# kan-bayashi/espnet

Hardware: AMD Instinct MI355X
Metric: frames/sec, 12L Conformer hybrid CTC/attention training step (B=32 T=1000 d=256 per GPU) (higher is better)
Workload: dtype f32; 1 GPU; BASELINE configs[1]: 12L Conformer enc d=256 h=4 ff=2048 k=31 macaron+cnn rel_pos, 6L Transformer dec, V=5000, fbank B=32 T=1000 L=100, mtlalpha 0.3, lsm 0.1; global_batch=32, frames=1000, parallelism=dp1, optimizer=adam+noam, clip 5.0, launch=hipGraph, wgrad_side_stream=False, optimizer_steps_done=113

## Files before the change

espnet_amd/_lib.py:

```python
import ctypes as C
import os
import re

import torch

_HERE = os.path.dirname(os.path.abspath(__file__))
LIB_PATH = os.path.join(_HERE, "csrc", "libespnet_amd_hip.so")


class EamdError(RuntimeError):
    pass


class GatherT(C.Structure):
    _fields_ = [("enabled", C.c_int32), ("C", C.c_int32), ("ntap", C.c_int32), ("Ho", C.c_int32),
                ("Wo", C.c_int32), ("Hin", C.c_int32), ("Win", C.c_int32), ("sh", C.c_int32),
                ("sw", C.c_int32), ("dh", C.c_int32 * 9), ("dw", C.c_int32 * 9)]


class RowMapT(C.Structure):
    _fields_ = [("enabled", C.c_int32), ("Ho", C.c_int32), ("Wo", C.c_int32), ("Hc", C.c_int32),
                ("Wc", C.c_int32), ("sh", C.c_int32), ("oh", C.c_int32), ("sw", C.c_int32),
                ("ow", C.c_int32)]


class RowStatsT(C.Structure):
    _fields_ = [("part", C.c_void_p), ("col", C.c_void_p), ("zcol", C.c_void_p), ("zfix", C.c_void_p),
                ("fix", C.c_int32), ("reserved", C.c_int32),
                ("rowc", C.c_void_p), ("gscale", C.c_void_p), ("scale", C.c_float), ("reserved2", C.c_int32)]


class GemmT(C.Structure):
    _fields_ = [("A", C.c_void_p), ("B", C.c_void_p), ("C", C.c_void_p), ("bias", C.c_void_p),
                ("aux", C.c_void_p), ("R", C.c_void_p), ("colsum", C.c_void_p),
                ("M", C.c_int32), ("N", C.c_int32), ("K", C.c_int32),
                ("transA", C.c_int32), ("transB", C.c_int32),
                ("lda", C.c_int64), ("ldb", C.c_int64), ("ldc", C.c_int64), ("ldaux", C.c_int64),
                ("ldr", C.c_int64),
                ("batch1", C.c_int32), ("batch2", C.c_int32),
                ("sA1", C.c_int64), ("sA2", C.c_int64), ("sB1", C.c_int64), ("sB2", C.c_int64),
                ("sC1", C.c_int64), ("sC2", C.c_int64),
                ("alpha", C.c_float), ("beta", C.c_float),
                ("a_act", C.c_int32), ("b_act", C.c_int32), ("epilogue", C.c_int32),
                ("splitk", C.c_int32), ("precision", C.c_int32), ("tile", C.c_int32),
                ("gather", GatherT), ("cmap", RowMapT),
                ("Cb", C.c_void_p), ("in_dtype", C.c_int32), ("aux_dtype", C.c_int32),
                ("drop_p", C.c_float), ("drop_salt", C.c_uint64), ("drop_step", C.c_void_p), ("Hb", C.c_void_p),
                ("h_act", C.c_int32), ("h_dtype", C.c_int32),
                ("stats", RowStatsT)]


class FfnT(C.Structure):
    _fields_ = [("x", C.c_void_p), ("w1", C.c_void_p), ("b1", C.c_void_p), ("w2", C.c_void_p), ("b2", C.c_void_p),
                ("R", C.c_void_p), ("out", C.c_void_p), ("f", C.c_void_p), ("h", C.c_void_p),
                ("M", C.c_int32), ("D", C.c_int32), ("F", C.c_int32), ("act", C.c_int32),
                ("alpha", C.c_float), ("p_in", C.c_float), ("salt_in", C.c_uint64), ("p_out", C.c_float),
                ("salt_out", C.c_uint64), ("drop_step", C.c_void_p), ("dtype", C.c_int32), ("hsplit", C.c_int32),
                ("ln_x", C.c_void_p), ("ln_w", C.c_void_p), ("ln_b", C.c_void_p), ("ln_mean", C.c_void_p),
                ("ln_rstd", C.c_void_p), ("ln_eps", C.c_float), ("reserved2", C.c_int32),
                ("lnb_x", C.c_void_p), ("lnb_gamma", C.c_void_p), ("lnb_mean", C.c_void_p), ("lnb_rstd", C.c_void_p),
                ("lnb_dres", C.c_void_p), ("lnb_ws", C.c_void_p), ("lnb_drop_out", C.c_void_p), ("lnb_drop_salt", C.c_uint64),
                ("lnb_drop_p", C.c_float), ("reserved3", C.c_int32)]


class RowProjT(C.Structure):
    _fields_ = [("a", C.c_void_p), ("lda", C.c_int64), ("w", C.c_void_p), ("bias", C.c_void_p), ("R", C.c_void_p),
                ("ldr", C.c_int64), ("out", C.c_void_p), ("ldo", C.c_int64),
                ("M", C.c_int32), ("K", C.c_int32), ("N", C.c_int32), ("a_act", C.c_int32),
                ("alpha", C.c_float), ("p_out", C.c_float), ("salt_out", C.c_uint64), ("drop_step", C.c_void_p),
                ("ln_x", C.c_void_p), ("ln_w", C.c_void_p), ("ln_b", C.c_void_p), ("ln_mean", C.c_void_p),
                ("ln_rstd", C.c_void_p), ("ln_eps", C.c_float), ("lnb_drop_p", C.c_float),
                ("a_scale", C.c_void_p), ("a_shift", C.c_void_p), ("a_out", C.c_void_p),
                ("lnb_x", C.c_void_p), ("lnb_gamma", C.c_void_p), ("lnb_mean", C.c_void_p), ("lnb_rstd", C.c_void_p),
                ("lnb_dres", C.c_void_p), ("lnb_ws", C.c_void_p), ("lnb_drop_out", C.c_void_p), ("lnb_drop_salt", C.c_uint64)]


class FfnPackT(C.Structure):
    _fields_ = [("w1", C.c_void_p), ("w2", C.c_void_p), ("fwd_first", C.c_void_p), ("fwd_second", C.c_void_p),
                ("bwd_first", C.c_void_p), ("bwd_second", C.c_void_p), ("D", C.c_int32), ("F", C.c_int32)]


class RowProjPackT(C.Structure):
    _fields_ = [("w", C.c_void_p), ("image", C.c_void_p), ("K", C.c_int32), ("N", C.c_int32), ("ldw", C.c_int32),
                ("trans", C.c_int32)]


class LstmSeqFwdT(C.Structure):
    _fields_ = [("gx", C.c_void_p), ("w_hh", C.c_void_p), ("b_hh", C.c_void_p), ("live", C.c_void_p),
                ("h_out", C.c_void_p), ("c_out", C.c_void_p), ("y", C.c_void_p), ("acts", C.c_void_p),
                ("reverse", C.c_int32), ("reserved", C.c_int32)]


class LstmSeqBwdT(C.Structure):
    _fields_ = [("dy", C.c_void_p), ("w_t", C.c_void_p), ("acts", C.c_void_p), ("c_out", C.c_void_p),
                ("live", C.c_void_p), ("dgates", C.c_void_p), ("reverse", C.c_int32), ("reserved", C.c_int32)]


_lib = None

HEADER_PATH = os.path.join(os.path.dirname(_HERE), "include", "espnet_amd.h")
_BY_VALUE = {"int": C.c_int, "int32_t": C.c_int, "int64_t": C.c_int64, "uint64_t": C.c_uint64, "float": C.c_float,
             "double": C.c_double}


def parse_prototypes(text):
    text = re.sub(r"/\*.*?\*/", "", text, flags=re.S)
    protos = {}
    for ret, name, params in re.findall(r"\b(\w+)\s+(eamd_\w+)\s*\(([^()]*)\)\s*;", text):
        def ctype(decl, named):
            if "*" in decl:
                return C.c_void_p
            words = [w for w in decl.split() if w != "const"]
            base = " ".join(words[:-1] if named else words)
            if base not in _BY_VALUE:
                raise EamdError(f"{name}: cannot bind by-value type '{base}' of '{decl.strip()}'")
            return _BY_VALUE[base]
        params = [] if params.strip() in ("", "void") else params.split(",")
        protos[name] = (ctype(ret, False), [ctype(p, True) for p in params])
    return protos


with open(HEADER_PATH) as _f:
    PROTOTYPES = parse_prototypes(_f.read())
SYMBOLS = list(PROTOTYPES)


def lib():
    global _lib
    if _lib is None:
        if not os.path.exists(LIB_PATH):
            raise EamdError(
                f"{LIB_PATH} not found: build it with `python -c 'import __graft_entry__ as g; g.build()'` "
                "or `make -C espnet_amd/csrc` (there is no CPU fallback)")
        handle = C.CDLL(LIB_PATH)
        for name, (restype, argtypes) in PROTOTYPES.items():
            fn = getattr(handle, name)
            fn.restype = restype
            fn.argtypes = argtypes
        _lib = handle
    return _lib


_raw_stream = getattr(torch._C, "_cuda_getCurrentRawStream", None)
_cur_device = getattr(torch._C, "_cuda_getDevice", None)


def stream_ptr():
    if _raw_stream is not None and _cur_device is not None:
        return _raw_stream(_cur_device())
    return torch.cuda.current_stream().cuda_stream


EAMD_EUNSUPPORTED = -2


def check(rc, what):
    if rc != 0:
        raise EamdError(f"{what} failed with code {rc}")


def ptr(t, offset=0):
    if t is None:
        return None
    if not t.is_cuda:
        raise EamdError("espnet_amd kernels need GPU tensors (no CPU fallback in the product path)")
    if offset == 0:
        return t.data_ptr()
    return t.data_ptr() + offset * t.element_size()


def f32(t):
    if t.dtype != torch.float32:
        raise EamdError(f"expected float32 tensor, got {t.dtype}")
    return t
```

espnet_amd/csrc/rowproj_f32.hip:

```cpp
#include <stdlib.h>
#include <type_traits>
#include "common.h"
#include "../../include/espnet_amd.h"
#include "ln_bwd_rows.h"

namespace {

constexpr int RBM = 32;
constexpr int RNT = 512;
constexpr int RCH = 256;
constexpr int ST_LD = 36;
constexpr int ST_SZ = RBM * ST_LD;
constexpr int TL_LD = 264;

__device__ __forceinline__ int xs_ld(int K) { return K + 8; }

__device__ __forceinline__ void stage_ln(const eamd_rowproj_t& p, const int m0, const int t, float* xs, const int LD) {
  constexpr int D = 256;
  const int row = t >> 4, l = t & 15;
  const bool live = m0 + row < p.M;
  const long gr = (long)min(m0 + row, p.M - 1);
  const float4* __restrict__ xr = reinterpret_cast<const float4*>(p.ln_x + gr * D);
  float4 v[4];
  float s = 0.f;
#pragma unroll
  for (int j = 0; j < 4; ++j) { v[j] = xr[l + 16 * j]; s += v[j].x + v[j].y + v[j].z + v[j].w; }
#pragma unroll
  for (int m = 1; m < 16; m <<= 1) s += __shfl_xor(s, m);
  const float mean = s / D;
  float q = 0.f;
#pragma unroll
  for (int j = 0; j < 4; ++j) {
    const float a = v[j].x - mean, b = v[j].y - mean, c = v[j].z - mean, d = v[j].w - mean;
    q += a * a + b * b + c * c + d * d;
  }
#pragma unroll
  for (int m = 1; m < 16; m <<= 1) q += __shfl_xor(q, m);
  const float rstd = rsqrtf(q / D + p.ln_eps);
  const float4* __restrict__ g4 = reinterpret_cast<const float4*>(p.ln_w);
  const float4* __restrict__ b4 = reinterpret_cast<const float4*>(p.ln_b);
#pragma unroll
  for (int j = 0; j < 4; ++j) {
    const float4 g = g4[l + 16 * j], b = b4[l + 16 * j];
    float4 o;
    o.x = (v[j].x - mean) * rstd * g.x + b.x;
    o.y = (v[j].y - mean) * rstd * g.y + b.y;
    o.z = (v[j].z - mean) * rstd * g.z + b.z;
    o.w = (v[j].w - mean) * rstd * g.w + b.w;
    const int col = (l + 16 * j) * 4;
    *reinterpret_cast<float4*>(&xs[row * LD + col]) = o;
    if (live) *reinterpret_cast<float4*>(const_cast<float*>(p.a) + gr * D + col) = o;
  }
  if (live && l == 0) { p.ln_mean[gr] = mean; p.ln_rstd[gr] = rstd; }
}

__device__ __forceinline__ void stage_affine(const eamd_rowproj_t& p, const int m0, const int t, float* xs, const int LD) {
  constexpr int D = 256;
#pragma unroll
  for (int i = 0; i < 4; ++i) {
    const int idx = t + RNT * i, row = idx >> 6, c4 = idx & 63;
    const long gr = (long)min(m0 + row, p.M - 1);
    const float4 v = *reinterpret_cast<const float4*>(p.a + gr * p.lda + c4 * 4);
    const float4 sc = *reinterpret_cast<const float4*>(p.a_scale + c4 * 4), sh = *reinterpret_cast<const float4*>(p.a_shift + c4 * 4);
    float4 o;
    o.x = eamd_act(v.x * sc.x + sh.x, p.a_act); o.y = eamd_act(v.y * sc.y + sh.y, p.a_act);
    o.z = eamd_act(v.z * sc.z + sh.z, p.a_act); o.w = eamd_act(v.w * sc.w + sh.w, p.a_act);
    *reinterpret_cast<float4*>(&xs[row * LD + c4 * 4]) = o;
    if (p.a_out && m0 + row < p.M) *reinterpret_cast<float4*>(p.a_out + gr * D + c4 * 4) = o;
  }
}

template <bool LNB>
__global__ __launch_bounds__(RNT, 2) void rowproj_f32_kernel(const eamd_rowproj_t p) {
  extern __shared__ __attribute__((aligned(16))) float sm[];
  const int K = p.K, N = p.N;
  const int LD = xs_ld(K);
  float* const xs = sm;
  const int t = threadIdx.x;
  const int lane = t & 63, wave = __builtin_amdgcn_readfirstlane(t >> 6);
  const int fr = lane & 15, fq = lane >> 4;
  const int m0 = blockIdx.x * RBM;
  const int S = K >> 5;
  const int nchunk = N / RCH;
  const int nsteps = S * nchunk;
  float* const st = sm + RBM * LD + wave * ST_SZ;

  if (p.ln_x) {
    stage_ln(p, m0, t, xs, LD);
  } else if (p.a_scale) {
    stage_affine(p, m0, t, xs, LD);
  } else {
    const int c4n = K >> 2;
    for (int idx = t; idx < RBM * c4n; idx += RNT) {
      const int row = idx / c4n, c4 = idx - row * c4n;
      *reinterpret_cast<f32x4*>(&xs[row * LD + c4 * 4]) =
          *reinterpret_cast<const f32x4*>(p.a + (long)min(m0 + row, p.M - 1) * p.lda + c4 * 4);
    }
  }

  const char* __restrict__ Wb = reinterpret_cast<const char*>(p.w) + (long)wave * 4096 + lane * 16;
  f32x4 bs[4][4];
  auto load_b = [&](auto set_c, int g) __attribute__((always_inline)) {
    constexpr int SET = decltype(set_c)::value;
    const char* base = Wb + (long)min(g, nsteps - 1) * (8 * 4096);
#pragma unroll
    for (int v = 0; v < 4; ++v) bs[SET][v] = *reinterpret_cast<const f32x4*>(base + v * 1024);
  };
  float fA[2][2][4];
  auto read_a = [&](int kcol, auto half_c) __attribute__((always_inline)) {
    constexpr int hh = decltype(half_c)::value;
#pragma unroll
    for (int i = 0; i < 2; ++i) {
      const float4 v = *reinterpret_cast<const float4*>(&xs[(i * 16 + fr) * LD + kcol + hh * 16 + fq * 4]);
      fA[hh][i][0] = v.x; fA[hh][i][1] = v.y; fA[hh][i][2] = v.z; fA[hh][i][3] = v.w;
    }
  };
  f32x4 acc[2][2];
  auto mfma_half = [&](auto set_c, auto half_c) __attribute__((always_inline)) {
    constexpr int SET = decltype(set_c)::value, q = decltype(half_c)::value;
#pragma unroll
    for (int e = 0; e < 4; ++e)
#pragma unroll
      for (int i = 0; i < 2; ++i)
#pragma unroll
        for (int j = 0; j < 2; ++j)
          acc[i][j] = __builtin_amdgcn_mfma_f32_16x16x4f32(fA[q][i][e], bs[SET][q * 2 + j][e], acc[i][j], 0, 0, 0);
  };
  using I0 = std::integral_constant<int, 0>;
  using I1 = std::integral_constant<int, 1>;
  auto step = [&](auto s_c, int g, int kcol, int kcol_next) __attribute__((always_inline)) {
    constexpr int s = decltype(s_c)::value;
    load_b(std::integral_constant<int, (s + 3) & 3>{}, g + 3);
    __builtin_amdgcn_sched_barrier(0);
    read_a(kcol, I1{});
    mfma_half(std::integral_constant<int, s & 3>{}, I0{});
    __builtin_amdgcn_sched_barrier(0);
    read_a(kcol_next, I0{});
    mfma_half(std::integral_constant<int, s & 3>{}, I1{});
  };

  load_b(std::integral_constant<int, 0>{}, 0);
  load_b(std::integral_constant<int, 1>{}, 1);
  load_b(std::integral_constant<int, 2>{}, 2);
  __syncthreads();
  read_a(0, I0{});

  const unsigned thr_out = eamd_drop_thr16(p.p_out);
  const float inv_out = eamd_drop_inv(thr_out);
  const unsigned seed_out = p.p_out > 0.f ? eamd_drop_seed((const unsigned long long*)p.drop_step, p.salt_out) : 0u;

  int g = 0;
  for (int c = 0; c < nchunk; ++c) {
#pragma unroll
    for (int i = 0; i < 2; ++i)
#pragma unroll
      for (int j = 0; j < 2; ++j) acc[i][j] = (f32x4){0.f, 0.f, 0.f, 0.f};
    for (int kp = 0; kp < S; kp += 4) {
      const int k0 = kp * 32;
      step(std::integral_constant<int, 0>{}, g + 0, k0, k0 + 32);
      step(std::integral_constant<int, 1>{}, g + 1, k0 + 32, k0 + 64);
      step(std::integral_constant<int, 2>{}, g + 2, k0 + 64, k0 + 96);
      step(std::integral_constant<int, 3>{}, g + 3, k0 + 96, (kp + 4 < S) ? k0 + 128 : 0);
      g += 4;
    }
    if constexpr (!LNB) {
#pragma unroll
      for (int i = 0; i < 2; ++i)
#pragma unroll
        for (int r = 0; r < 4; ++r)
          *reinterpret_cast<float2*>(&st[(i * 16 + fq * 4 + r) * ST_LD + 2 * fr]) = make_float2(acc[i][0][r], acc[i][1][r]);
      __builtin_amdgcn_fence(__ATOMIC_RELEASE, "wavefront");
      __builtin_amdgcn_wave_barrier();
      __builtin_amdgcn_fence(__ATOMIC_ACQUIRE, "wavefront");
      const int col0 = c * RCH + wave * 32 + (lane & 7) * 4;
      float4 b4 = make_float4(0.f, 0.f, 0.f, 0.f);
      if (p.bias) b4 = *reinterpret_cast<const float4*>(p.bias + col0);
#pragma unroll
      for (int it = 0; it < 4; ++it) {
        const int lr = it * 8 + (lane >> 3);
        const int row = m0 + lr;
        const float4 a4 = *reinterpret_cast<const float4*>(&st[lr * ST_LD + (lane & 7) * 4]);
        if (row < p.M) {
          float v[4] = {a4.x + b4.x, a4.y + b4.y, a4.z + b4.z, a4.w + b4.w};
          const long gi = (long)row * N + col0;
          if (p.p_out > 0.f) {
            bool keep[4];
            eamd_drop_keep4(seed_out, (unsigned long long)gi, thr_out, keep);
#pragma unroll
            for (int e = 0; e < 4; ++e) v[e] = keep[e] ? v[e] * inv_out : 0.f;
          }
          float4 r4 = make_float4(0.f, 0.f, 0.f, 0.f);
          if (p.R) r4 = *reinterpret_cast<const float4*>(p.R + (long)row * p.ldr + col0);
          *reinterpret_cast<float4*>(p.out + (long)row * p.ldo + col0) =
              make_float4(v[0] * p.alpha + r4.x, v[1] * p.alpha + r4.y, v[2] * p.alpha + r4.z, v[3] * p.alpha + r4.w);
        }
      }
      __builtin_amdgcn_wave_barrier();
    }
  }

  if constexpr (LNB) {
    constexpr int D = 256;
    float* const tl = sm;
    float* const gs = sm + RBM * TL_LD;
    float* const bsum = gs + RBM * D;
    __syncthreads();
#pragma unroll
    for (int i = 0; i < 2; ++i)
#pragma unroll
      for (int r = 0; r < 4; ++r)
        *reinterpret_cast<float2*>(&tl[(i * 16 + fq * 4 + r) * TL_LD + wave * 32 + 2 * fr]) = make_float2(acc[i][0][r], acc[i][1][r]);
    __syncthreads();
    const EamdLnbArgs la{p.lnb_x, p.lnb_gamma, p.lnb_mean, p.lnb_rstd, p.lnb_dres, p.lnb_ws, p.lnb_drop_out, p.lnb_drop_p,
                         (unsigned long long)p.lnb_drop_salt, p.drop_step, p.out, (long)p.ldo, p.M};
    eamd_ln_bwd_rows32<TL_LD>(la, tl, gs, bsum, m0, t, (int)blockIdx.x);
  }
}

struct PackJob { const float* w; float* img; int K, N, ldw, trans; long npiece; };
constexpr int PACK_JOBS = 48;
struct PackTable { PackJob j[PACK_JOBS]; };
__global__ __launch_bounds__(256) void rowproj_pack_kernel(const PackTable tab) {
  const PackJob jb = tab.j[blockIdx.y];
  for (long piece = (long)blockIdx.x * 256 + threadIdx.x; piece < jb.npiece; piece += (long)gridDim.x * 256) {
    const int lane = piece & 63, v = (piece >> 6) & 3, w = (piece >> 8) & 7;
    const long gs_ = piece >> 11;
    const int S = jb.K >> 5;
    const int c = (int)(gs_ / S), s = (int)(gs_ - (long)c * S);
    const int fr = lane & 15, fq = lane >> 4, q = v >> 1, j = v & 1;
    const int col = c * RCH + w * 32 + 2 * fr + j, k = s * 32 + q * 16 + fq * 4;
    float4 o;
    if (jb.trans) {
      const float* r0 = jb.w + (long)k * jb.ldw + col;
      o = make_float4(r0[0], r0[jb.ldw], r0[2L * jb.ldw], r0[3L * jb.ldw]);
    } else {
      o = *reinterpret_cast<const float4*>(jb.w + (long)col * jb.ldw + k);
    }
    *reinterpret_cast<float4*>(jb.img + piece * 4) = o;
  }
}

bool al16(const void* q) { return (reinterpret_cast<uintptr_t>(q) & 15) == 0; }

size_t smem_bytes(int K, bool lnb) {
  size_t rows = (size_t)RBM * (K + 8);
  if (lnb) {
    const size_t need = (size_t)RBM * TL_LD + 2 * (size_t)RBM * 256;
    return (rows > need ? rows : need) * sizeof(float);
  }
  return (rows + 8 * (size_t)ST_SZ) * sizeof(float);
}

int check_rowproj(const eamd_rowproj_t* p) {
  if (!p || !p->a || !p->w || !p->out) return EAMD_EINVAL;
  if (p->M <= 0 || p->K <= 0 || p->N <= 0) return EAMD_EINVAL;
  if (p->K % 256 != 0 || p->N % RCH != 0 || p->K > 768) return EAMD_EUNSUPPORTED;
  if (p->lda < p->K || p->ldo < p->N || (p->R && p->ldr < p->N)) return EAMD_EINVAL;
  if (p->lda % 4 != 0 || p->ldo % 4 != 0 || (p->R && p->ldr % 4 != 0)) return EAMD_EUNSUPPORTED;
  if (!al16(p->a) || !al16(p->w) || !al16(p->out) || (p->R && !al16(p->R)) || (p->bias && !al16(p->bias))) return EAMD_EUNSUPPORTED;
  if (p->p_out < 0.f || p->p_out >= 1.f) return EAMD_EINVAL;
  if (p->p_out > 0.f && (!p->drop_step || p->ldo != p->N)) return EAMD_EINVAL;
  if (p->ln_x) {
    if (p->K != 256 || p->a_scale || !p->ln_w || !p->ln_b || !p->ln_mean || !p->ln_rstd || p->lda != 256) return EAMD_EINVAL;
    if (!al16(p->ln_x) || !al16(p->ln_w) || !al16(p->ln_b)) return EAMD_EUNSUPPORTED;
  }
  if (p->a_scale) {
    if (p->K != 256 || !p->a_shift) return EAMD_EINVAL;
    if (!al16(p->a_scale) || !al16(p->a_shift) || (p->a_out && !al16(p->a_out))) return EAMD_EUNSUPPORTED;
  }
  if (p->lnb_x) {
    if (p->N != 256 || !p->lnb_gamma || !p->lnb_mean || !p->lnb_rstd || !p->lnb_ws || p->R || p->p_out > 0.f) return EAMD_EINVAL;
    if (p->lnb_drop_out && (!p->drop_step || p->lnb_drop_p < 0.f || p->lnb_drop_p >= 1.f)) return EAMD_EINVAL;
    if (!al16(p->lnb_x) || !al16(p->lnb_gamma) || (p->lnb_dres && !al16(p->lnb_dres)) || (p->lnb_drop_out && !al16(p->lnb_drop_out)))
      return EAMD_EUNSUPPORTED;
  }
  return EAMD_OK;
}

template <bool LNB>
int launch_rowproj(const eamd_rowproj_t& p, hipStream_t stream) {
  const size_t smem = smem_bytes(p.K, LNB);
  static int attr_done = 0;
  if (!attr_done) {
    const hipError_t e = hipFuncSetAttribute(reinterpret_cast<const void*>(&rowproj_f32_kernel<LNB>),
                                             hipFuncAttributeMaxDynamicSharedMemorySize, (int)smem_bytes(768, LNB));
    if (e != hipSuccess) return (int)e;
    attr_done = 1;
  }
  hipLaunchKernelGGL((rowproj_f32_kernel<LNB>), dim3((p.M + RBM - 1) / RBM), dim3(RNT), smem, stream, p);
  EAMD_LAUNCH_CHECK();
  return EAMD_OK;
}

}

extern "C" int64_t eamd_rowproj_lnb_workspace(int M) { return (int64_t)((M + RBM - 1) / RBM) * 2 * 256; }

extern "C" int eamd_rowproj(const eamd_rowproj_t* p, void* stream) {
  const int rc = check_rowproj(p);
  if (rc != EAMD_OK) return rc;
  return p->lnb_x ? launch_rowproj<true>(*p, (hipStream_t)stream) : launch_rowproj<false>(*p, (hipStream_t)stream);
}

extern "C" int eamd_rowproj_pack_f32(const eamd_rowproj_pack_t* jobs, int njobs, void* stream) {
  if (!jobs || njobs <= 0) return EAMD_EINVAL;
  for (int i0 = 0; i0 < njobs; i0 += PACK_JOBS) {
    const int n = njobs - i0 < PACK_JOBS ? njobs - i0 : PACK_JOBS;
    PackTable tab;
    long most = 0;
    for (int i = 0; i < n; ++i) {
      const eamd_rowproj_pack_t& q = jobs[i0 + i];
      if (!q.w || !q.image || q.K <= 0 || q.N <= 0 || q.ldw <= 0) return EAMD_EINVAL;
      if (q.K % 256 != 0 || q.N % RCH != 0 || !al16(q.image)) return EAMD_EUNSUPPORTED;
      if (!q.trans && (!al16(q.w) || q.ldw % 4 != 0)) return EAMD_EUNSUPPORTED;
      if (q.ldw < (q.trans ? q.N : q.K)) return EAMD_EINVAL;
      tab.j[i] = PackJob{q.w, q.image, q.K, q.N, q.ldw, q.trans, (long)q.K * q.N / 4};
      if (tab.j[i].npiece > most) most = tab.j[i].npiece;
    }
    const unsigned bx = (unsigned)((most + 255) / 256 < 256 ? (most + 255) / 256 : 256);
    hipLaunchKernelGGL(rowproj_pack_kernel, dim3(bx, n), dim3(256), 0, (hipStream_t)stream, tab);
    EAMD_LAUNCH_CHECK();
  }
  return EAMD_OK;
}
```

espnet_amd/functional.py:

```python
import math

import torch

from . import ops
from .ops import (ACT_NONE, ACT_RELU, ACT_SWISH, EPI_DACT_FACTOR, EPI_MUL_AUX, EPI_MUL_DSWISH, EPI_MUL_RELU_MASK, EPI_NONE,
                  EPI_RELU)


class GradSink:

    on_done = None
    on_use = None

    @staticmethod
    def use(params):
        if GradSink.on_use is not None and torch.is_grad_enabled():
            GradSink.on_use(params)
        return params

    def __init__(self, params):
        self.params = list(params)
        self.ret = [None] * len(self.params)

    def buf(self, i):
        p = self.params[i]
        if p is None:
            return None
        g = getattr(p, "_eamd_grad", None)
        if g is not None:
            return g
        if self.ret[i] is None:
            self.ret[i] = torch.zeros_like(p)
        return self.ret[i]

    def results(self):
        if GradSink.on_done is not None:
            ops.wgrad_join()
            GradSink.on_done(self.params)
        return tuple(self.ret)


FUSE_GRAD_DROP = True


def _tag_out(out, p_out, s_out):
    if FUSE_GRAD_DROP and p_out > 0.0:
        out._eamd_out_drop = (float(p_out), int(s_out))
    return out


def _prev_drop(x):
    return getattr(x, "_eamd_out_drop", None) if FUSE_GRAD_DROP else None


def _grad_in(dout, do, p_out, s_out):
    pre = getattr(dout, "_eamd_dropped", None)
    if pre is not None and pre[1] == (float(p_out), int(s_out)) and pre[0].numel() == do.numel():
        return pre[0].view(do.shape)
    return ops.dropout(do, p_out, s_out, out_dtype=ops.act_dtype()) if p_out > 0.0 else ops.to_act(do)


def _ln_fwd_in(x2, ln_w, ln_b, eps, adt):
    if eps is None:
        return ops.to_act(x2), None, None
    return ops.layernorm_fwd(x2, ln_w, ln_b, eps, adt)


def _ln_bwd_out(dxn, x2, ln_w, mean, rstd, do, gbuf, bbuf, prev, shp):
    if mean is None:
        return dxn.float().view(shp) if dxn.dtype != torch.float32 else dxn.view(shp)
    if prev is not None and x2.shape[1] in (256, 512):
        dx, dx16 = ops.layernorm_bwd(dxn, x2, ln_w, mean, rstd, do, gbuf, bbuf, drop=prev)
        out = dx.view(shp)
        out._eamd_dropped = (dx16, prev)
        return out
    return ops.layernorm_bwd(dxn, x2, ln_w, mean, rstd, do, gbuf, bbuf).view(shp)


def _rp_ln_bwd(dy, img, x2, ln_w, mean, rstd, do, gbuf, bbuf, prev, shp):
    M, D = x2.shape
    ws = ops.rowproj_lnb_ws(M, x2.device)
    dcopy = torch.empty(M, D, device=x2.device, dtype=torch.float32) if prev is not None else None
    dx = ops.rowproj(dy, img, D, lnb=(x2, ln_w, mean, rstd, do, ws, dcopy, prev))
    ops.ln_partials_reduce(ws, gbuf, bbuf, (M + 31) // 32, D)
    out = dx.view(shp)
    if prev is not None:
        out._eamd_dropped = (dcopy, prev)
    return out


def _act_epi(act):
    return {ACT_RELU: EPI_MUL_RELU_MASK, ACT_SWISH: EPI_MUL_DSWISH}[act]


class _NoGradCtx:
    needs_input_grad = (False,) * 64

    def save_for_backward(self, *tensors):
        pass

    def mark_non_differentiable(self, *tensors):
        pass

    def set_materialize_grads(self, value):
        pass


def run(fn, *args):
    if torch.is_grad_enabled():
        return fn.apply(*args)
    with ops.inference():
        return fn.forward(_NoGradCtx(), *args)


class DropoutFn(torch.autograd.Function):
    @staticmethod
    def forward(ctx, x, p, salt):
        ctx.cfg = (p, salt)
        return ops.dropout(x.contiguous(), p, salt)

    @staticmethod
    def backward(ctx, dy):
        p, salt = ctx.cfg
        return ops.dropout(dy.contiguous(), p, salt), None, None


def dropout(x, p, salt, training):
    return DropoutFn.apply(x, p, salt) if (training and p > 0.0) else x


class MaskRowsFn(torch.autograd.Function):

    @staticmethod
    def forward(ctx, x, keep):
        k8 = keep.reshape(-1).to(torch.uint8).contiguous()
        ctx.save_for_backward(k8)
        return ops.mask_rows(x.reshape(-1, x.shape[-1]).contiguous(), k8).view(x.shape)

    @staticmethod
    def backward(ctx, dy):
        (k8,) = ctx.saved_tensors
        return ops.mask_rows(dy.reshape(-1, dy.shape[-1]).contiguous(), k8).view(dy.shape), None


class LayerNormFn(torch.autograd.Function):
    @staticmethod
    def forward(ctx, x, weight, bias, eps):
        shp = x.shape
        x2 = x.reshape(-1, shp[-1]).contiguous()
        y, mean, rstd = ops.layernorm_fwd(x2, weight, bias, eps)
        ctx.save_for_backward(x2, mean, rstd)
        ctx.pr = GradSink.use((weight, bias))
        ctx.shp = shp
        ctx.prev = _prev_drop(x)
        return y.view(shp)

    @staticmethod
    def backward(ctx, dy):
        x2, mean, rstd = ctx.saved_tensors
        w, b = ctx.pr
        sink = GradSink([w, b])
        dy2 = dy.reshape(x2.shape).contiguous()
        dx = _ln_bwd_out(dy2, x2, w, mean, rstd, None, sink.buf(0), sink.buf(1), ctx.prev, ctx.shp)
        return (dx,) + sink.results() + (None,)


class LinearFn(torch.autograd.Function):
    @staticmethod
    def forward(ctx, x, weight, bias):
        shp = x.shape
        x2 = ops.to_act(x.reshape(-1, shp[-1]).contiguous())
        y = ops.linear_fwd(x2, ops.wshadow(weight), bias)
        ctx.save_for_backward(x2)
        ctx.pr = GradSink.use((weight, bias))
        ctx.shp = shp
        return y.view(*shp[:-1], weight.shape[0])

    @staticmethod
    def backward(ctx, dy):
        (x2,) = ctx.saved_tensors
        w, b = ctx.pr
        sink = GradSink([w, b] if b is not None else [w])
        dy2 = ops.to_act(dy.reshape(x2.shape[0], w.shape[0]).contiguous())
        dx = ops.linear_bwd_x(dy2, ops.wshadow(w)) if ctx.needs_input_grad[0] else None
        ops.linear_bwd_w(dy2, x2, sink.buf(0), db=sink.buf(1) if b is not None else None)
        res = sink.results()
        return (dx.view(ctx.shp) if dx is not None else None, res[0], res[1] if b is not None else None)


FFN_FACTOR = True


class FFNBlockFn(torch.autograd.Function):

    @staticmethod
    def forward(ctx, x, ln_w, ln_b, w1, b1, w2, b2, scale, act, eps, drop=(0.0, 0, 0.0, 0)):
        shp = x.shape
        D = shp[-1]
        adt = ops.act_dtype()
        p_in, s_in, p_out, s_out = drop
        x2 = x.reshape(-1, D).contiguous()
        assert eps is not None or p_out <= 0.0
        fused = ops.fast()
        h, zf = None, False
        one = eps is not None and (ops.fast() or ops.f32_epilogue_drop())
        ln_in = None
        if one and ops.FFN_LN_FUSED and x2.dtype == torch.float32 and D == 256:
            xn = torch.empty(x2.shape, device=x2.device, dtype=adt)
            if ops.ffn_fused_ok(xn, ops.wshadow(w1), ops.wshadow(w2), act):
                mean = torch.empty(x2.shape[0], device=x2.device, dtype=torch.float32)
                rstd = torch.empty(x2.shape[0], device=x2.device, dtype=torch.float32)
                ln_in = (x2, ln_w, ln_b, eps, mean, rstd)
        if ln_in is None:
            xn, mean, rstd = _ln_fwd_in(x2, ln_w, ln_b, eps, adt)
        if one and (ln_in is not None or ops.ffn_fused_ok(xn, ops.wshadow(w1), ops.wshadow(w2), act)):
            need = any(ctx.needs_input_grad[:7])
            packs = ops.ffn_pack(w1, w2)
            out, z, h = ops.ffn_fwd(xn, ops.wshadow(w1), b1, ops.wshadow(w2), b2, act=act, alpha=scale, R=x2,
                                    drop=(p_in, s_in, p_out, s_out), save=need, packed=packs[:2], ln=ln_in)
            ctx.packs = packs[2:]
            ctx.save_for_backward(x2, mean, rstd, xn, z, h)
            ctx.pr = GradSink.use((ln_w, ln_b, w1, b1, w2, b2))
            ctx.cfg = (scale, act, shp, drop)
            ctx.zf, ctx.one_launch = True, True
            ctx.prev = _prev_drop(x)
            return _tag_out(out.view(shp), p_out, s_out)
        ctx.one_launch = False
        if act not in (ACT_RELU, ACT_SWISH):
            if not (p_in > 0.0 and (fused or ops.f32_epilogue_drop())):
                z = ops.linear_fwd(xn, ops.wshadow(w1), b1)
                h = ops.act_fwd_any(z, act)
                if p_in > 0.0:
                    h = ops.dropout(h, p_in, s_in)
                hop = ops.to_act(h)
                if p_out > 0.0 and (fused or ops.f32_epilogue_drop()):
                    out = ops.linear_fwd(hop, ops.wshadow(w2), b2, R=x2 if eps is not None else None, alpha=scale, drop=(p_out, s_out))
                elif p_out > 0.0:
                    out = ops.axpby(x2, ops.dropout(ops.linear_fwd(hop, ops.wshadow(w2), b2), p_out, s_out), 1.0, scale)
                else:
                    out = ops.linear_fwd(hop, ops.wshadow(w2), b2, R=x2 if eps is not None else None, alpha=scale)
                ctx.save_for_backward(x2, mean, rstd, xn, z, hop)
                ctx.pr = GradSink.use((ln_w, ln_b, w1, b1, w2, b2))
                ctx.cfg = (scale, act, shp, drop)
                ctx.zf, ctx.generic_act = False, True
                ctx.prev = _prev_drop(x)
                return _tag_out(out.view(shp), p_out, s_out)
        ctx.generic_act = False
        if p_in > 0.0 and (fused or ops.f32_epilogue_drop()):
            h = torch.empty(x2.shape[0], w1.shape[0], device=x2.device, dtype=adt)
            z = ops.linear_fwd(xn, ops.wshadow(w1), b1, out_dtype=adt, drop=(p_in, s_in), Hb=h, h_act=act,
                               act=EPI_DACT_FACTOR if FFN_FACTOR else EPI_NONE)
            zf = FFN_FACTOR
        else:
            z = ops.linear_fwd(xn, ops.wshadow(w1), b1, out_dtype=adt)
            if p_in > 0.0:
                h = ops.dropout(z, p_in, s_in, act=act)
        src, a_act = (h, ACT_NONE) if h is not None else (z, act)
        if p_out > 0.0 and (fused or ops.f32_epilogue_drop()):
            out = ops.linear_fwd(src, ops.wshadow(w2), b2, R=x2, alpha=scale, a_act=a_act, drop=(p_out, s_out))
        elif p_out > 0.0:
            br = ops.linear_fwd(src, ops.wshadow(w2), b2, a_act=a_act)
            out = ops.axpby(x2, ops.dropout(br, p_out, s_out), 1.0, scale)
        else:
            out = ops.linear_fwd(src, ops.wshadow(w2), b2, R=x2 if eps is not None else None, alpha=scale, a_act=a_act)
        ctx.save_for_backward(x2, mean, rstd, xn, z, h)
        ctx.pr = GradSink.use((ln_w, ln_b, w1, b1, w2, b2))
        ctx.cfg = (scale, act, shp, drop)
        ctx.zf = zf
        ctx.prev = _prev_drop(x)
        return _tag_out(out.view(shp), p_out, s_out)

    @staticmethod
    def backward(ctx, dout):
        x2, mean, rstd, xn, z, h = ctx.saved_tensors
        ln_w, ln_b, w1, b1, w2, b2 = ctx.pr
        scale, act, shp, (p_in, s_in, p_out, s_out) = ctx.cfg
        adt = ops.act_dtype()
        sink = GradSink(ctx.pr)
        do = dout.reshape(x2.shape).contiguous()
        dob = _grad_in(dout, do, p_out, s_out)
        inner = h is not None
        if h is not None:
            ops.linear_bwd_w(dob, h, sink.buf(4), alpha=scale, db=sink.buf(5))
        else:
            ops.linear_bwd_w(dob, z, sink.buf(4), alpha=scale, b_act=act, db=sink.buf(5))
        if getattr(ctx, "generic_act", False):
            dh = ops.linear_bwd_x(dob, ops.wshadow(w2), alpha=scale)
            if p_in > 0.0:
                dh = ops.dropout(dh, p_in, s_in)
            dz = ops.to_act(ops.act_bwd_any(dh, z, act))
            ops.linear_bwd_w(dz, xn, sink.buf(2), db=sink.buf(3))
            dxn = ops.linear_bwd_x(dz, ops.wshadow(w1))
            dx = _ln_bwd_out(dxn, x2, ln_w, mean, rstd, do, sink.buf(0), sink.buf(1), ctx.prev, shp)
            return (dx,) + sink.results() + (None, None, None, None)
        if ctx.one_launch and dob.dtype == z.dtype:
            M, D = x2.shape
            if mean is not None and D == 256 and ops.ROWPROJ and ops.ffn_bwd_lnb_ok(M, w1.shape[0], dob.dtype):
                ws = ops.rowproj_lnb_ws(M, x2.device)
                prev = ctx.prev
                dcopy = torch.empty(M, D, device=x2.device, dtype=torch.float32) if prev is not None else None
                dz, dx = ops.ffn_bwd(dob, w1, w2, z, alpha=scale, packed=ctx.packs,
                                     lnb=(x2, ln_w, mean, rstd, do, ws, dcopy, prev))
                ops.ln_partials_reduce(ws, sink.buf(0), sink.buf(1), (M + 31) // 32, D)
                ops.linear_bwd_w(dz, xn, sink.buf(2), db=sink.buf(3))
                dx = dx.view(shp)
                if prev is not None:
                    dx._eamd_dropped = (dcopy, prev)
                return (dx,) + sink.results() + (None, None, None, None)
            dz, dxn = ops.ffn_bwd(dob, w1, w2, z, alpha=scale, packed=ctx.packs)
            ops.linear_bwd_w(dz, xn, sink.buf(2), db=sink.buf(3))
            dx = _ln_bwd_out(dxn, x2, ln_w, mean, rstd, do, sink.buf(0), sink.buf(1), ctx.prev, shp)
            return (dx,) + sink.results() + (None, None, None, None)
        if ctx.zf:
            dz = ops.linear_bwd_x(dob, ops.wshadow(w2), epilogue=EPI_MUL_AUX, aux=z, alpha=scale, out_dtype=adt)
        elif inner and (ops.fast() or ops.f32_epilogue_drop()):
            dz = ops.linear_bwd_x(dob, ops.wshadow(w2), epilogue=_act_epi(act), aux=z, alpha=scale, out_dtype=adt,
                                  drop=(p_in, s_in))
        else:
            dz = ops.linear_bwd_x(dob, ops.wshadow(w2), epilogue=_act_epi(act), aux=z, alpha=scale, out_dtype=adt)
            if inner:
                dz = ops.dropout(dz, p_in, s_in)
        ops.linear_bwd_w(dz, xn, sink.buf(2), db=sink.buf(3))
        dxn = ops.linear_bwd_x(dz, ops.wshadow(w1))
        dx = _ln_bwd_out(dxn, x2, ln_w, mean, rstd, do, sink.buf(0), sink.buf(1), ctx.prev, shp)
        return (dx,) + sink.results() + (None, None, None, None)


class Conv1dFFNBlockFn(torch.autograd.Function):

    @staticmethod
    def forward(ctx, x, ln_w, ln_b, w1, b1, w2, b2, scale, eps, drop=(0.0, 0, 0.0, 0)):
        B, T, D = x.shape
        H, k1 = w1.shape[0], w1.shape[2]
        k2 = w2.shape[2] if w2.dim() == 3 else 1
        adt = ops.act_dtype()
        p_in, s_in, p_out, s_out = drop
        x2 = x.reshape(-1, D).contiguous()
        xn, mean, rstd = ops.layernorm_fwd(x2, ln_w, ln_b, eps, adt)
        w1k = torch.empty(H, k1 * D, device=x.device, dtype=torch.float32)
        ops.permute4(w1.contiguous(), w1k, (H, D, k1, 1), (k1 * D, 1, D, 0))
        w1k = ops.to_act(w1k)
        col1 = ops.unfold1d(xn, B, T, D, k1) if k1 > 1 else xn
        z = ops.linear_fwd(col1, w1k, b1)
        h = ops.dropout(z, p_in, s_in, act=ACT_RELU, out_dtype=adt)
        if k2 > 1:
            w2k = torch.empty(D, k2 * H, device=x.device, dtype=torch.float32)
            ops.permute4(w2.contiguous(), w2k, (D, H, k2, 1), (k2 * H, 1, H, 0))
            w2k = ops.to_act(w2k)
            col2 = ops.unfold1d(h, B, T, H, k2)
        else:
            w2k, col2 = ops.wshadow(w2), h
        if p_out > 0.0:
            br = ops.linear_fwd(col2, w2k, b2)
            out = ops.axpby(x2, ops.dropout(br, p_out, s_out), 1.0, scale)
        else:
            out = ops.linear_fwd(col2, w2k, b2, R=x2, alpha=scale)
        ctx.save_for_backward(x2, mean, rstd, col1, z, col2, w1k, w2k)
        ctx.pr = GradSink.use((ln_w, ln_b, w1, b1, w2, b2))
        ctx.cfg = (scale, (B, T, D, H, k1, k2), drop)
        return out.view(B, T, D)

    @staticmethod
    def backward(ctx, dout):
        x2, mean, rstd, col1, z, col2, w1k, w2k = ctx.saved_tensors
        ln_w, ln_b, w1, b1, w2, b2 = ctx.pr
        scale, (B, T, D, H, k1, k2), (p_in, s_in, p_out, s_out) = ctx.cfg
        adt = ops.act_dtype()
        sink = GradSink(ctx.pr)
        do = dout.reshape(x2.shape).contiguous()
        dob = ops.dropout(do, p_out, s_out, out_dtype=adt) if p_out > 0.0 else ops.to_act(do)
        if k2 > 1:
            dw2k = torch.zeros(D, k2 * H, device=do.device, dtype=torch.float32)
            ops.linear_bwd_w(dob, col2, dw2k, alpha=scale, db=sink.buf(5))
            ops.permute4(dw2k, sink.buf(4), (D, k2, H, 1), (H * k2, 1, k2, 0), accumulate=True)
            dh = ops.fold1d(ops.linear_bwd_x(dob, w2k, alpha=scale), B, T, H, k2)
        else:
            ops.linear_bwd_w(dob, col2, sink.buf(4), alpha=scale, db=sink.buf(5))
            dh = ops.linear_bwd_x(dob, w2k, alpha=scale)
        if p_in > 0.0:
            dh = ops.dropout(dh, p_in, s_in)
        dz = ops.to_act(ops.act_bwd_any(dh, z, ACT_RELU))
        dw1k = torch.zeros(H, k1 * D, device=do.device, dtype=torch.float32)
        ops.linear_bwd_w(dz, col1, dw1k, db=sink.buf(3))
        ops.permute4(dw1k, sink.buf(2), (H, k1, D, 1), (D * k1, 1, k1, 0), accumulate=True)
        dcol = ops.linear_bwd_x(dz, w1k)
        dxn = ops.fold1d(dcol, B, T, D, k1) if k1 > 1 else dcol
        dx = ops.layernorm_bwd(dxn, x2, ln_w, mean, rstd, do, sink.buf(0), sink.buf(1))
        return (dx.view(B, T, D),) + sink.results() + (None, None, None)


def _ldp(T2):
    return (T2 + 7) // 8 * 8


class _MV:

    __slots__ = ("t", "off", "ld")

    def __init__(self, t, off=0, ld=None):
        self.t, self.off, self.ld = t, off, (t.shape[-1] if ld is None else ld)


def _mv(x):
    return x if isinstance(x, _MV) else _MV(x)


def attn_scores_fwd(qu, qv, k, p, mask, B, T1, T2, H, dk):
    D = H * dk
    ldp = _ldp(T2)
    qu, k = _mv(qu), _mv(k)
    ac = torch.empty(H * B * T1 * ldp, device=qu.t.device, dtype=torch.float32)
    ops.gemm(qu.t, k.t, ac, T1, T2, dk, qu.ld, k.ld, ldp, batch=(B, H), sA=(T1 * qu.ld, dk), sB=(T2 * k.ld, dk),
             sC=(T1 * ldp, B * T1 * ldp), a_off=qu.off, b_off=k.off)
    bd = None
    if p is not None:
        pm = _mv(p)
        bd = torch.empty_like(ac)
        ops.gemm(qv, pm.t, bd, T1, T2, dk, D, pm.ld, ldp, batch=(B, H), sA=(T1 * D, dk), sB=(0, dk),
                 sC=(T1 * ldp, B * T1 * ldp), b_off=pm.off)
    if ops.fast():
        P = torch.empty(H * B * T1 * ldp, device=ac.device, dtype=torch.bfloat16)
    else:
        P = ac
    ops.softmax_fwd(ac, bd, mask, P, H * B, B, T1, T2, ldp, 1.0 / math.sqrt(dk))
    return P


FUSE_ATTN = True
ATTN_RECOMPUTE_MB = 256.0
ATTN_TAP = None


def attn_fwd_fused(qu, qv, k, v, p, mask, B, T1, T2, H, dk, drop=None, shift_len=None):
    qu, k, v = _mv(qu), _mv(k), _mv(v)
    qv3 = p3 = None
    if p is not None:
        qvm, pm = _mv(qv), _mv(p)
        qv3, p3 = (qvm.t, qvm.off, qvm.ld), (pm.t, pm.off, pm.ld)
    return ops.attn_fwd((qu.t, qu.off, qu.ld), qv3, (k.t, k.off, k.ld), (v.t, v.off, v.ld), p3, mask, B, T1, T2, H, dk,
                        _ldp(T2), 1.0 / math.sqrt(dk), drop=drop, shift_len=shift_len)


def attn_context_fwd(P, v, B, T1, T2, H, dk):
    D = H * dk
    ldp = _ldp(T2)
    v = _mv(v)
    ctxv = torch.empty(B * T1, D, device=P.device, dtype=ops.act_dtype())
    ops.gemm(P, v.t, ctxv, T1, dk, T2, ldp, v.ld, D, transB=1, batch=(B, H), sA=(T1 * ldp, B * T1 * ldp),
             sB=(T2 * v.ld, dk), sC=(T1 * D, dk), b_off=v.off)
    return ctxv


def attn_core_bwd(dctx, P, qu, qv, k, v, p, B, T1, T2, H, dk, Pd=None, attn_drop=(0.0, 0), dqkv=None, dkv_out=None, shift_len=None,
                  dp_out=None):
    D = H * dk
    ldp = _ldp(T2)
    dev = dctx.device
    adt = ops.act_dtype()
    qu, k, v = _mv(qu), _mv(k), _mv(v)
    sP = (T1 * ldp, B * T1 * ldp)
    if dkv_out is not None:
        assert dqkv is None
        ldo = dkv_out.ld
        dkk, dk_off, dv, dv_off = dkv_out.t, dkv_out.off, dkv_out.t, dkv_out.off + D
    elif dqkv is None:
        dv, dv_off, ldo = torch.empty(B * T2, D, device=dev, dtype=adt), 0, D
        dkk, dk_off = torch.empty(B * T2, D, device=dev, dtype=adt), 0
    else:
        ldo = 3 * D
        dv, dv_off, dkk, dk_off = dqkv, 2 * D, dqkv, D
    kv_try = kv_fused = FUSE_ATTN and ops.FUSED_ATTN_KV and P.dtype == adt and dk == 64 and dctx.dtype == adt \
        and qu.t.dtype == adt
    if not kv_fused:
        ops.gemm(Pd if Pd is not None else P, dctx, dv, T2, dk, T1, ldp, D, ldo, transA=1, transB=1, batch=(B, H), sA=sP,
                 sB=(T1 * D, dk), sC=(T2 * ldo, dk), c_off=dv_off)
    dq_in_qkv = dqkv is not None and p is None
    dS = dbd = dqu = None
    if FUSE_ATTN and P.dtype == adt and ops.attn_fwd_supported(T1, T2, dk, p is not None):
        dS = torch.empty(H * B * T1 * ldp, device=dev, dtype=adt)
        dbd = torch.empty(H * B * T1 * ldp, device=dev, dtype=adt) if p is not None else None
        dqu = None if dq_in_qkv else torch.empty(B * T1, D, device=dev, dtype=torch.float32)
        dq_view = (dqkv, 0, ldo) if dq_in_qkv else (dqu, 0, D)
        if not ops.attn_bwd_q((dctx, 0, D), (k.t, k.off, k.ld), (v.t, v.off, v.ld), P, dS, dbd, dq_view, B, T1, T2, H, dk,
                              ldp, 1.0 / math.sqrt(dk), drop=attn_drop if Pd is not None else None, shift_len=shift_len):
            dS = None
    if dS is None and shift_len is not None:
        raise ops._lib.EamdError("relative-position attention backward on a shape-bucketed batch needs the fused kernel")
    if dS is None:
        dP = torch.empty(H * B * T1 * ldp, device=dev, dtype=torch.float32)
        ops.gemm(dctx, v.t, dP, T1, T2, dk, D, v.ld, ldp, batch=(B, H), sA=(T1 * D, dk), sB=(T2 * v.ld, dk), sC=sP,
                 b_off=v.off)
        if Pd is not None:
            dP = ops.dropout(dP, attn_drop[0], attn_drop[1])
        dbd = torch.empty(H * B * T1 * ldp, device=dev, dtype=adt) if p is not None else None
        if ops.fast():
            dS = torch.empty(H * B * T1 * ldp, device=dev, dtype=torch.bfloat16)
            ops.softmax_bwd(P, dP, dbd, H * B, T1, T2, ldp, 1.0 / math.sqrt(dk), dS16=dS)
        else:
            ops.softmax_bwd(P, dP, dbd, H * B, T1, T2, ldp, 1.0 / math.sqrt(dk))
            dS = dP
        if dq_in_qkv:
            dqu = None
            ops.gemm(dS, k.t, dqkv, T1, dk, T2, ldp, k.ld, ldo, transB=1, batch=(B, H), sA=sP, sB=(T2 * k.ld, dk),
                     sC=(T1 * ldo, dk), b_off=k.off)
        else:
            dqu = torch.empty(B * T1, D, device=dev, dtype=torch.float32)
            ops.gemm(dS, k.t, dqu, T1, dk, T2, ldp, k.ld, D, transB=1, batch=(B, H), sA=sP, sB=(T2 * k.ld, dk),
                     sC=(T1 * D, dk), b_off=k.off)
    dqv = dp = dpt = None
    if p is not None:
        pm = _mv(p)
        dqv = torch.empty(B * T1, D, device=dev, dtype=torch.float32)
        ops.gemm(dbd, pm.t, dqv, T1, dk, T2, ldp, pm.ld, D, transB=1, batch=(B, H), sA=sP, sB=(0, dk), sC=(T1 * D, dk),
                 b_off=pm.off)
        if dp_out is None:
            dp = torch.zeros(T2, D, device=dev, dtype=torch.float32)
            dpt, dp_off, ldd = dp, 0, D
        else:
            dpt, dp_off, ldd = dp_out.t, dp_out.off, dp_out.ld
    if kv_fused:
        kv_fused = ops.attn_bwd_kv(Pd if Pd is not None else P, dS, None, (dctx, 0, D), (qu.t, qu.off, qu.ld), None,
                                   (dv, dv_off, ldo), (dkk, dk_off, ldo), None, B, T1, T2, H, dk, ldp)
    if not kv_fused:
        if kv_try:
            ops.gemm(Pd if Pd is not None else P, dctx, dv, T2, dk, T1, ldp, D, ldo, transA=1, transB=1, batch=(B, H), sA=sP,
                     sB=(T1 * D, dk), sC=(T2 * ldo, dk), c_off=dv_off)
        ops.gemm(dS, qu.t, dkk, T2, dk, T1, ldp, qu.ld, ldo, transA=1, transB=1, batch=(B, H), sA=sP, sB=(T1 * qu.ld, dk),
                 sC=(T2 * ldo, dk), b_off=qu.off, c_off=dk_off)
    if p is not None:
        ops.gemm(dbd, qv, dpt, T2, dk, B * T1, ldp, D, ldd, transA=1, transB=1, batch=(1, H),
                 sA=(0, B * T1 * ldp), sB=(0, dk), sC=(0, dk), c_off=dp_off,
                 splitk=max(2, ops.auto_splitk(T2, dk, B * T1) // 2))
    return dqu, dqv, dkk, dv, dp


FUSE_QKV = True


def _adjacent3(a, b, c):
    n = a.numel() * a.element_size()
    return (a.is_contiguous() and b.is_contiguous() and c.is_contiguous() and a.numel() == b.numel() == c.numel()
            and b.data_ptr() == a.data_ptr() + n and c.data_ptr() == b.data_ptr() + n)


def _qkv_adjacent(wq, wk, wv, bq, bk, bv):
    if not FUSE_QKV or bq is None or not (_adjacent3(wq, wk, wv) and _adjacent3(bq, bk, bv)):
        return False
    gw = [getattr(t, "_eamd_grad", None) for t in (wq, wk, wv, bq, bk, bv)]
    if any(g is None for g in gw) or not (_adjacent3(*gw[:3]) and _adjacent3(*gw[3:])):
        return False
    return _adjacent3(ops.wshadow(wq), ops.wshadow(wk), ops.wshadow(wv))


def _span3(first, shape):
    stride = (shape[1], 1) if len(shape) == 2 else (1,)
    return first.detach().as_strided(shape, stride)


SHARE_PROJ = True


def _adjacent_run(ts):
    return all(a.is_contiguous() and b.is_contiguous() and b.data_ptr() == a.data_ptr() + a.numel() * a.element_size()
               for a, b in zip(ts, ts[1:]))


def shared_proj_ok(weights, biases=None):
    if not SHARE_PROJ or len(weights) < 2:
        return False
    for grp in (weights, biases):
        if grp is None:
            continue
        gr = [getattr(t, "_eamd_grad", None) for t in grp]
        if any(g is None for g in gr) or not (_adjacent_run(list(grp)) and _adjacent_run(gr)):
            return False
        if not _adjacent_run([ops.wshadow(t) for t in grp]):
            return False
    return True


class SharedProj:

    def __init__(self, out, nblk, zero_grad, grad_dtype):
        self.out, self.n = out, nblk
        self.ld = out.shape[1]
        self.width = self.ld // nblk
        self.dout, self.pending, self.done = None, [], 0
        self.zero_grad, self.grad_dtype = zero_grad, grad_dtype

    def block(self, i, sub=0):
        return _MV(self.out, i * self.width + sub, self.ld)

    def grad_block(self, i):
        if self.dout is None:
            mk = torch.zeros if self.zero_grad else torch.empty
            self.dout = mk(self.out.shape, device=self.out.device, dtype=self.grad_dtype)
        self.pending.append(i)
        return _MV(self.dout, i * self.width, self.ld)


class SharedProjFn(torch.autograd.Function):

    @staticmethod
    def forward(ctx, inp, box, zero_grad, nblk, n_w, *params):
        ctx.set_materialize_grads(False)
        ws, bs = params[:n_w], params[n_w:]
        Din = ws[0].shape[1]
        rows_w = sum(w.shape[0] for w in ws)
        adt = ops.act_dtype()
        inp2 = ops.to_act_shared(inp).reshape(-1, Din)
        W = ops.wshadow(ws[0]).detach().as_strided((rows_w, Din), (Din, 1))
        b = bs[0].detach().as_strided((rows_w,), (1,)) if bs else None
        out = ops.linear_fwd(inp2, W, b, out_dtype=adt)
        sp = SharedProj(out, nblk, zero_grad, torch.float32 if zero_grad else adt)
        box.append(sp)
        ctx.sp, ctx.inp2, ctx.W, ctx.shape = sp, inp2, W, inp.shape
        ctx.pr = GradSink.use(params)
        ctx.n_w = n_w
        return torch.zeros((), device=inp.device)

    @staticmethod
    def backward(ctx, _dtoken):
        sp, inp2, W = ctx.sp, ctx.inp2, ctx.W
        params = ctx.pr
        ws, bs = params[:ctx.n_w], params[ctx.n_w:]
        blocks = sorted(sp.pending)
        sp.pending = []
        dinp = None
        if blocks:
            assert blocks == list(range(blocks[0], blocks[-1] + 1)), "consumers of one backward pass are consecutive blocks"
            lo, hi = blocks[0] * sp.width, (blocks[-1] + 1) * sp.width
            M, Din, n = inp2.shape[0], inp2.shape[1], hi - lo
            dy = sp.dout if sp.dout.dtype == inp2.dtype else ops.to_act(sp.dout)
            rows_w = W.shape[0]
            dW = ws[0]._eamd_grad.as_strided((rows_w, Din), (Din, 1))[lo:hi]
            db = bs[0]._eamd_grad.as_strided((rows_w,), (1,))[lo:hi] if bs else None
            sk = ops.auto_splitk(n, Din, M)
            ops.gemm(dy, inp2, dW, n, Din, M, sp.ld, Din, Din, transA=1, transB=1, splitk=sk,
                     beta=1.0 if sk == 1 else 0.0, colsum=db, a_off=lo)
            if ctx.needs_input_grad[0]:
                dinp = torch.empty(M, Din, device=inp2.device, dtype=torch.float32)
                ops.gemm(dy, W, dinp, M, Din, n, sp.ld, Din, Din, transB=1, a_off=lo, b_off=lo * Din)
                dinp = dinp.view(ctx.shape)
            sp.done += len(blocks)
        if sp.done >= sp.n and GradSink.on_done is not None:
            ops.wgrad_join()
            GradSink.on_done(params)
        return (dinp, None, None, None, None) + (None,) * len(params)


class MHABlockFn(torch.autograd.Function):

    @staticmethod
    def forward(ctx, x, memory, pos_emb, mask, H, eps, last_query_only, drop, pre, token, *params):
        p_att, s_att, p_out, s_out = drop
        pre_kv = pre if (pre is not None and pre[0] == "kv") else None
        pre_pos = pre if (pre is not None and pre[0] == "pos") else None
        ln_w, ln_b, wq, bq, wk, bk, wv, bv, wo, bo = params[:10]
        rel = len(params) > 10
        B, T1f, D = x.shape
        dk = D // H
        adt = ops.act_dtype()
        x2 = x.reshape(-1, D).contiguous()
        fused = memory is None and not last_query_only and _qkv_adjacent(wq, wk, wv, bq, bk, bv)
        rp = None
        if fused and eps is not None and D == 256 and x2.dtype == torch.float32 and adt == torch.float32 \
                and ops.rowproj_ok(x2.shape[0], D, 3 * D) and (p_out <= 0.0 or ops.f32_epilogue_drop()):
            w3 = _span3(ops.wshadow(wq), (3 * D, D))
            rp = ops.rowproj_images(wq, [(w3, False), (w3, True), (wo.detach(), False), (wo.detach(), True)])
        if rp is not None:
            xn = torch.empty_like(x2)
            mean = torch.empty(x2.shape[0], device=x2.device, dtype=torch.float32)
            rstd = torch.empty_like(mean)
        else:
            xn, mean, rstd = _ln_fwd_in(x2, ln_w, ln_b, eps, adt)
        assert eps is not None or (p_out <= 0.0 and not last_query_only)
        if memory is None:
            kv_in, T2 = xn, T1f
        else:
            kv_in, T2 = ops.to_act_shared(memory).reshape(-1, D), memory.shape[1]
        if last_query_only:
            xq = xn.view(B, T1f, D)[:, -1, :]
            res = x2.view(B, T1f, D)[:, -1, :]
            if torch.is_grad_enabled():
                xq, res = xq.contiguous(), res.contiguous()
            T1 = 1
        else:
            xq, res, T1 = xn, (x2 if eps is not None else None), T1f
        if rp is not None:
            qkv = ops.rowproj(xn, rp[0], 3 * D, bias=_span3(bq, (3 * D,)), ln=(x2, ln_w, ln_b, eps, mean, rstd))
            q, k, v = _MV(qkv, 0, 3 * D), _MV(qkv, D, 3 * D), _MV(qkv, 2 * D, 3 * D)
        elif fused:
            w3, b3 = _span3(ops.wshadow(wq), (3 * D, D)), _span3(bq, (3 * D,))
            qkv = ops.linear_fwd(xq, w3, b3, out_dtype=adt)
            q, k, v = _MV(qkv, 0, 3 * D), _MV(qkv, D, 3 * D), _MV(qkv, 2 * D, 3 * D)
        else:
            qkv = None
            q = ops.linear_fwd(xq, ops.wshadow(wq), bq, out_dtype=adt)
            if pre_kv is not None:
                assert memory is not None
                k, v = pre_kv[1].block(pre_kv[2], 0), pre_kv[1].block(pre_kv[2], D)
            else:
                k = ops.linear_fwd(kv_in, ops.wshadow(wk), bk, out_dtype=adt)
                v = ops.linear_fwd(kv_in, ops.wshadow(wv), bv, out_dtype=adt)
        pos2 = None
        if rel:
            wpos, pu, pv = params[10:13]
            if pre_pos is not None:
                p = pre_pos[1].block(pre_pos[2])
            else:
                pos2 = ops.to_act_shared(pos_emb).reshape(-1, D)
                p = ops.linear_fwd(pos2, ops.wshadow(wpos), None, out_dtype=adt)
            if fused:
                qu, qv = ops.add_bias2(qkv, pu.reshape(-1), pv.reshape(-1), rows=B * T1, D=D, ldq=3 * D, q_off=0)
            else:
                qu, qv = ops.add_bias2(q, pu.reshape(-1), pv.reshape(-1))
        else:
            p, qu, qv = None, q, None
        fwd = None
        tb = ops.time_bound() if (rel and T1 == T2) else None
        ctx.shift_len = tb
        if FUSE_ATTN and ops.attn_fwd_supported(T1, T2, dk, rel):
            fwd = attn_fwd_fused(qu, qv, k, v, p, mask, B, T1, T2, H, dk, drop=(p_att, s_att) if p_att > 0.0 else None,
                                 shift_len=tb)
        if fwd is not None:
            P, Pd, cx = fwd
        else:
            if tb is not None:
                raise ops._lib.EamdError("relative-position attention on a shape-bucketed batch needs the fused attention kernels "
                                         "(d_k = 64, T' <= 4096: ops.attn_fwd_supported; train.BucketedGraphStep checks this per bucket up front); "
                                         "this shape runs the GEMM + softmax path")
            P = attn_scores_fwd(qu, qv, k, p, mask, B, T1, T2, H, dk)
            Pd = ops.dropout(P, p_att, s_att) if p_att > 0.0 else P
            cx = attn_context_fwd(Pd, v, B, T1, T2, H, dk)
        if ATTN_TAP is not None:
            ATTN_TAP.append(Pd.view(H, B, T1, _ldp(T2))[..., :T2].permute(1, 0, 2, 3).float())
        if rp is not None:
            out = ops.rowproj(cx, rp[2], D, bias=bo, R=res, drop=(p_out, s_out) if p_out > 0.0 else None)
        elif p_out > 0.0 and (ops.fast() or ops.f32_epilogue_drop()):
            out = ops.linear_fwd(cx, ops.wshadow(wo), bo, R=res, drop=(p_out, s_out))
        elif p_out > 0.0:
            br = ops.linear_fwd(cx, ops.wshadow(wo), bo)
            out = ops.axpby(res, ops.dropout(br, p_out, s_out), 1.0, 1.0)
        else:
            out = ops.linear_fwd(cx, ops.wshadow(wo), bo, R=res)
        ctx.rp = rp
        ctx.recompute = None
        if fwd is not None and ATTN_RECOMPUTE_MB >= 0:
            held = P.numel() * P.element_size() * (2 if p_att > 0.0 else 1)
            if held >= ATTN_RECOMPUTE_MB * 2 ** 20:
                ctx.recompute = mask
                P = Pd = None
        p_sv = None if pre_pos is not None else p
        if fused:
            ctx.save_for_backward(x2, mean, rstd, xn, None, qu if rel else None, qv, qkv, None, p_sv, P, cx, pos2,
                                  Pd if (p_att > 0.0 and P is not None) else None)
        elif pre_kv is not None:
            ctx.save_for_backward(x2, mean, rstd, xn, None, qu, qv, None, None, p_sv, P, cx, pos2,
                                  Pd if (p_att > 0.0 and P is not None) else None)
        else:
            ctx.save_for_backward(x2, mean, rstd, xn, kv_in if memory is not None else None, qu, qv, k, v, p_sv, P, cx,
                                  pos2, Pd if (p_att > 0.0 and P is not None) else None)
        ctx.pre = pre
        if pre is not None:
            skip = (4, 5, 6, 7) if pre_kv is not None else (10,)
            params = tuple(None if i in skip else q_ for i, q_ in enumerate(params))
        ctx.pr = GradSink.use(params)
        ctx.fused = fused
        ctx.cfg = (B, T1, T2, H, dk, D, rel, memory is not None, last_query_only, drop)
        ctx.prev = _prev_drop(x)
        return _tag_out(out.view(B, T1, D), p_out, s_out)

    @staticmethod
    def backward(ctx, dout):
        x2, mean, rstd, xn, mem2, qu, qv, k, v, p, P, cx, pos2, Pd = ctx.saved_tensors
        B, T1, T2, H, dk, D, rel, cross, last, (p_att, s_att, p_out, s_out) = ctx.cfg
        assert not last, "cached decoding path is inference-only"
        params = ctx.pr
        ln_w, ln_b, wq, bq, wk, bk, wv, bv, wo, bo = params[:10]
        adt = ops.act_dtype()
        sink = GradSink(params)
        pre = ctx.pre
        pre_kv = pre if (pre is not None and pre[0] == "kv") else None
        dp_out = None
        if pre is not None and pre[0] == "pos":
            p, dp_out = pre[1].block(pre[2]), pre[1].grad_block(pre[2])
        do = dout.reshape(-1, D).contiguous()
        dob = _grad_in(dout, do, p_out, s_out)
        rp = ctx.rp
        ops.linear_bwd_w(dob, cx, sink.buf(8), db=sink.buf(9))
        if rp is not None:
            dctx = ops.rowproj(dob, rp[3], D)
        else:
            dctx = ops.linear_bwd_x(dob, ops.wshadow(wo), out_dtype=adt)
        def again(qu_, qv_, k_, v_):
            f = attn_fwd_fused(qu_, qv_, k_, v_, p, ctx.recompute, B, T1, T2, H, dk, drop=(p_att, s_att) if p_att > 0.0 else None,
                               shift_len=ctx.shift_len)
            if f is None:
                raise ops._lib.EamdError("attention recompute: the fused forward declined operands it took in forward")
            return f[0], (f[1] if p_att > 0.0 else None)
        if ctx.fused:
            qkv = k
            dqkv = torch.empty(B * T1, 3 * D, device=do.device, dtype=adt)
            quv = qu if rel else _MV(qkv, 0, 3 * D)
            if P is None:
                P, Pd = again(quv, qv, _MV(qkv, D, 3 * D), _MV(qkv, 2 * D, 3 * D))
            dqu, dqv, _, _, dp = attn_core_bwd(dctx, P, quv, qv, _MV(qkv, D, 3 * D), _MV(qkv, 2 * D, 3 * D), p, B, T1,
                                               T2, H, dk, Pd=Pd, attn_drop=(p_att, s_att), dqkv=dqkv, dp_out=dp_out,
                                               shift_len=ctx.shift_len)
            if rel:
                wpos = params[10]
                ops.add_cast_colsum2(dqu, dqv, sink.buf(11).view(-1), sink.buf(12).view(-1), out=dqkv, out_off=0,
                                     ld_out=3 * D)
                if dp_out is None:
                    ops.linear_bwd_w(ops.to_act(dp), pos2, sink.buf(10))
            ops.linear_bwd_w(dqkv, xn, _span3(sink.buf(2), (3 * D, D)), db=_span3(sink.buf(3), (3 * D,)))
            if rp is not None:
                dx = _rp_ln_bwd(dqkv, rp[1], x2, ln_w, mean, rstd, do, sink.buf(0), sink.buf(1), ctx.prev, (B, T1, D))
            else:
                dxn = ops.linear_bwd_x(dqkv, _span3(ops.wshadow(wq), (3 * D, D)))
                dx = _ln_bwd_out(dxn, x2, ln_w, mean, rstd, do, sink.buf(0), sink.buf(1), ctx.prev, (B, T1, D))
            return (dx, None, None, None, None, None, None, None, None, None) + sink.results()
        dkv_out = None
        if pre_kv is not None:
            k, v = pre_kv[1].block(pre_kv[2], 0), pre_kv[1].block(pre_kv[2], D)
            dkv_out = pre_kv[1].grad_block(pre_kv[2])
        if P is None:
            P, Pd = again(qu, qv, k, v)
        dqu, dqv, dkk, dv, dp = attn_core_bwd(dctx, P, qu, qv, k, v, p, B, T1, T2, H, dk,
                                              Pd=Pd, attn_drop=(p_att, s_att), dkv_out=dkv_out, dp_out=dp_out,
                                              shift_len=ctx.shift_len)
        if rel:
            wpos = params[10]
            dq = ops.add_cast_colsum2(dqu, dqv, sink.buf(11).view(-1), sink.buf(12).view(-1))
            if dp_out is None:
                ops.linear_bwd_w(ops.to_act(dp), pos2, sink.buf(10))
        else:
            dq = ops.to_act(dqu)
        kv_in = mem2 if cross else xn
        ops.linear_bwd_w(dq, xn, sink.buf(2), db=sink.buf(3))
        dxn = ops.linear_bwd_x(dq, ops.wshadow(wq))
        dmem = None
        if pre_kv is not None:
            dx = _ln_bwd_out(dxn, x2, ln_w, mean, rstd, do, sink.buf(0), sink.buf(1), ctx.prev, (B, T1, D))
            return (dx, None, None, None, None, None, None, None, None, None) + sink.results()
        ops.linear_bwd_w(dkk, kv_in, sink.buf(4), db=sink.buf(5))
        ops.linear_bwd_w(dv, kv_in, sink.buf(6), db=sink.buf(7))
        if cross:
            dmem = ops.linear_bwd_x(dkk, ops.wshadow(wk))
            ops.linear_bwd_x(dv, ops.wshadow(wv), out=dmem, beta=1.0)
            dmem = dmem.view(B, T2, D)
        else:
            ops.linear_bwd_x(dkk, ops.wshadow(wk), out=dxn, beta=1.0)
            ops.linear_bwd_x(dv, ops.wshadow(wv), out=dxn, beta=1.0)
        dx = _ln_bwd_out(dxn, x2, ln_w, mean, rstd, do, sink.buf(0), sink.buf(1), ctx.prev, (B, T1, D))
        return (dx, dmem, None, None, None, None, None, None, None, None) + sink.results()


FUSE_GLU_DWCONV = True


class ConvModuleBlockFn(torch.autograd.Function):
    @staticmethod
    def forward(ctx, x, running_mean, running_var, training, act, eps, bn_eps, bn_momentum, drop, *params):
        p_out, s_out = drop
        ln_w, ln_b, w1, b1, wd, bd_, g, be, w2, b2 = params
        B, T, D = x.shape
        Cc = w2.shape[0]
        K = wd.shape[-1]
        M = B * T
        adt = ops.act_dtype()
        x2 = x.reshape(M, D).contiguous()
        rp = None
        if eps is not None and D == 256 and Cc == 256 and x2.dtype == torch.float32 and adt == torch.float32 \
                and ops.rowproj_ok(M, D, 2 * Cc) and (p_out <= 0.0 or ops.f32_epilogue_drop()):
            w1v, w2v = w1.detach().view(2 * Cc, D), w2.detach().view(Cc, Cc)
            rp = ops.rowproj_images(w1, [(w1v, False), (w1v, True), (w2v, False), (w2v, True)])
        if rp is not None:
            xn = torch.empty_like(x2)
            mean = torch.empty(M, device=x2.device, dtype=torch.float32)
            rstd = torch.empty_like(mean)
            a = ops.rowproj(xn, rp[0], 2 * Cc, bias=b1, ln=(x2, ln_w, ln_b, eps, mean, rstd))
        else:
            xn, mean, rstd = _ln_fwd_in(x2, ln_w, ln_b, eps, adt)
            a = ops.linear_fwd(xn, ops.wshadow(w1).view(2 * Cc, D), b1)
        assert eps is not None or p_out <= 0.0
        tb = ops.time_bound()
        bound = (T, tb) if tb is not None else None
        if bound is not None:
            ops.mask_time(a, T, tb)
        gl = d = bmean = None
        nbt = getattr(running_mean, "_eamd_nbt", None)
        if FUSE_GLU_DWCONV:
            d = ops.dwconv_glu_fwd(a, wd.view(Cc, K), bd_, B, T, Cc, K,
                                   bn=(bn_eps, bn_momentum, running_mean, running_var, nbt) if (training and bound is None) else None)
            if d is not None and training and bound is None:
                d, bmean, brstd = d
        if d is None:
            gl = ops.glu_fwd(a, Cc)
            d = ops.dwconv_fwd(gl, wd.view(Cc, K), bd_, B, T, Cc, K)
        if training:
            if bmean is None:
                bmean, brstd = ops.bn_stats(d, M, Cc, bn_eps, bn_momentum, running_mean, running_var, nbt, bound=bound)
        else:
            bmean = running_mean
            brstd = ops.axpby(running_var, None, 1.0, 0.0)
            brstd = torch.rsqrt_(brstd.add_(bn_eps))
        e = ops.bn_apply(d, bmean, brstd, g, be, M, Cc, act, adt)
        ctx.rp = rp
        if rp is not None:
            out = ops.rowproj(e, rp[2], Cc, bias=b2, R=x2, drop=(p_out, s_out) if p_out > 0.0 else None)
        elif p_out > 0.0 and (ops.fast() or ops.f32_epilogue_drop()):
            out = ops.linear_fwd(e, ops.wshadow(w2).view(Cc, Cc), b2, R=x2, drop=(p_out, s_out))
        elif p_out > 0.0:
            br = ops.linear_fwd(e, ops.wshadow(w2).view(Cc, Cc), b2)
            out = ops.axpby(x2, ops.dropout(br, p_out, s_out), 1.0, 1.0)
        else:
            out = ops.linear_fwd(e, ops.wshadow(w2).view(Cc, Cc), b2, R=x2 if eps is not None else None)
        ctx.save_for_backward(x2, mean, rstd, xn, a, gl, d, bmean, brstd, e)
        ctx.pr = GradSink.use(params)
        ctx.cfg = (B, T, D, Cc, K, act, training, drop)
        ctx.bound = bound
        ctx.prev = _prev_drop(x)
        return _tag_out(out.view(B, T, D), p_out, s_out)

    @staticmethod
    def backward(ctx, dout):
        x2, mean, rstd, xn, a, gl, d, bmean, brstd, e = ctx.saved_tensors
        ln_w, ln_b, w1, b1, wd, bd_, g, be, w2, b2 = ctx.pr
        B, T, D, Cc, K, act, training, (p_out, s_out) = ctx.cfg
        M = B * T
        adt = ops.act_dtype()
        sink = GradSink(ctx.pr)
        do = dout.reshape(M, D).contiguous()
        dob = _grad_in(dout, do, p_out, s_out)
        rp = ctx.rp
        ops.linear_bwd_w(dob, e, sink.buf(8).view(Cc, Cc), db=sink.buf(9))
        if rp is not None:
            de = ops.rowproj(dob, rp[3], Cc)
        else:
            de = ops.linear_bwd_x(dob, ops.wshadow(w2).view(Cc, Cc))
        dd = ops.bn_bwd(de, d, bmean, brstd, g, be, sink.buf(6), sink.buf(7), M, Cc, act, training, bound=ctx.bound)
        if gl is None:
            da = ops.dwconv_glu_bwd_x(dd, wd.view(Cc, K), a, B, T, Cc, K, adt)
            if ctx.bound is not None:
                ops.mask_time(da, T, ctx.bound[1])
            ops.dwconv_glu_bwd_w(dd, a, sink.buf(4).view(Cc, K), sink.buf(5), B, T, Cc, K)
        else:
            dgl = ops.dwconv_bwd_x(dd, wd.view(Cc, K), B, T, Cc, K)
            ops.dwconv_bwd_w(dd, gl, sink.buf(4).view(Cc, K), sink.buf(5), B, T, Cc, K)
            da = ops.glu_bwd(dgl, a, Cc, adt)
            if ctx.bound is not None:
                ops.mask_time(da, T, ctx.bound[1])
        ops.linear_bwd_w(da, xn, sink.buf(2).view(2 * Cc, D), db=sink.buf(3))
        if rp is not None and da.dtype == torch.float32:
            dx = _rp_ln_bwd(da, rp[1], x2, ln_w, mean, rstd, do, sink.buf(0), sink.buf(1), ctx.prev, (B, T, D))
        else:
            dxn = ops.linear_bwd_x(da, ops.wshadow(w1).view(2 * Cc, D))
            dx = _ln_bwd_out(dxn, x2, ln_w, mean, rstd, do, sink.buf(0), sink.buf(1), ctx.prev, (B, T, D))
        return (dx, None, None, None, None, None, None, None, None) + sink.results()


_TAPS_FWD = [(kh, kw) for kh in range(3) for kw in range(3)]
_CLASSES = [((0, 0), [(0, 0), (0, 2), (2, 0), (2, 2)]), ((0, 1), [(0, 1), (2, 1)]),
            ((1, 0), [(1, 0), (1, 2)]), ((1, 1), [(1, 1)])]


def _conv3s2_fwd(y_in, w, b, B, Hi, Wi, Cc, adt):
    Ho, Wo = (Hi - 3) // 2 + 1, (Wi - 3) // 2 + 1
    wf, wd = ops.conv2_weight_prep(w, adt)
    g = ops.make_gather(Cc, _TAPS_FWD, Ho, Wo, Hi, Wi, 2, 2)
    M = B * Ho * Wo
    y = torch.empty(M, Cc, device=y_in.device, dtype=adt)
    ops.gemm(y_in, wf, y, M, Cc, 9 * Cc, 9 * Cc, Cc, Cc, transB=1, bias=b, epilogue=EPI_RELU, gather=g)
    return y, wd, Ho, Wo


FUSE_CONV1_WGRAD = True


def _conv3s2_bwd_w(dy, y_in, dw_buf, db_buf, B, Hi, Wi, Ho, Wo, Cc):
    dev = dy.device
    M = B * Ho * Wo
    bsum = not ops.fast() and dy.dtype == torch.float32 and y_in.dtype == torch.float32
    if not bsum:
        ops.colsum(dy, db_buf)
    dwf = torch.zeros(9 * Cc, Cc, device=dev, dtype=torch.float32)
    g = ops.make_gather(Cc, _TAPS_FWD, Ho, Wo, Hi, Wi, 2, 2)
    f32_big = (not ops.fast()) and Cc % 128 == 0
    tile = 128 if f32_big else 64
    ntile = (9 * Cc // tile) * ((Cc + tile - 1) // tile)
    want = 1024 if ops.fast() else 1008 if f32_big else 2304
    sk = max(2, min(64, (want + ntile - 1) // ntile, max(1, M // 256)))
    ops.gemm(y_in, dy, dwf, 9 * Cc, Cc, M, 9 * Cc, Cc, Cc, transA=1, transB=1, gather=g, splitk=sk, tile=tile,
             colsum=db_buf if bsum else None)
    ops.conv2_weight_grad(dwf, dw_buf, Cc, Cc)


def _conv3s2_dx_classes(dy, y_in, wd, dy_in, B, Hi, Wi, Ho, Wo, Cc, tile=0):
    q0, classes = 0, []
    for (ph, pw), taps in _CLASSES:
        Hc, Wc = (Hi - ph + 1) // 2, (Wi - pw + 1) // 2
        if Hc > 0 and Wc > 0:
            gt = ops.make_gather(Cc, [((ph - kh) // 2, (pw - kw) // 2) for kh, kw in taps], Hc, Wc, Ho, Wo, 1, 1)
            cm = ops.make_rowmap(Hc, Wc, Hi, Wi, 2, ph, 2, pw)
            nt = len(taps)
            ops.gemm(dy, wd, dy_in, B * Hc * Wc, Cc, nt * Cc, nt * Cc, Cc, Cc, transB=1, b_off=q0 * Cc * Cc,
                     gather=gt, cmap=cm, epilogue=EPI_MUL_RELU_MASK, aux=y_in, ldaux=Cc, defer=classes, tile=tile)
        q0 += len(taps)
    return classes


def _conv3s2_bwd(dy, y_in, wd, dw_buf, db_buf, B, Hi, Wi, Ho, Wo, Cc, adt):
    _conv3s2_bwd_w(dy, y_in, dw_buf, db_buf, B, Hi, Wi, Ho, Wo, Cc)
    dy_in = torch.empty(y_in.shape, device=dy.device, dtype=adt)
    ops.gemm_multi(_conv3s2_dx_classes(dy, y_in, wd, dy_in, B, Hi, Wi, Ho, Wo, Cc))
    return dy_in


def _conv1w_fusable(y_in, Cc):
    return FUSE_CONV1_WGRAD and not ops.fast() and y_in.dtype == torch.float32 and Cc % 128 == 0


def _conv3s2_bwd_conv1w(dy, y_in, wd, dw_buf, db_buf, B, Hi, Wi, Ho, Wo, Cc, x, dw1_buf, db1_buf):
    _conv3s2_bwd_w(dy, y_in, dw_buf, db_buf, B, Hi, Wi, Ho, Wo, Cc)
    ops.conv2_bwd_x_conv1_bwd_w(_conv3s2_dx_classes(dy, y_in, wd, None, B, Hi, Wi, Ho, Wo, Cc, tile=128), x, dw1_buf, db1_buf)


def _taps(k):
    return [(kh, kw) for kh in range(k) for kw in range(k)]


def _conv_ks_fwd(y_in, w, b, B, Hi, Wi, Cc, adt, k, st):
    Ho, Wo = (Hi - k) // st + 1, (Wi - k) // st + 1
    KK = k * k
    wf = torch.empty(KK, Cc, Cc, device=y_in.device, dtype=torch.float32)
    ops.permute4(w.contiguous(), wf, (Cc, Cc, KK, 1), (1, Cc, Cc * Cc, 0))
    wd = torch.empty(KK, Cc, Cc, device=y_in.device, dtype=torch.float32)
    ops.permute4(w.contiguous(), wd, (Cc, Cc, KK, 1), (Cc, 1, Cc * Cc, 0))
    wf, wd = ops.to_act(wf), ops.to_act(wd)
    M = B * Ho * Wo
    y32 = torch.empty(M, Cc, device=y_in.device, dtype=torch.float32)
    taps = _taps(k)
    for t0 in range(0, KK, 9):
        ch = taps[t0:t0 + 9]
        g = ops.make_gather(Cc, ch, Ho, Wo, Hi, Wi, st, st)
        ops.gemm(y_in, wf, y32, M, Cc, len(ch) * Cc, len(ch) * Cc, Cc, Cc, transB=1, bias=b if t0 == 0 else None,
                 beta=0.0 if t0 == 0 else 1.0, gather=g, b_off=t0 * Cc * Cc)
    y = ops.dropout(y32, 0.0, 0, act=ACT_RELU, out_dtype=adt)
    return y, wd, Ho, Wo


def _conv_ks_bwd(dy, y_in, wd, dw_buf, db_buf, B, Hi, Wi, Ho, Wo, Cc, adt, k, st):
    dev = dy.device
    M = B * Ho * Wo
    KK = k * k
    taps = _taps(k)
    ops.colsum(dy, db_buf)
    dwf = torch.zeros(KK * Cc, Cc, device=dev, dtype=torch.float32)
    for t0 in range(0, KK, 9):
        ch = taps[t0:t0 + 9]
        g = ops.make_gather(Cc, ch, Ho, Wo, Hi, Wi, st, st)
        ntile = (len(ch) * Cc // 64) * ((Cc + 63) // 64)
        sk = max(2, min(64, (1024 + ntile - 1) // ntile, max(1, M // 256)))
        ops.gemm(y_in, dy, dwf, len(ch) * Cc, Cc, M, len(ch) * Cc, Cc, Cc, transA=1, transB=1, gather=g, splitk=sk, tile=64,
                 c_off=t0 * Cc * Cc)
    ops.permute4(dwf, dw_buf, (KK, Cc, Cc, 1), (1, KK, Cc * KK, 0), accumulate=True)
    dy_in = torch.empty(y_in.shape, device=dev, dtype=adt)
    order, classes = [], []
    for ph in range(st):
        for pw in range(st):
            ct = [(kh, kw) for kh in range(ph, k, st) for kw in range(pw, k, st)]
            classes.append(((ph, pw), ct))
            order += [kh * k + kw for kh, kw in ct]
    wd_cls = wd.index_select(0, torch.tensor(order, device=dev)).contiguous()
    q0, jobs = 0, []
    for (ph, pw), ct in classes:
        Hc, Wc = (Hi - ph + st - 1) // st, (Wi - pw + st - 1) // st
        if Hc > 0 and Wc > 0 and ct:
            gt = ops.make_gather(Cc, [((ph - kh) // st, (pw - kw) // st) for kh, kw in ct], Hc, Wc, Ho, Wo, 1, 1)
            cm = ops.make_rowmap(Hc, Wc, Hi, Wi, st, ph, st, pw)
            nt = len(ct)
            ops.gemm(dy, wd_cls, dy_in, B * Hc * Wc, Cc, nt * Cc, nt * Cc, Cc, Cc, transB=1, b_off=q0 * Cc * Cc,
                     gather=gt, cmap=cm, epilogue=EPI_MUL_RELU_MASK, aux=y_in, ldaux=Cc, defer=jobs)
        q0 += len(ct)
    ops.gemm_multi(jobs)
    return dy_in


class Conv2dSubsamplingFn(torch.autograd.Function):

    @staticmethod
    def forward(ctx, x, xscale, c1_w, c1_b, lin_w, lin_b, *convs):
        B, T, F = x.shape
        Cc = c1_w.shape[0]
        D = lin_w.shape[0]
        H1, W1 = (T - 3) // 2 + 1, (F - 3) // 2 + 1
        adt = ops.act_dtype()
        x = x.contiguous()
        ys = [ops.conv1_fwd(x, c1_w, c1_b, B, T, F, Cc, adt)]
        dims, wds = [(H1, W1)], []
        for i in range(0, len(convs), 2):
            k = convs[i].shape[-1]
            if k == 3:
                y, wd, Ho, Wo = _conv3s2_fwd(ys[-1].view(-1, Cc), convs[i], convs[i + 1], B, dims[-1][0], dims[-1][1], Cc, adt)
            else:
                y, wd, Ho, Wo = _conv_ks_fwd(ys[-1].view(-1, Cc), convs[i], convs[i + 1], B, dims[-1][0], dims[-1][1], Cc,
                                             adt, k, (k + 1) // 2)
            ys.append(y)
            wds.append(wd)
            dims.append((Ho, Wo))
        Hl, Wl = dims[-1]
        assert lin_w.shape[1] == Cc * Wl
        wl = torch.empty(D, Wl * Cc, device=x.device, dtype=torch.float32)
        ops.permute4(lin_w, wl, (D, Cc, Wl, 1), (Wl * Cc, 1, Cc, 0))
        wl = ops.to_act(wl)
        out = ops.linear_fwd(ys[-1].view(B * Hl, Wl * Cc), wl, lin_b, alpha=xscale)
        ctx.save_for_backward(x, wl, *ys, *wds)
        ctx.pr = GradSink.use((c1_w, c1_b, lin_w, lin_b) + tuple(convs))
        ctx.cfg = (B, T, F, Cc, D, dims, xscale)
        ctx.ks = [convs[i].shape[-1] for i in range(0, len(convs), 2)]
        return out.view(B, Hl, D)

    @staticmethod
    def backward(ctx, dout):
        B, T, F, Cc, D, dims, xscale = ctx.cfg
        n = len(dims) - 1
        x, wl = ctx.saved_tensors[:2]
        ys = ctx.saved_tensors[2:3 + n]
        wds = ctx.saved_tensors[3 + n:]
        adt = ops.act_dtype()
        sink = GradSink(ctx.pr)
        dev = x.device
        Hl, Wl = dims[-1]
        dob = ops.to_act(dout.reshape(B * Hl, D).contiguous())
        ylv = ys[-1].view(B * Hl, Wl * Cc)
        dwl = torch.zeros(D, Wl * Cc, device=dev, dtype=torch.float32)
        ops.linear_bwd_w(dob, ylv, dwl, alpha=xscale, db=sink.buf(3))
        ops.permute4(dwl, sink.buf(2), (D, Wl, Cc, 1), (Wl * Cc, 1, Wl, 0), accumulate=True)
        dy = ops.linear_bwd_x(dob, wl, epilogue=EPI_MUL_RELU_MASK, aux=ylv, alpha=xscale, out_dtype=adt)
        dy = dy.view(B * Hl * Wl, Cc)
        for i in range(n - 1, -1, -1):
            (Hi, Wi), (Ho, Wo) = dims[i], dims[i + 1]
            if i == 0 and ctx.ks[i] == 3 and _conv1w_fusable(ys[0], Cc):
                _conv3s2_bwd_conv1w(dy, ys[0].view(-1, Cc), wds[0], sink.buf(4), sink.buf(5), B, Hi, Wi, Ho, Wo, Cc, x,
                                    sink.buf(0), sink.buf(1))
                return (None, None) + sink.results()
            if ctx.ks[i] == 3:
                dy = _conv3s2_bwd(dy, ys[i].view(-1, Cc), wds[i], sink.buf(4 + 2 * i), sink.buf(5 + 2 * i), B, Hi, Wi, Ho,
                                  Wo, Cc, adt)
            else:
                dy = _conv_ks_bwd(dy, ys[i].view(-1, Cc), wds[i], sink.buf(4 + 2 * i), sink.buf(5 + 2 * i), B, Hi, Wi, Ho,
                                  Wo, Cc, adt, ctx.ks[i], (ctx.ks[i] + 1) // 2)
        ops.conv1_bwd_w(dy, x, sink.buf(0), sink.buf(1), B, T, F, Cc)
        return (None, None) + sink.results()


class EmbedPEFn(torch.autograd.Function):
    @staticmethod
    def forward(ctx, tokens, table, pe, scale, pos_offset):
        B, U = tokens.shape
        if U == 1 and not torch.is_grad_enabled():
            return ops.embed_pe(tokens, table, pe, U, scale, pos_offset).view(B, U, table.shape[1])
        tok = tokens.contiguous()
        out = ops.embed_pe(tok, table, pe, U, scale, pos_offset)
        ctx.save_for_backward(tok)
        ctx.pr = GradSink.use((table,))
        ctx.scale = scale
        return out.view(B, U, table.shape[1])

    @staticmethod
    def backward(ctx, dout):
        (tok,) = ctx.saved_tensors
        sink = GradSink(ctx.pr)
        ops.embed_bwd(tok, dout.reshape(-1, dout.shape[-1]).contiguous(), sink.buf(0), ctx.scale)
        return (None,) + sink.results() + (None, None, None)


class PosEncFn(torch.autograd.Function):

    @staticmethod
    def forward(ctx, x, pe, scale):
        B, T, D = x.shape
        ctx.scale = scale
        return ops.posenc(x.reshape(-1, D).contiguous(), pe, T, scale).view(B, T, D)

    @staticmethod
    def backward(ctx, dout):
        return ops.axpby(dout.contiguous(), None, ctx.scale, 0.0), None, None


class ScaledPosEncFn(torch.autograd.Function):

    @staticmethod
    def forward(ctx, x, pe, alpha, scale):
        B, T, D = x.shape
        ctx.save_for_backward(pe)
        ctx.pr = GradSink.use((alpha,))
        ctx.cfg = (T, scale)
        return ops.posenc_scaled(x.reshape(-1, D).contiguous(), pe, alpha.reshape(1), T, scale).view(B, T, D)

    @staticmethod
    def backward(ctx, dout):
        (pe,) = ctx.saved_tensors
        T, scale = ctx.cfg
        sink = GradSink(ctx.pr)
        do = dout.contiguous()
        ops.posenc_scaled_bwd(do.view(-1, do.shape[-1]), pe, sink.buf(0).view(1), T)
        dx = do if scale == 1.0 else ops.axpby(do, None, scale, 0.0)
        res = sink.results()
        return dx, None, res[0], None


# ... 100 lines not shown
```

espnet_amd/nets/e2e_asr_transformer.py:

```python
import argparse
import math
from itertools import groupby

import numpy as np
import torch

from .. import functional as F_
from .. import ops
from .asr_interface import ASRInterface
from .modules import (CTC, Decoder, LabelSmoothingLoss, TransformerEncoder, make_non_pad_mask,
                      embed_output_lengths, grad_cut, subsampled_lengths, subsampled_stride, subsequent_mask, th_accuracy)

CTC_LOSS_THRESHOLD = 10000


def strtobool(v):
    v = str(v).lower()
    if v in ("y", "yes", "t", "true", "on", "1"):
        return 1
    if v in ("n", "no", "f", "false", "off", "0"):
        return 0
    raise ValueError("invalid truth value %r" % (v,))


def add_arguments_transformer_common(group):
    group.add_argument("--transformer-init", type=str, default="pytorch")
    group.add_argument("--transformer-input-layer", type=str, default="conv2d",
                       choices=["conv2d", "linear", "embed"])
    group.add_argument("--transformer-attn-dropout-rate", default=None, type=float)
    group.add_argument("--transformer-lr", default=10.0, type=float)
    group.add_argument("--transformer-warmup-steps", default=25000, type=int)
    group.add_argument("--transformer-length-normalized-loss", default=True, type=strtobool)
    group.add_argument("--transformer-encoder-selfattn-layer-type", type=str, default="selfattn")
    group.add_argument("--transformer-decoder-selfattn-layer-type", type=str, default="selfattn")
    group.add_argument("--wshare", default=4, type=int)
    group.add_argument("--ldconv-encoder-kernel-length", default="21_23_25_27_29_31_33_35_37_39_41_43", type=str)
    group.add_argument("--ldconv-decoder-kernel-length", default="11_13_15_17_19_21", type=str)
    group.add_argument("--ldconv-usebias", type=strtobool, default=False)
    group.add_argument("--dropout-rate", default=0.0, type=float)
    group.add_argument("--elayers", default=4, type=int)
    group.add_argument("--eunits", "-u", default=300, type=int)
    group.add_argument("--adim", default=320, type=int)
    group.add_argument("--aheads", default=4, type=int)
    group.add_argument("--dlayers", default=1, type=int)
    group.add_argument("--dunits", default=320, type=int)
    return group


_DEFAULTS = dict(mtlalpha=0.3, lsm_weight=0.0, ctc_type="warpctc", report_cer=False, report_wer=False,
                 char_list=None, sym_space="<space>", sym_blank="<blank>")


def fill_missing_args(args, add_arguments):
    parser = argparse.ArgumentParser()
    add_arguments(parser)
    defaults, _ = parser.parse_known_args([])
    merged = dict(_DEFAULTS)
    merged.update(vars(defaults))
    merged.update(vars(args))
    return argparse.Namespace(**merged)


class Reporter:

    def __init__(self):
        self.last = {}

    def report(self, loss_ctc, loss_att, acc, cer_ctc, cer, wer, mtl_loss):
        self.last = dict(loss_ctc=loss_ctc, loss_att=loss_att, acc=acc, cer_ctc=cer_ctc, cer=cer, wer=wer,
                         loss=mtl_loss)


class E2E(ASRInterface, torch.nn.Module):

    @staticmethod
    def add_arguments(parser):
        group = parser.add_argument_group("transformer model setting")
        add_arguments_transformer_common(group)
        return parser

    def get_total_subsampling_factor(self):
        return 4

    reports_errors = True

    def _build_encoder(self, idim, args):
        if args.transformer_encoder_selfattn_layer_type != "selfattn":
            raise NotImplementedError("encoder selfattention_layer_type must be selfattn for the Transformer E2E")
        return TransformerEncoder(
            idim=idim, attention_dim=args.adim, attention_heads=args.aheads, linear_units=args.eunits,
            num_blocks=args.elayers, input_layer=args.transformer_input_layer, dropout_rate=args.dropout_rate,
            positional_dropout_rate=args.dropout_rate, attention_dropout_rate=args.transformer_attn_dropout_rate)

    def __init__(self, idim, odim, args, ignore_id=-1):
        torch.nn.Module.__init__(self)
        args = fill_missing_args(args, self.add_arguments)
        if args.transformer_attn_dropout_rate is None:
            args.transformer_attn_dropout_rate = args.dropout_rate
        self.encoder = self._build_encoder(idim, args)
        if args.mtlalpha < 1:
            self.decoder = Decoder(
                odim=odim, selfattention_layer_type=args.transformer_decoder_selfattn_layer_type,
                attention_dim=args.adim, attention_heads=args.aheads, linear_units=args.dunits,
                num_blocks=args.dlayers, dropout_rate=args.dropout_rate, positional_dropout_rate=args.dropout_rate,
                self_attention_dropout_rate=args.transformer_attn_dropout_rate,
                src_attention_dropout_rate=args.transformer_attn_dropout_rate)
            self.criterion = LabelSmoothingLoss(odim, ignore_id, args.lsm_weight,
                                                bool(args.transformer_length_normalized_loss))
        else:
            self.decoder = None
            self.criterion = None
        self.blank = 0
        self.sos = odim - 1
        self.eos = odim - 1
        self.odim = odim
        self.ignore_id = ignore_id
        self.subsample = np.array([1])
        self.reporter = Reporter()
        self.adim = args.adim
        self.mtlalpha = args.mtlalpha
        if args.mtlalpha > 0.0:
            self.ctc = CTC(odim, args.adim, args.dropout_rate, ctc_type=args.ctc_type, reduce=True)
        else:
            self.ctc = None
        if self.reports_errors and (args.report_cer or args.report_wer):
            from .e2e_asr_common import ErrorCalculator
            self.error_calculator = ErrorCalculator(args.char_list, args.sym_space, args.sym_blank, args.report_cer,
                                                    args.report_wer)
        else:
            self.error_calculator = None
        self.rnnlm = None
        self.sync_report = True
        self.reset_parameters(args)

    def reset_parameters(self, args):
        init_type = args.transformer_init
        if init_type == "pytorch":
            return
        fn = {"xavier_uniform": torch.nn.init.xavier_uniform_, "xavier_normal": torch.nn.init.xavier_normal_,
              "kaiming_uniform": lambda p: torch.nn.init.kaiming_uniform_(p, nonlinearity="relu"),
              "kaiming_normal": lambda p: torch.nn.init.kaiming_normal_(p, nonlinearity="relu")}
        if init_type not in fn:
            raise ValueError("Unknown initialization: " + init_type)
        for p in self.parameters():
            if p.dim() > 1:
                fn[init_type](p.data)
        for p in self.parameters():
            if p.dim() == 1:
                p.data.zero_()
        for m in self.modules():
            if isinstance(m, (torch.nn.Embedding, torch.nn.LayerNorm)):
                m.reset_parameters()

    def prepare(self, xs_pad, ilens, ys_pad, pad_to=None):
        il = [int(v) for v in (ilens.tolist() if isinstance(ilens, torch.Tensor) else ilens)]
        tmax = max(il)
        dev = next(self.parameters()).device
        hl_true = tbound = None
        if pad_to is not None:
            Tb, Lb = pad_to
            assert Tb >= tmax
            hl_true = embed_output_lengths(self.encoder.embed, il, tmax)
            tbound = embed_output_lengths(self.encoder.embed, [tmax], tmax)[0]
            xp = xs_pad.new_zeros(xs_pad.shape[0], Tb, xs_pad.shape[2])
            xp[:, :tmax] = xs_pad[:, :tmax]
            yp = ys_pad.new_full((ys_pad.shape[0], Lb), self.ignore_id)
            n = min(Lb, ys_pad.shape[1])
            yp[:, :n] = ys_pad[:, :n]
            xs_pad, ys_pad, tmax = xp, yp, Tb
        xs_pad = ops.h2d_async(xs_pad[:, :tmax], dev).contiguous()
        ys_host = ys_pad
        ys_pad = ops.h2d_async(ys_pad, dev).contiguous()
        if hl_true is None:
            mask_len = il
        else:
            stride = max(1, subsampled_stride(self.encoder.embed))
            mask_len = [(h - 1) * stride + 1 if h > 0 else 0 for h in hl_true]
        src_mask = ops.h2d_async(make_non_pad_mask(mask_len, tmax).unsqueeze(-2).to(torch.uint8), dev)
        batch = dict(xs_pad=xs_pad, ys_pad=ys_pad, src_mask=src_mask, B=xs_pad.size(0))
        if tbound is not None:
            batch["tbound"] = ops.h2d_async(torch.tensor([tbound], dtype=torch.int32), dev)
        if self.decoder is not None:
            batch.update(self.decoder_inputs(ys_host, ys_pad, dev))
        if self.mtlalpha > 0.0:
            hl = hl_true if hl_true is not None else embed_output_lengths(self.encoder.embed, il, tmax)
            batch["hs_len"] = ops.h2d_async(torch.tensor(hl, dtype=torch.int32), dev)
        return batch

    def decoder_inputs(self, ys_host, ys_pad, dev):
        ys_in_pad, ys_out_pad, _ = ops.add_sos_eos(ys_pad, self.sos, self.eos, self.ignore_id)
        U = ys_in_pad.size(1)
        ys_mask = subsequent_mask(U).unsqueeze(0).expand(ys_pad.size(0), U, U).to(torch.uint8).contiguous()
        return dict(ys_in_pad=ys_in_pad, ys_out_pad=ys_out_pad, ys_mask=ops.h2d_async(ys_mask, dev),
                    n_valid=(ys_out_pad != self.ignore_id).sum())

    def forward_core(self, batch):
        xs_pad = batch["xs_pad"]
        ops.set_time_bound(batch.get("tbound"))
        try:
            hs_pad, hs_mask = self.encoder(xs_pad, batch["src_mask"])
        finally:
            ops.set_time_bound(None)
        hs_pad = grad_cut(hs_pad)
        self.hs_pad = hs_pad
        if hs_mask is not None and not hs_mask.is_contiguous():
            hs_mask = hs_mask.contiguous()
        loss_att = loss_ctc = None
        self._acc_t = None
        if self.decoder is not None:
            pred_pad, _ = self.decoder(batch["ys_in_pad"], batch["ys_mask"], hs_pad, hs_mask)
            self.pred_pad = pred_pad
            loss_att = self.criterion(pred_pad, batch["ys_out_pad"])
            self._acc_t = ops.reduce_sum(self.criterion.correct_rows) / batch["n_valid"]
        if self.mtlalpha > 0.0:
            loss_ctc = self.ctc(hs_pad.view(batch["B"], -1, self.adim), batch["hs_len"], batch["ys_pad"])
        alpha = self.mtlalpha
        if alpha == 0:
            self.loss = loss_att
        elif alpha == 1:
            self.loss = loss_ctc
        else:
            self.loss = F_.WeightedSumFn.apply(loss_ctc, loss_att, alpha)
        self._loss_ctc_t, self._loss_att_t = loss_ctc, loss_att
        self._cer_ctc_n = self._cer_n = self._wer_n = None
        if not self.training and self.error_calculator is not None:
            with torch.no_grad():
                if self.mtlalpha > 0.0:
                    ys_hat = self.ctc.argmax(hs_pad.view(batch["B"], -1, self.adim))
                    self._cer_ctc_n = self.error_calculator.counts(ys_hat, batch["ys_pad"], is_ctc=True)
                if self.decoder is not None:
                    B, U, V = pred_pad.shape
                    ys_hat = ops.argmax_rows(pred_pad.detach().reshape(B * U, V).contiguous()).view(B, U)
                    self._cer_n, self._wer_n = self.error_calculator.counts(ys_hat, batch["ys_pad"])
        return self.loss

    def forward(self, xs_pad, ilens, ys_pad):
        self.loss = self.forward_core(self.prepare(xs_pad, ilens, ys_pad))
        self.acc = None
        if self.sync_report:
            self._report()
        return self.loss

    def _report(self):
        lc = float(self._loss_ctc_t.detach()) if self._loss_ctc_t is not None else None
        la = float(self._loss_att_t.detach()) if self._loss_att_t is not None else None
        self.acc = float(self._acc_t) if self.decoder is not None else None
        loss_data = float(self.loss.detach())
        cer_ctc = cer = wer = None
        if self.error_calculator is not None:
            n_ctc, n_cer, n_wer = self.error_calculator.sums(self._cer_ctc_n, self._cer_n, self._wer_n)
            cer_ctc = float(n_ctc[0]) / n_ctc[1] if n_ctc is not None and n_ctc[1] > 0 else None
            cer = float(n_cer[0]) / n_cer[1] if n_cer is not None else None
            wer = float(n_wer[0]) / n_wer[1] if n_wer is not None else None
        if loss_data < CTC_LOSS_THRESHOLD and not math.isnan(loss_data):
            self.reporter.report(lc, la, self.acc, cer_ctc, cer, wer, loss_data)
        return loss_data

    def scorers(self):
        from .ctc_prefix_score import CTCPrefixScorer
        return dict(decoder=self.decoder, ctc=CTCPrefixScorer(self.ctc, self.eos))

    def encode(self, x):
        self.eval()
        dev = next(self.parameters()).device
        x = torch.as_tensor(np.asarray(x) if not isinstance(x, torch.Tensor) else x, dtype=torch.float32)
        x = x.to(dev).unsqueeze(0)
        with torch.no_grad():
            enc_output, _ = self.encoder(x, None)
        return enc_output.squeeze(0)

    @ops.inference_call
    def recognize(self, x, recog_args, char_list=None, rnnlm=None, use_jit=False, ngram=None):
        if self.mtlalpha == 1.0:
            recog_args.ctc_weight = 1.0
        if self.mtlalpha > 0 and recog_args.ctc_weight == 1.0 and recog_args.beam_size > 1:
            self._refuse_rnnlm_for_pure_ctc(rnnlm)
            enc_output = self.encode(x)
            return self._ctc_prefix_beam(enc_output.unsqueeze(0), [enc_output.shape[0]], recog_args, ngram)[0]
        enc_output = self.encode(x).unsqueeze(0)
        if self.mtlalpha > 0 and recog_args.ctc_weight == 1.0:
            with torch.no_grad():
                ids = self.ctc.argmax(enc_output).to(torch.int32)
                hyp, n = ops.ctc_collapse(ids.contiguous(), None, self.blank)
            hyp = hyp[0, : int(n[0])].tolist()
            return [{"score": 0.0, "yseq": [self.sos] + hyp}]
        from .beam_search import recognize_beam
        return recognize_beam(self, enc_output.squeeze(0), recog_args, char_list, rnnlm, ngram=ngram)

    @staticmethod
    def _refuse_rnnlm_for_pure_ctc(rnnlm):
        if rnnlm is not None:
            raise ValueError("a neural LM (rnnlm) cannot be fused into the time-synchronous pure-CTC beam search: "
                             "pass an n-gram LM (ngram=) or decode with ctc_weight < 1")

    def _ctc_prefix_beam(self, hs_pad, hlens, recog_args, ngram):
        if self.blank != 0 or self.eos != self.odim - 1:
            raise ValueError("CTC prefix beam search: blank = 0 and eos = odim - 1, not %d / %d" % (self.blank, self.eos))
        return self.ctc.prefix_beam_search(
            hs_pad, hlens, beam_size=recog_args.beam_size, cand_size=getattr(recog_args, "ctc_cand_size", None),
            nbest=min(getattr(recog_args, "nbest", 1), recog_args.beam_size), penalty=getattr(recog_args, "penalty", 0.0),
            ngram=ngram, ngram_weight=getattr(recog_args, "ngram_weight", 0.0) if ngram is not None else 0.0)

    @ops.inference_call
    def recognize_batch(self, xs, recog_args, char_list=None, rnnlm=None, ngram=None):
        if self.mtlalpha == 1.0 or (self.mtlalpha > 0 and recog_args.ctc_weight == 1.0):
            if recog_args.beam_size > 1:
                self._refuse_rnnlm_for_pure_ctc(rnnlm)
                encs = [self.encode(x) for x in xs]
                hs_pad = torch.nn.utils.rnn.pad_sequence(encs, batch_first=True)
                return self._ctc_prefix_beam(hs_pad, [e.shape[0] for e in encs], recog_args, ngram)
            return [self.recognize(x, recog_args, char_list, rnnlm) for x in xs]
        from .beam_search import recognize_beam_batch
        return recognize_beam_batch(self, [self.encode(x) for x in xs], recog_args, char_list, rnnlm, ngram=ngram)

    def greedy_ctc_batch(self, xs_pad, ilens):
        il = [int(v) for v in (ilens.tolist() if isinstance(ilens, torch.Tensor) else ilens)]
        tmax = max(il)
        with torch.no_grad():
            hs, _ = self.encoder(xs_pad[:, :tmax], make_non_pad_mask(il).unsqueeze(-2))
            ids = self.ctc.argmax(hs).to(torch.int32).contiguous()
            hl = torch.tensor(embed_output_lengths(self.encoder.embed, il, tmax), dtype=torch.int32).to(ids.device)
            return ops.ctc_collapse(ids, hl, self.blank)

    def calculate_all_attentions(self, xs_pad, ilens, ys_pad):
        from .modules import MultiHeadedAttention
        self.eval()
        F_.ATTN_TAP = []
        try:
            with torch.no_grad():
                self.forward(xs_pad, ilens, ys_pad)
        finally:
            F_.ATTN_TAP = None
        ret = dict()
        for name, m in self.named_modules():
            if isinstance(m, MultiHeadedAttention) and m.attn is not None:
                ret[name] = m.attn.cpu().numpy()
        self.train()
        return ret

    def calculate_all_ctc_probs(self, xs_pad, ilens, ys_pad):
        if self.mtlalpha == 0:
            return None
        self.eval()
        with torch.no_grad():
            self.forward(xs_pad, ilens, ys_pad)
            ret = self.ctc.softmax(self.hs_pad).cpu().numpy()
        self.train()
        return ret
```

espnet_amd/ops.py:

```python
import ctypes as C
import os
import math

import torch

from . import _lib
from ._lib import GatherT, GemmT, RowMapT, check, ptr, stream_ptr

ACT_NONE, ACT_RELU, ACT_SWISH = 0, 1, 2
EPI_NONE, EPI_RELU, EPI_SWISH, EPI_MUL_RELU_MASK, EPI_MUL_DSWISH, EPI_MUL_AUX, EPI_DACT_FACTOR, EPI_ROW_STATS, EPI_ROW_GRAD = 0, 1, 2, 3, 4, 5, 6, 7, 8

_PRECISIONS = {"fp32": 0, "bf16": 1}
_state = {"precision": 0}


def set_precision(name):
    if name not in _PRECISIONS:
        raise ValueError(f"precision must be one of {list(_PRECISIONS)}")
    _state["precision"] = _PRECISIONS[name]


def get_precision():
    return [k for k, v in _PRECISIONS.items() if v == _state["precision"]][0]

# ... 288 lines not shown
        if dyc.shape[0] <= STACK_WGRAD_MAX_ROWS:
            sk = auto_splitk(dyc.shape[1], xc.shape[1], dyc.shape[0])
            gemm(dyc, xc, dW, dyc.shape[1], xc.shape[1], dyc.shape[0], dyc.shape[1], xc.shape[1], xc.shape[1], transA=1,
                 transB=1, splitk=sk, beta=1.0 if sk == 1 else 0.0, colsum=db, group=True)
        else:
            _linear_bwd_w(dyc, xc, dW, db=db)
    items = _wgroup["items"]
    if not items:
        return
    _wgroup["items"], _wgroup["ranges"], _wgroup["bytes"] = [], [], 0
    for tile in (64, 128):
        part = [it for it in items if (128 if it[0].tile == 128 else 64) == tile]
        if part:
            _wgroup_launch(part, tile)


def _wgroup_launch(items, tile):
    L = _lib.lib()

    def separately():
        for p, keep in items:
            if _gemm_record is not None:
                _gemm_record.append((p, keep, lambda sp, p=p: check(L.eamd_gemm(C.byref(p), sp), "eamd_gemm")))
            check(L.eamd_gemm(C.byref(p), stream_ptr()), "eamd_gemm")

    if len(items) == 1:
        return separately()
    n = len(items)
    dev = items[0][1][0].device
    arr = (GemmT * n)(*[it[0] for it in items])
    first = (C.c_int32 * (n + 1))()
    total = L.eamd_gemm_group_plan(arr, n, first)
    check(min(total, 0), "eamd_gemm_group_plan")
    nb_desc, nb_first = C.sizeof(arr), C.sizeof(first)
    host = _wgroup_staging(nb_desc + nb_first)
    if host is None:
        return separately()
    C.memmove(host.data_ptr(), arr, nb_desc)
    C.memmove(host.data_ptr() + nb_desc, first, nb_first)
    tab = torch.empty(nb_desc + nb_first, dtype=torch.uint8, device=dev)
    tab.copy_(host, non_blocking=True)
    in_dtype = int(arr[0].in_dtype)
    args = (ptr(tab), ptr(tab, nb_desc), n, total, in_dtype, tile)
    check(L.eamd_gemm_group_launch(*args, stream_ptr()), "eamd_gemm_group_launch")
    if _gemm_record is not None:
        _gemm_record.append((dict(kind="group%d" % tile, flop=sum(2.0 * it[0].M * it[0].N * it[0].K * it[0].batch1 * it[0].batch2 for it in items)),
                             (tab, [it[1] for it in items]),
                             lambda sp, args=args: check(L.eamd_gemm_group_launch(*args, sp), "eamd_gemm_group_launch")))


def cast_bf16(x, out=None):
    if out is None:
        out = torch.empty(x.shape, device=x.device, dtype=torch.bfloat16)
    assert x.dtype == torch.float32 and x.is_contiguous() and out.numel() == x.numel()
    check(_lib.lib().eamd_cast_bf16(ptr(x), ptr(out), x.numel(), stream_ptr()), "eamd_cast_bf16")
    return out


def auto_splitk(m_out, n_out, k_red):
    tiles = ((m_out + 63) // 64) * ((n_out + 63) // 64)
    if tiles >= 512:
        return 1
    want = 4.0 * (128.0 / tiles) ** 0.5
    s = 1
    while s < want:
        s *= 2
    return max(1, min(s, 64, max(1, k_red // 128)))


LINEAR_ROWS = True
_infer = 0


class inference:

    def __enter__(self):
        global _infer
        _infer += 1

    def __exit__(self, *exc):
        global _infer
        _infer -= 1
        return False


def inference_call(fn):
    import functools

    @functools.wraps(fn)
    def wrapped(*a, **k):
        with inference():
            return fn(*a, **k)
    return wrapped
LINEAR_ROWS_MAX = 16
LINEAR_ROWS_BLOCK_MAX = 1024
LINEAR_ROWS_KSPLIT = True


def linear_fwd(x, W, b, out=None, *, act=EPI_NONE, R=None, alpha=1.0, a_act=ACT_NONE, out_dtype=torch.float32,
               drop=None, Hb=None, h_act=ACT_NONE):
    M, K = x.shape
    N = W.shape[0]
    assert W.shape[1] == K and W.is_contiguous() and x.stride(1) == 1 and (R is None or R.stride(-1) == 1)
    if (LINEAR_ROWS and (M <= LINEAR_ROWS_MAX or (M <= LINEAR_ROWS_BLOCK_MAX and (K <= 512 or (K >= 1024 and LINEAR_ROWS_KSPLIT)) and N <= 1024
                                                  and K % 16 == 0)) and out is None and out_dtype == torch.float32 and x.dtype == torch.float32 and W.dtype == torch.float32
            and act in (EPI_NONE, EPI_RELU, EPI_SWISH) and a_act in (ACT_NONE, ACT_RELU, ACT_SWISH) and drop is None and Hb is None
            and K % 4 == 0 and _state["precision"] == 0 and _infer > 0 and not torch.is_grad_enabled()
            and (R is None or (tuple(R.shape) == (M, N) and (M == 1 or R.stride(0) >= N))) and (M == 1 or x.stride(0) >= K)):
        y = torch.empty(M, N, device=x.device, dtype=torch.float32)
        rc = _lib.lib().eamd_linear_rows_f32(ptr(x), ptr(W), ptr(b), ptr(R), ptr(y), M, N, K, a_act, act, alpha,
                                             x.stride(0), R.stride(0) if R is not None else 0, stream_ptr())
        if rc == 0:
            return y
        if rc != _lib.EAMD_EUNSUPPORTED:
            check(rc, "eamd_linear_rows_f32")
    x = x.contiguous()
    R = R.contiguous() if R is not None else None
    sk = 1
    if (out_dtype if out is None else out.dtype) == torch.float32 and act == EPI_NONE and drop is None and Hb is None:
        if R is None and alpha == 1.0:
            sk = _skinny_splitk(M, N, K)
        elif K >= 1024 and M <= 512 and x.is_cuda and torch.cuda.is_current_stream_capturing():
            sk = _skinny_splitk(M, N, K, max_rows=512)
    if out is None:
        out = zeros(M, N, device=x.device) if sk > 1 else torch.empty(M, N, device=x.device, dtype=out_dtype)
    elif sk > 1:
        out.zero_()
    gemm(x, W, out, M, N, K, K, K, N, bias=b, epilogue=act, R=R, ldr=N, alpha=alpha, a_act=a_act, drop=drop, Hb=Hb,
         h_act=h_act, splitk=sk)
    return out


class _ZeroArena:
    buf = None
    off = 0
    need = 0
    cap = 0
    active = False
    tracking = False
    capture = 0


_zarena = _ZeroArena()
ZERO_ARENA = True
ZERO_ARENA_MAX = 1024 << 20


def _capture_id():
    if not torch.cuda.is_available() or not torch.cuda.is_current_stream_capturing():
        return 0
    try:
        from . import graphs
        return graphs.capture_id()
    except Exception:
        return -1


def zero_arena_begin(device):
    a = _zarena
    if a.tracking:
        a.cap = min(ZERO_ARENA_MAX, (int(a.need * 1.25) + 4095) // 4096 * 4096)
    a.off, a.need, a.tracking = 0, 0, True
    a.active = ZERO_ARENA and a.cap > 0
    a.capture = _capture_id() if (a.active and torch.device(device).type == "cuda") else 0
    a.buf = torch.zeros(a.cap // 4, device=device, dtype=torch.float32) if a.active else None


def zero_arena_off():
    a = _zarena
    a.active, a.tracking, a.buf, a.off, a.need, a.capture = False, False, None, 0, 0, 0


def zeros(*shape, device):
    if len(shape) == 1 and isinstance(shape[0], (tuple, list, torch.Size)):
        shape = tuple(shape[0])
    n = 1
    for d in shape:
        n *= int(d)
    a = _zarena
    nb = (n * 4 + 255) // 256 * 256
    if a.tracking:
        a.need += nb
    if a.active and n > 0 and a.off + nb <= a.buf.numel() * 4 and a.buf.device == torch.device(device) \
            and (not a.buf.is_cuda or _capture_id() == a.capture):
        t = a.buf[a.off // 4: a.off // 4 + n].view(shape)
        a.off += nb
        return t
    return torch.zeros(shape, device=device, dtype=torch.float32)


def _skinny_splitk(M, N, K, max_rows=64):
    if M > max_rows or N * K < 512 * 512:
        return 1
    tiles = (M + 63) // 64 * ((N + 63) // 64)
    sk = 1
    while tiles * sk < 256 and K // (sk * 2) >= 128:
        sk *= 2
    return sk


def linear_bwd_x(dy, W, out=None, *, beta=0.0, epilogue=EPI_NONE, aux=None, alpha=1.0, out_dtype=torch.float32,
                 drop=None):
    M, N = dy.shape
    K = W.shape[1]
    assert W.shape[0] == N and dy.is_contiguous()
    fresh = out is None
    sk = 1
    if fresh and out_dtype == torch.float32 and epilogue == EPI_NONE and aux is None and drop is None and alpha == 1.0:
        sk = _skinny_splitk(M, K, N)
    if out is None:
        assert beta == 0.0
        out = zeros(M, K, device=dy.device) if sk > 1 else torch.empty(M, K, device=dy.device, dtype=out_dtype)
    gemm(dy, W, out, M, K, N, N, K, K, transB=1, beta=beta, epilogue=epilogue, aux=aux, ldaux=K, alpha=alpha,
         drop=drop, splitk=sk)
    return out


FUSED_FFN = True
FUSED_FFN_MIN_ROWS = 4096


def ffn_fused_ok(x, w1, w2, act):
    bf = x.dtype == torch.bfloat16
    if not FUSED_FFN or x.dtype != w1.dtype or w1.dtype != w2.dtype or (bf and _state["precision"] != 1) or \
            (not bf and (x.dtype != torch.float32 or _state["precision"] != 0)):
        return False
    return (x.shape[1] == 256 and w1.shape[1] == 256 and w1.shape[0] % (256 if bf else 128) == 0 and w1.shape[0] >= 256
            and tuple(w2.shape) == (256, w1.shape[0]) and act in (ACT_RELU, ACT_SWISH)
            and (x.shape[0] >= FUSED_FFN_MIN_ROWS or ffn_hsplit(x.shape[0], w1.shape[0], bf) > 1))


FUSED_FFN_HSPLIT_MIN_ROWS = 1536


def ffn_hsplit(M, F, bf):
    if bf or M >= FUSED_FFN_MIN_ROWS or M < FUSED_FFN_HSPLIT_MIN_ROWS or F % 256 != 0 or F < 512:
        return 1
    return 2


def _ffn_desc(x, w1, b1, w2, b2, R, out, f, h, act, alpha, drop, F=None):
    p = _lib.FfnT()
    p.x, p.w1, p.b1, p.w2, p.b2, p.R = ptr(x), ptr(w1), ptr(b1), ptr(w2), ptr(b2), ptr(R)
    p.out, p.f, p.h = ptr(out), ptr(f), ptr(h)
    p.M, p.D, p.F, p.act = x.shape[0], x.shape[1], (F if F is not None else w1.shape[0]), act
    p.alpha = alpha
    p.dtype = 1 if x.dtype == torch.bfloat16 else 0
    p_in, s_in, p_out, s_out = drop
    p.p_in, p.salt_in, p.p_out, p.salt_out = float(p_in), int(s_in), float(p_out), int(s_out)
    if p_in > 0.0 or p_out > 0.0:
        p.drop_step = ptr(rng_state(x.device))
    return p


def _ffn_call(name, p, keep):
    fn = getattr(_lib.lib(), name)
    if _gemm_record is not None:
        _gemm_record.append((dict(kind=name, flop=4.0 * p.M * p.D * p.F), keep, lambda sp, p=p: check(fn(C.byref(p), sp), name)))
    check(fn(C.byref(p), stream_ptr()), name)


FFN_LN_FUSED = True


def ffn_fwd(x, w1, b1, w2, b2, *, act, alpha=1.0, R=None, drop=(0.0, 0, 0.0, 0), save=True, packed=None, ln=None):
    M, D = x.shape
    F = w1.shape[0]
    dt = x.dtype
    for t_ in (x, w1, w2):
        if t_.dtype != dt or dt not in (torch.float32, torch.bfloat16) or not t_.is_contiguous():
            raise _lib.EamdError("ffn_fwd: contiguous float32 or bfloat16 operands of one dtype")
    for t_ in tuple(v for v in (b1, b2, R) if v is not None):
        if t_.dtype != torch.float32 or not t_.is_contiguous():
            raise _lib.EamdError("ffn_fwd: biases / residual are contiguous float32 tensors")
    hs = ffn_hsplit(M, F, dt == torch.bfloat16)
    out = zeros(M, D, device=x.device) if hs > 1 else torch.empty(M, D, device=x.device, dtype=torch.float32)
    f = torch.empty(M, F, device=x.device, dtype=dt) if save else None
    h = torch.empty(M, F, device=x.device, dtype=dt) if save else None
    if packed is None:
        packed = ffn_pack(w1, w2)[:2]
    p = _ffn_desc(x, packed[0], b1, packed[1], b2, R, out, f, h, act, alpha, drop, F=F)
    p.hsplit = hs
    if ln is not None:
        xr, g, b, eps, mean, rstd = ln
        for t_ in (xr, g, b, mean, rstd):
            if t_.dtype != torch.float32 or not t_.is_contiguous():
                raise _lib.EamdError("ffn_fwd: LayerNorm operands are contiguous float32 tensors")
        if tuple(xr.shape) != (M, D) or g.numel() != D or b.numel() != D or mean.numel() < M or rstd.numel() < M:
            raise _lib.EamdError("ffn_fwd: LayerNorm operand shapes")
        p.ln_x, p.ln_w, p.ln_b, p.ln_mean, p.ln_rstd, p.ln_eps = ptr(xr), ptr(g), ptr(b), ptr(mean), ptr(rstd), float(eps)
    _ffn_call("eamd_ffn_fwd", p, (x, packed, b1, b2, R, out, f, h, ln))
    return out, f, h


def ffn_pack(w1, w2):
    F, D = w1.shape
    bf = fast() or w1.dtype == torch.bfloat16
    s1, s2 = (wshadow(w1), wshadow(w2)) if w1.dtype != torch.bfloat16 else (w1, w2)
    dt = torch.bfloat16 if bf else torch.float32
    buf = getattr(w1, "_eamd_ffn_pack", None)
    if buf is None or buf.numel() != 4 * F * D or buf.device != s1.device or buf.dtype != dt:
        buf = torch.empty(4, F * D, device=s1.device, dtype=dt)
        w1._eamd_ffn_pack = buf
    elif _rp["active"] and getattr(w1, "_eamd_ffn_pack_epoch", -1) == _rp["epoch"]:
        return buf[0], buf[1], buf[2], buf[3]
    name = "eamd_ffn_pack_bf16" if bf else "eamd_ffn_pack_f32"
    check(getattr(_lib.lib(), name)(ptr(s1), ptr(s2), ptr(buf[0]), ptr(buf[1]), ptr(buf[2]), ptr(buf[3]), D, F, stream_ptr()), name)
    return buf[0], buf[1], buf[2], buf[3]


def ffn_prepack(pairs):
    if fast() or not pairs or not _rp["active"]:
        return
    arr = (_lib.FfnPackT * len(pairs))()
    n = 0
    for w1, w2 in pairs:
        F, D = w1.shape
        if D != 256 or F % 128 != 0 or F < 256 or w1.dtype != torch.float32:
            continue
        buf = getattr(w1, "_eamd_ffn_pack", None)
        if buf is None or buf.numel() != 4 * F * D or buf.device != w1.device or buf.dtype != torch.float32:
            buf = torch.empty(4, F * D, device=w1.device, dtype=torch.float32)
            w1._eamd_ffn_pack = buf
        q = arr[n]
        q.w1, q.w2, q.fwd_first, q.fwd_second, q.bwd_first, q.bwd_second = ptr(w1), ptr(w2), ptr(buf[0]), ptr(buf[1]), ptr(buf[2]), ptr(buf[3])
        q.D, q.F = D, F
        w1._eamd_ffn_pack_epoch = _rp["epoch"]
        n += 1
    if n:
        check(_lib.lib().eamd_ffn_pack_f32_multi(arr, n, stream_ptr()), "eamd_ffn_pack_f32_multi")


def ffn_bwd_lnb_ok(M, F, dt):
    return dt == torch.float32 and ffn_hsplit(M, F, False) == 1


def ffn_bwd(dy, w1, w2, f, *, alpha=1.0, packed=None, lnb=None):
    M, D = dy.shape
    F = w1.shape[0]
    dt = dy.dtype
    assert f.shape == (M, F) and f.dtype == dt and f.is_contiguous() and dy.is_contiguous()
    dz = torch.empty(M, F, device=dy.device, dtype=dt)
    hs = ffn_hsplit(M, F, dt == torch.bfloat16)
    dx = zeros(M, D, device=dy.device) if hs > 1 else torch.empty(M, D, device=dy.device, dtype=torch.float32)
    if packed is None:
        packed = ffn_pack(w1, w2)[2:]
    assert packed[0].numel() == F * D and packed[1].numel() == F * D and packed[0].dtype == dt
    p = _ffn_desc(dy, packed[0], None, packed[1], None, None, dx, f, dz, ACT_NONE, alpha, (0.0, 0, 0.0, 0), F=F)
    p.hsplit = hs
    if lnb is not None:
        xb, g, mean, rstd, dres, ws, d_out, d_ps = lnb
        p.lnb_x, p.lnb_gamma, p.lnb_mean, p.lnb_rstd, p.lnb_dres, p.lnb_ws = ptr(xb), ptr(g), ptr(mean), ptr(rstd), ptr(dres), ptr(ws)
        if d_out is not None:
            p.lnb_drop_out, p.lnb_drop_p, p.lnb_drop_salt, p.drop_step = ptr(d_out), float(d_ps[0]), int(d_ps[1]), ptr(rng_state(dy.device))
    _ffn_call("eamd_ffn_bwd", p, (dy, packed, f, dz, dx, lnb))
    return dz, dx


ROWPROJ = True
ROWPROJ_MIN_ROWS = 4096


def rowproj_ok(M, K, N):
    return (ROWPROJ and _state["precision"] == 0 and M >= ROWPROJ_MIN_ROWS and K % 256 == 0 and N % 256 == 0 and 256 <= K <= 768
            and N <= 1024)


_rp = {"epoch": 0, "active": False}
_rp_bufs = {}


def rowproj_prepack(groups):
    _rp["epoch"] += 1
    _rp["active"] = True
    flat = [job for _, jobs in groups for job in jobs]
    if not flat:
        return
    imgs = rowproj_pack(flat)
    i = 0
    for holder, jobs in groups:
        holder._eamd_rp = (_rp["epoch"], [id(w) for w, _ in jobs], imgs[i:i + len(jobs)])
        i += len(jobs)
    _rp["active"] = True


def rowproj_prepack_end():
    _rp["active"] = False


def rowproj_images(holder, jobs):
    c = getattr(holder, "_eamd_rp", None)
    if _rp["active"] and c is not None and c[0] == _rp["epoch"] and len(c[2]) == len(jobs):
        return c[2]
    return rowproj_pack(jobs)


def rowproj_pack(jobs):
    arr = (_lib.RowProjPackT * len(jobs))()
    imgs = []
    for q, (W, trans) in zip(arr, jobs):
        assert W.dim() == 2 and W.dtype == torch.float32 and W.stride(1) == 1
        K, N = (W.shape[0], W.shape[1]) if trans else (W.shape[1], W.shape[0])
        key = (W.data_ptr(), K, N, bool(trans), W.device.index)
        img = _rp_bufs.get(key)
        if img is None:
            if len(_rp_bufs) > 4096:
                _rp_bufs.clear()
            img = _rp_bufs[key] = torch.empty(K * N, device=W.device, dtype=torch.float32)
        q.w, q.image, q.K, q.N, q.ldw, q.trans = ptr(W), ptr(img), K, N, W.stride(0), bool(trans)
        imgs.append(img)
    check(_lib.lib().eamd_rowproj_pack_f32(arr, len(jobs), stream_ptr()), "eamd_rowproj_pack_f32")
    return imgs


def rowproj(a, img, N, *, bias=None, R=None, alpha=1.0, drop=None, ln=None, affine=None, lnb=None, out=None):
    M, K = a.shape
    dev = a.device
    if out is None:
        out = torch.empty(M, N, device=dev, dtype=torch.float32)
    p = _lib.RowProjT()
    p.a, p.lda, p.w, p.bias = ptr(a), a.stride(0), ptr(img), ptr(bias)
    p.R, p.ldr = ptr(R), (R.stride(0) if R is not None else 0)
    p.out, p.ldo = ptr(out), out.stride(0)
    p.M, p.K, p.N, p.alpha = M, K, N, float(alpha)
    if drop is not None and drop[0] > 0.0:
        p.p_out, p.salt_out, p.drop_step = float(drop[0]), int(drop[1]), ptr(rng_state(dev))
    if ln is not None:
        xr, g, b, eps, mean, rstd = ln
        p.ln_x, p.ln_w, p.ln_b, p.ln_mean, p.ln_rstd, p.ln_eps = ptr(xr), ptr(g), ptr(b), ptr(mean), ptr(rstd), float(eps)
    if affine is not None:
        sc, sh, act, a_out = affine
        p.a_scale, p.a_shift, p.a_act, p.a_out = ptr(sc), ptr(sh), int(act), ptr(a_out)
    if lnb is not None:
        xb, g, mean, rstd, dres, ws, d_out, d_ps = lnb
        p.lnb_x, p.lnb_gamma, p.lnb_mean, p.lnb_rstd, p.lnb_dres, p.lnb_ws = ptr(xb), ptr(g), ptr(mean), ptr(rstd), ptr(dres), ptr(ws)
        if d_out is not None:
            p.lnb_drop_out, p.lnb_drop_p, p.lnb_drop_salt, p.drop_step = ptr(d_out), float(d_ps[0]), int(d_ps[1]), ptr(rng_state(dev))
    fn = _lib.lib().eamd_rowproj
    keep = (a, img, bias, R, out, ln, affine, lnb)
    if _gemm_record is not None:
        _gemm_record.append((dict(kind="rowproj", flop=2.0 * M * K * N), keep, lambda sp, p=p: check(fn(C.byref(p), sp), "eamd_rowproj")))
    check(fn(C.byref(p), stream_ptr()), "eamd_rowproj")
    return out


def rowproj_lnb_ws(M, device):
    return torch.empty(_lib.lib().eamd_rowproj_lnb_workspace(M), device=device, dtype=torch.float32)


_wgrad = {"stream": None, "used": False}


def enable_wgrad_stream(enable=True):
    _wgrad["stream"] = torch.cuda.Stream() if enable else None
    _wgrad["used"] = False


def wgrad_group_end():
    wgrad_group_flush()
    _wgroup["on"] = False


def wgrad_join():
    wgrad_group_flush()
    st = _wgrad["stream"]
    if st is not None and _wgrad["used"]:
        torch.cuda.current_stream().wait_stream(st)
        _wgrad["used"] = False


def linear_bwd_w(dy, x, dW, *, alpha=1.0, b_act=ACT_NONE, db=None, group=True):
    st = _wgrad["stream"]
    if st is None:
        return _linear_bwd_w(dy, x, dW, alpha=alpha, b_act=b_act, db=db, group=group)
    cur = torch.cuda.current_stream()
    st.wait_stream(cur)
    with torch.cuda.stream(st):
        _linear_bwd_w(dy, x, dW, alpha=alpha, b_act=b_act, db=db)
    dy.record_stream(st)
    x.record_stream(st)
    _wgrad["used"] = True


def _linear_bwd_w(dy, x, dW, *, alpha=1.0, b_act=ACT_NONE, db=None, group=True):
    M, N = dy.shape
    K = x.shape[1]
    assert x.shape[0] == M and dW.numel() == N * K and dW.dtype == torch.float32
    grouping = group and _wgroup["on"] and _wgrad["stream"] is None
    if (grouping and M <= STACK_WGRAD_MAX_ROWS and alpha == 1.0 and b_act == ACT_NONE
            and dy.is_contiguous() and x.is_contiguous() and _in_grad_arena(dW)):
        key = (dW.data_ptr(), db.data_ptr() if db is not None else 0, dy.dtype, x.dtype, N, K)
        _wgroup["stack"].setdefault(key, (dW, db, [], []))
        ent = _wgroup["stack"][key]
        ent[2].append(dy)
        ent[3].append(x)
        return
    sk = auto_splitk(N, K, M)
    tile = 0
    t64 = ((N + 63) // 64) * ((K + 63) // 64)
    if grouping and t64 <= GROUP_WGRAD_MAX_TILES and _in_grad_arena(dW):
        if t64 >= GROUP_WGRAD_TILE128_MIN and N >= 128 and K >= 128 and dy.dtype == torch.float32 and _state["precision"] == 0:
            tile = 128
            sk = max(1, min(GROUP_WGRAD_T128_WGS // (((N + 127) // 128) * ((K + 127) // 128)), M // 256))
        else:
            tile = 64
            sk = max(1, sk // GROUP_WGRAD_SK_DIV)
    gemm(dy, x, dW, N, K, M, N, K, K, transA=1, transB=1, alpha=alpha, b_act=b_act, splitk=sk, tile=tile,
         beta=1.0 if sk == 1 else 0.0, colsum=db, group=grouping)


def colsum(x, out, scale=1.0, rows=None, D=None, ld=None):
    rows = x.shape[0] if rows is None else rows
    D = x.shape[1] if D is None else D
    ld = D if ld is None else ld
    assert out.numel() >= D
    check(_lib.lib().eamd_colsum(ptr(x), ld, ptr(out), rows, D, scale,
                                 1 if x.dtype == torch.bfloat16 else 0, stream_ptr()), "eamd_colsum")


def layernorm_fwd(x, gamma, beta, eps, out_dtype=torch.float32):
    rows, D = x.shape
    y = torch.empty(rows, D, device=x.device, dtype=out_dtype)
    mean = torch.empty(rows, device=x.device, dtype=torch.float32)
    rstd = torch.empty(rows, device=x.device, dtype=torch.float32)
    y32, y16 = (ptr(y), None) if out_dtype == torch.float32 else (None, ptr(y))
    check(_lib.lib().eamd_layernorm_fwd(ptr(x), ptr(gamma), ptr(beta), y32, y16, ptr(mean), ptr(rstd), rows, D,
                                        eps, stream_ptr()), "eamd_layernorm_fwd")
    return y, mean, rstd


class _LnReduceJob(C.Structure):
    _fields_ = [("ws", C.c_void_p), ("dgamma", C.c_void_p), ("dbeta", C.c_void_p), ("nblk", C.c_int32), ("D", C.c_int32)]


defer_ln_reduce = True
_ln_pending = []
_ln_task = -1


def flush_ln_reduce():
    global _ln_pending, _ln_task
    jobs, _ln_pending, _ln_task = _ln_pending, [], -1
    if not jobs:
        return
    tab = (_LnReduceJob * len(jobs))()
    for i, (ws, dg, db, nblk, D) in enumerate(jobs):
        tab[i].ws, tab[i].dgamma, tab[i].dbeta, tab[i].nblk, tab[i].D = ws.data_ptr(), dg.data_ptr(), db.data_ptr(), nblk, D
    with torch.cuda.device(jobs[0][0].device):
        check(_lib.lib().eamd_layernorm_bwd_reduce(tab, len(jobs), stream_ptr()), "eamd_layernorm_bwd_reduce")


def ln_partials_reduce(ws, dgamma, dbeta, nblk, D):
    if _defer_ln(ws, dgamma, dbeta, nblk, D):
        return
    tab = (_LnReduceJob * 1)()
    tab[0].ws, tab[0].dgamma, tab[0].dbeta, tab[0].nblk, tab[0].D = ws.data_ptr(), dgamma.data_ptr(), dbeta.data_ptr(), nblk, D
    check(_lib.lib().eamd_layernorm_bwd_reduce(tab, 1, stream_ptr()), "eamd_layernorm_bwd_reduce")


def _defer_ln(ws, dgamma, dbeta, nblk, D):
    global _ln_pending, _ln_task
    if not defer_ln_reduce or not (getattr(dgamma, "_eamd_arena", False) and getattr(dbeta, "_eamd_arena", False)):
        return False
    task = torch._C._current_graph_task_id()
    if task < 0:
        return False
    if task != _ln_task:
        _ln_pending = []
        torch.autograd.Variable._execution_engine.queue_callback(flush_ln_reduce)
        _ln_task = task
    _ln_pending.append((ws, dgamma, dbeta, nblk, D))
    return True


def layernorm_bwd(dy, x, gamma, mean, rstd, dres, dgamma, dbeta, drop=None):
    rows, D = x.shape
    assert dy.shape == x.shape and dgamma.numel() == D and dbeta.numel() == D
    dx = torch.empty_like(x)
    L = _lib.lib()
    nws = L.eamd_layernorm_bwd_workspace(rows, D)
    ws = torch.empty(nws, device=x.device, dtype=torch.float32)
    pg, pb = ptr(dgamma), ptr(dbeta)
    if _defer_ln(ws, dgamma, dbeta, nws // (2 * D), D):
        pg = pb = None
    if drop is not None:
        dx16 = torch.empty(rows, D, device=x.device, dtype=act_dtype())
        fn, name = ((L.eamd_layernorm_bwd_drop, "eamd_layernorm_bwd_drop") if fast()
                    else (L.eamd_layernorm_bwd_drop_f32, "eamd_layernorm_bwd_drop_f32"))
        check(fn(ptr(dy), ptr(x), ptr(gamma), ptr(mean), ptr(rstd), ptr(dres), ptr(dx), ptr(dx16),
                 drop[0], ptr(rng_state(x.device)), drop[1], pg,
                 pb, ptr(ws), rows, D, stream_ptr()), name)
        return dx, dx16
    check(L.eamd_layernorm_bwd(ptr(dy), ptr(x), ptr(gamma), ptr(mean), ptr(rstd), ptr(dres), ptr(dx),
                               pg, pb, ptr(ws), rows, D, stream_ptr()), "eamd_layernorm_bwd")
    return dx


F32_FUSED_ATTN = True


def attn_fwd_supported(T1, T2, dk, rel):
    if dk != 64 or (rel and T1 != T2):
        return False
    return (fast() or F32_FUSED_ATTN) and T2 <= 4096


def attn_fwd(qu, qv, k, v, pos, mask, B, T1, T2, H, dk, ldp, scale, drop=None, shift_len=None):
    dev = qu[0].device
    dt = qu[0].dtype
    D = H * dk
    mb = mi = 0
    if mask is not None:
        assert mask.dtype == torch.uint8 and mask.is_contiguous() and mask.dim() == 3 and mask.shape[0] in (1, B)
        assert mask.shape[2] == T2 and mask.shape[1] in (1, T1)
        mb = 0 if mask.shape[0] == 1 else mask.shape[1] * mask.shape[2]
        mi = 0 if mask.shape[1] == 1 else T2
    assert dt in (torch.bfloat16, torch.float32)
    for t_, _, _ in (qu, k, v) + ((qv,) if qv is not None else ()):
        assert t_.dtype == dt and t_.is_cuda
    assert pos is None or (pos[0].dtype == dt and pos[2] >= D)
    P = torch.empty(H * B * T1 * ldp, device=dev, dtype=dt)
    cx = torch.empty(B * T1, D, device=dev, dtype=dt)
    dropping = drop is not None and drop[0] > 0.0
    Pd = torch.empty_like(P) if dropping else P
    dargs = ((ptr(Pd), drop[0], ptr(rng_state(dev)), drop[1]) if dropping
             else (None, 0.0, None, 0))
    args = (ptr(qu[0], qu[1]), qu[2], ptr(qv[0], qv[1]) if qv is not None else None, qv[2] if qv is not None else 0,
            ptr(k[0], k[1]), k[2], ptr(v[0], v[1]), v[2], ptr(pos[0], pos[1]) if pos is not None else None,
            pos[2] if pos is not None else 0,
            ptr(mask), mb, mi, ptr(P), ldp, ptr(cx), D, B, H, T1, T2, dk, scale) + dargs
    args = args + (ptr(shift_len) if (pos is not None and T1 == T2) else None,)
    name = "eamd_attn_fwd" if dt == torch.bfloat16 else "eamd_attn_fwd_f32"
    fn = getattr(_lib.lib(), name)
    rc = fn(*args, stream_ptr())
    if rc == _lib.EAMD_EUNSUPPORTED:
        return None
    check(rc, name)
    if _gemm_record is not None:
        _gemm_record.append((dict(kind=name, flop=0.0), (qu, qv, k, v, pos, mask, P, Pd, cx), lambda sp, args=args: check(fn(*args, sp), name)))
    return P, Pd, cx


def attn_bwd_q(dctx, k, v, P, dS, dbd, dq, B, T1, T2, H, dk, ldp, scale, drop=None, shift_len=None):
    dropping = drop is not None and drop[0] > 0.0
    dargs = ((drop[0], ptr(rng_state(P.device)), drop[1]) if dropping
             else (0.0, None, 0))
    if P.dtype == torch.bfloat16:
        name = "eamd_attn_bwd_q"
        args = (ptr(dctx[0], dctx[1]), dctx[2], ptr(k[0], k[1]), k[2], ptr(v[0], v[1]), v[2], ptr(P), ldp,
                ptr(dS), ptr(dbd), ptr(dq[0], dq[1]), dq[2], dq[0].dtype == torch.bfloat16, B, H, T1, T2, dk,
                scale) + dargs
    else:
        name = "eamd_attn_bwd_q_f32"
        for t_ in (dctx[0], k[0], v[0], P, dS, dq[0]) + ((dbd,) if dbd is not None else ()):
            assert t_.dtype == torch.float32
        args = (ptr(dctx[0], dctx[1]), dctx[2], ptr(k[0], k[1]), k[2], ptr(v[0], v[1]), v[2], ptr(P), ldp,
                ptr(dS), ptr(dbd), ptr(dq[0], dq[1]), dq[2], B, H, T1, T2, dk, scale) + dargs
    args = args + (ptr(shift_len) if (dbd is not None and T1 == T2) else None,)
    fn = getattr(_lib.lib(), name)
    rc = fn(*args, stream_ptr())
    if rc == _lib.EAMD_EUNSUPPORTED:
        return False
    check(rc, name)
    if _gemm_record is not None:
        _gemm_record.append((dict(kind=name, flop=0.0), (dctx, k, v, P, dS, dbd, dq), lambda sp, args=args: check(fn(*args, sp), name)))
    return True


FUSED_ATTN_KV = True


def attn_bwd_kv(Pd, dS, dbd, dctx, qu, qv, dv, dk_, dpos, B, T1, T2, H, dk, ldp):
    dt = Pd.dtype
    assert dt in (torch.float32, torch.bfloat16)
    for t_ in (Pd, dS, dctx[0], qu[0], dv[0], dk_[0]):
        assert t_.dtype == dt and t_.is_cuda
    assert dv[2] == dk_[2]
    rel = dbd is not None
    if dt == torch.float32:
        args = (ptr(Pd), ptr(dS), ptr(dbd) if rel else None, ldp, ptr(dctx[0], dctx[1]), dctx[2], ptr(qu[0], qu[1]),
                qu[2], ptr(qv[0], qv[1]) if rel else None, qv[2] if rel else 0, ptr(dv[0], dv[1]), ptr(dk_[0], dk_[1]),
                dv[2], ptr(dpos[0], dpos[1]) if rel else None, dpos[2] if rel else 0, B, H, T1, T2, dk)
        name = "eamd_attn_bwd_kv_f32"
    else:
        assert not rel, "the bf16 key-side launch leaves the positional product to the GEMM"
        args = (ptr(Pd), ptr(dS), ldp, ptr(dctx[0], dctx[1]), dctx[2], ptr(qu[0], qu[1]), qu[2],
                ptr(dv[0], dv[1]), ptr(dk_[0], dk_[1]), dv[2], B, H, T1, T2, dk)
        name = "eamd_attn_bwd_kv"
    fn = getattr(_lib.lib(), name)
    rc = fn(*args, stream_ptr())
    if rc == _lib.EAMD_EUNSUPPORTED:
        return False
    check(rc, name)
    if _gemm_record is not None:
        _gemm_record.append((dict(kind=name, flop=0.0), (Pd, dS, dbd, dctx, qu, qv, dv, dk_, dpos),
                             lambda sp, args=args: check(fn(*args, sp), name)))
    return True


def softmax_fwd(ac, bd, mask, P, nblocks, B, T1, T2, ld, scale):
    mb = mi = 0
    if mask is not None:
        assert mask.dtype == torch.uint8 and mask.is_contiguous() and mask.dim() == 3 and mask.shape[0] in (1, B)
        assert mask.shape[2] == T2 and mask.shape[1] in (1, T1)
        mb = 0 if mask.shape[0] == 1 else mask.shape[1] * mask.shape[2]
        mi = 0 if mask.shape[1] == 1 else T2
    assert ac.numel() >= nblocks * T1 * ld and P.numel() >= nblocks * T1 * ld
    p32, p16 = (ptr(P), None) if P.dtype == torch.float32 else (None, ptr(P))
    check(_lib.lib().eamd_softmax_fwd(ptr(ac), ptr(bd), ptr(mask), mb, mi, p32, p16, nblocks,
                                      B, T1, T2, ld, scale, stream_ptr()),
          "eamd_softmax_fwd")


def softmax_bwd(P, dP, dbd, nblocks, T1, T2, ld, scale, dS16=None):
    assert P.numel() >= nblocks * T1 * ld and dP.numel() >= nblocks * T1 * ld and dP.dtype == torch.float32
    if P.dtype == torch.bfloat16:
        assert dS16 is not None and dS16.dtype == torch.bfloat16 and (dbd is None or dbd.dtype == torch.bfloat16)
        check(_lib.lib().eamd_softmax_bwd(None, ptr(P), ptr(dP), None, ptr(dS16), ptr(dbd), nblocks, T1, T2,
                                          ld, scale, stream_ptr()), "eamd_softmax_bwd")
    else:
        check(_lib.lib().eamd_softmax_bwd(ptr(P), None, ptr(dP), ptr(dbd), None, None, nblocks, T1, T2,
                                          ld, scale, stream_ptr()), "eamd_softmax_bwd")


def lsm_loss(logits, target, smoothing, inv_denom, ignore_id, want_grad=True):
    rows, V = logits.shape
    assert target.numel() == rows and target.dtype == torch.int64
    loss_rows = torch.empty(rows, device=logits.device, dtype=torch.float32)
    correct = torch.empty(rows, device=logits.device, dtype=torch.float32)
    grad = torch.empty_like(logits) if want_grad else None
    check(_lib.lib().eamd_lsm_loss(ptr(logits), ptr(target), ptr(loss_rows), ptr(correct), ptr(grad), rows, V,
                                   ignore_id, smoothing, inv_denom, stream_ptr()),
          "eamd_lsm_loss")
    return loss_rows, correct, grad


def argmax_rows(x):
    rows, V = x.shape
    out = torch.empty(rows, device=x.device, dtype=torch.int32)
    check(_lib.lib().eamd_argmax_rows(ptr(x), V, ptr(out), rows, V, stream_ptr()), "eamd_argmax_rows")
    return out


def reduce_sum(x, scale=1.0):
    out = torch.empty((), device=x.device, dtype=torch.float32)
# ... 1691 lines not shown
```

include/espnet_amd.h:

```cpp
#ifndef ESPNET_AMD_H_
#define ESPNET_AMD_H_
#include <stdint.h>
#ifdef __cplusplus
extern "C" {
#endif

int eamd_abi_version(void);

typedef struct {
  int32_t enabled;
  int32_t C;
  int32_t ntap;
  int32_t Ho, Wo;
  int32_t Hin, Win;
  int32_t sh, sw;
  int32_t dh[9], dw[9];
} eamd_gather_t;

typedef struct {
  int32_t enabled;
  int32_t Ho, Wo;
  int32_t Hc, Wc;
  int32_t sh, oh, sw, ow;
} eamd_rowmap_t;

typedef struct {
  const float* A; const float* B; float* C;
  const float* bias; const float* aux; const float* R;
  float* colsum;
  int32_t M, N, K;
  int32_t transA, transB;
  int64_t lda, ldb, ldc, ldaux, ldr;
  int32_t batch1, batch2;
  int64_t sA1, sA2, sB1, sB2, sC1, sC2;
  float alpha, beta;
  int32_t a_act, b_act, epilogue;
  int32_t splitk;
  int32_t precision;
  int32_t tile;
  eamd_gather_t gather;
  eamd_rowmap_t cmap;
  void* Cb;
  int32_t in_dtype;
  int32_t aux_dtype;
  float drop_p;
  uint64_t drop_salt;
  const uint64_t* drop_step;
  void* Hb;
  int32_t h_act;
  int32_t h_dtype;
  struct {
    float* part; const int32_t* col; float* zcol; float* zfix; int32_t fix; int32_t reserved;
    const float* rowc; const float* gscale; float scale; int32_t reserved2;
  } stats;
} eamd_gemm_t;

int eamd_gemm(const eamd_gemm_t* p, void* stream);

#define EAMD_GEMM_MULTI_MAX 4
int eamd_gemm_multi(const eamd_gemm_t* descs, int n, void* stream);

int eamd_conv2_bwd_x_conv1_bwd_w(const eamd_gemm_t* descs, int n, const float* x, int T, int F, float* part, float* dw,
                                 float* db, void* stream);

int eamd_gemm_group_plan(const eamd_gemm_t* descs, int n, int32_t* first);
int eamd_gemm_group_launch(const eamd_gemm_t* descs_dev, const int32_t* first_dev, int n, int total, int in_dtype, int tile,
                           void* stream);

typedef struct {
  const float* x; const float* w1; const float* b1; const float* w2; const float* b2; const float* R;
  float* out; float* f; float* h;
  int32_t M, D, F, act;
  float alpha;
  float p_in; uint64_t salt_in; float p_out; uint64_t salt_out; const void* drop_step;
  int32_t dtype;
  int32_t hsplit;
  const float* ln_x; const float* ln_w; const float* ln_b; float* ln_mean; float* ln_rstd;
  float ln_eps; int32_t reserved2;
  const float* lnb_x; const float* lnb_gamma; const float* lnb_mean; const float* lnb_rstd; const float* lnb_dres;
  float* lnb_ws; float* lnb_drop_out; uint64_t lnb_drop_salt; float lnb_drop_p; int32_t reserved3;
} eamd_ffn_t;
int eamd_ffn_fwd(const eamd_ffn_t* p, void* stream);
int eamd_ffn_bwd(const eamd_ffn_t* p, void* stream);
typedef struct {
  const float* w1; const float* w2;
  float* fwd_first; float* fwd_second; float* bwd_first; float* bwd_second;
  int32_t D, F;
} eamd_ffn_pack_t;
int eamd_ffn_pack_f32_multi(const eamd_ffn_pack_t* jobs, int njobs, void* stream);

typedef struct {
  const float* a; int64_t lda;
  const float* w; const float* bias;
  const float* R; int64_t ldr;
  float* out; int64_t ldo;
  int32_t M, K, N, a_act;
  float alpha; float p_out; uint64_t salt_out; const void* drop_step;
  const float* ln_x; const float* ln_w; const float* ln_b; float* ln_mean; float* ln_rstd; float ln_eps; float lnb_drop_p;
  const float* a_scale; const float* a_shift; float* a_out;
  const float* lnb_x; const float* lnb_gamma; const float* lnb_mean; const float* lnb_rstd; const float* lnb_dres;
  float* lnb_ws; float* lnb_drop_out; uint64_t lnb_drop_salt;
} eamd_rowproj_t;
typedef struct {
  const float* w; float* image;
  int32_t K, N, ldw, trans;
} eamd_rowproj_pack_t;
int eamd_rowproj(const eamd_rowproj_t* p, void* stream);
int eamd_rowproj_pack_f32(const eamd_rowproj_pack_t* jobs, int njobs, void* stream);
int64_t eamd_rowproj_lnb_workspace(int M);
int eamd_ffn_pack_f32(const float* w1, const float* w2, float* fwd_first, float* fwd_second, float* bwd_first, float* bwd_second,
                      int D, int F, void* stream);
int eamd_ffn_pack_bf16(const void* w1, const void* w2, void* fwd_first, void* fwd_second, void* bwd_first, void* bwd_second,
                       int D, int F, void* stream);

int eamd_layernorm_fwd(const float* x, const float* gamma, const float* beta, float* y, void* y_bf16, float* mean,
                       float* rstd, int rows, int D, float eps, void* stream);
int64_t eamd_layernorm_bwd_workspace(int rows, int D);
typedef struct {
  const float* ws; float* dgamma; float* dbeta;
  int32_t nblk, D;
} eamd_ln_reduce_job_t;
int eamd_layernorm_bwd_reduce(const eamd_ln_reduce_job_t* jobs, int njobs, void* stream);
int eamd_layernorm_bwd(const float* dy, const float* x, const float* gamma, const float* mean,
                       const float* rstd, const float* dres, float* dx, float* dgamma, float* dbeta,
                       float* workspace, int rows, int D, void* stream);
int eamd_layernorm_bwd_drop(const float* dy, const float* x, const float* gamma, const float* mean, const float* rstd,
                            const float* dres, float* dx, void* dx_drop_bf16, float drop_p, const uint64_t* step_dev,
                            uint64_t salt, float* dgamma, float* dbeta, float* workspace, int rows, int D, void* stream);
int eamd_layernorm_bwd_drop_f32(const float* dy, const float* x, const float* gamma, const float* mean, const float* rstd,
                                const float* dres, float* dx, float* dx_drop, float drop_p, const uint64_t* step_dev,
                                uint64_t salt, float* dgamma, float* dbeta, float* workspace, int rows, int D, void* stream);

int eamd_softmax_fwd(const float* ac, const float* bd, const unsigned char* mask, int64_t mask_bstride,
                     int64_t mask_qstride, float* P, void* P_bf16, int nblocks, int B, int T1, int T2, int64_t ld,
                     float scale, void* stream);
int eamd_softmax_bwd(const float* P, const void* P_bf16, float* dP, float* dbd, void* dS_bf16, void* dbd_bf16,
                     int nblocks, int T1, int T2, int64_t ld, float scale, void* stream);

int eamd_attn_fwd(const void* qu, int64_t ldq, const void* qv, int64_t ldqv, const void* k, int64_t ldk, const void* v,
                  int64_t ldv, const void* pos, int64_t ldpos, const unsigned char* mask, int64_t mask_bstride,
                  int64_t mask_qstride, void* P_bf16, int64_t ldp, void* ctx_bf16, int64_t ldc, int B, int H, int T1,
                  int T2, int dk, float scale, void* Pd_bf16, float drop_p, const uint64_t* drop_step, uint64_t drop_salt,
                  const int32_t* shift_len, void* stream);

int eamd_attn_bwd_q(const void* dctx, int64_t ldd, const void* k, int64_t ldk, const void* v, int64_t ldv,
                    const void* P_bf16, int64_t ldp, void* dS_bf16, void* dbd_bf16, void* dq, int64_t ldo, int dq_is_bf16,
                    int B, int H, int T1, int T2, int dk, float scale, float drop_p, const uint64_t* drop_step,
                    uint64_t drop_salt, const int32_t* shift_len, void* stream);

int eamd_attn_fwd_f32(const float* qu, int64_t ldq, const float* qv, int64_t ldqv, const float* k, int64_t ldk,
                      const float* v, int64_t ldv, const float* pos, int64_t ldpos, const unsigned char* mask,
                      int64_t mask_bstride, int64_t mask_qstride, float* P, int64_t ldp, float* ctx, int64_t ldc, int B,
                      int H, int T1, int T2, int dk, float scale, float* Pd, float drop_p, const uint64_t* drop_step,
                      uint64_t drop_salt, const int32_t* shift_len, void* stream);
int eamd_attn_bwd_q_f32(const float* dctx, int64_t ldd, const float* k, int64_t ldk, const float* v, int64_t ldv,
                        const float* P, int64_t ldp, float* dS, float* dbd, float* dq, int64_t ldo, int B, int H, int T1,
                        int T2, int dk, float scale, float drop_p, const uint64_t* drop_step, uint64_t drop_salt,
                        const int32_t* shift_len, void* stream);

int eamd_attn_bwd_kv_f32(const float* Pd, const float* dS, const float* dbd, int64_t ldp, const float* dctx, int64_t ldd,
                         const float* qu, int64_t ldq, const float* qv, int64_t ldqv, float* dv, float* dk_out, int64_t ldo,
                         float* dpos, int64_t ldpos, int B, int H, int T1, int T2, int dk, void* stream);

int eamd_attn_bwd_kv(const void* Pd_bf16, const void* dS_bf16, int64_t ldp, const void* dctx, int64_t ldd, const void* qu,
                     int64_t ldq, void* dv, void* dk_out, int64_t ldo, int B, int H, int T1, int T2, int dk, void* stream);

int eamd_lsm_loss(const float* logits, const int64_t* target, float* loss_rows, float* correct_rows,
                  float* grad, int rows, int V, int ignore_id, float smoothing, float inv_denom,
                  void* stream);
int eamd_argmax_rows(const float* x, int64_t ld, int32_t* out, int rows, int V, void* stream);
int eamd_reduce_sum(const float* in, int64_t n, float* out, float scale, void* stream);
int eamd_log_softmax_rows(const float* x, float* y, int rows, int V, void* stream);
int eamd_transducer_expand_rows(const float* logits, int64_t ld, int n, int V, int k, const float* lm, const int32_t* lm_row,
                                const int32_t* pairs, int g, float* rec, float* pair_out, void* stream);
int eamd_beam_finish(const float* top_s, const int64_t* top_i, int n, int beam, int V, int W, int L, int step, int eos,
                     const int64_t* maxlen, int ns, int nf, const float* sc_in, const float* const* logps, const float* c_local,
                     int64_t ldc, int full_mode, const int64_t* ids, int ncand, const int64_t* yseq_in, float* sc_out,
                     int64_t* yseq_out, float* hyp_out, int64_t* hyp_i, int64_t* tok_i, int64_t* pos, float* rec, void* stream);
int eamd_linear_rows_f32(const float* x, const float* W, const float* bias, const float* R, float* y, int M, int N, int K,
                         int a_act, int act, float alpha, int64_t ldx, int64_t ldr, void* stream);
int eamd_linear_rows_ln_f32(const float* x, const float* gamma, const float* beta, float eps, const float* W, const float* bias,
                            const float* R, float* y, int M, int N, int K, int act, float alpha, int64_t ldx, int64_t ldr,
                            int64_t ldy, void* stream);
int eamd_decode_self_attn_dyn(const float* qkv, int64_t ldq, float* kcache, float* vcache, const int32_t* slot_at, int Lcap, int pos,
                              const int32_t* pos_dev, int n, int H, int D, float* ctx, void* stream);
int eamd_beam_slots_dyn(const int32_t* slot_in, int32_t* slot_out, const int64_t* hyp, int n, int Lcap, int pos, const int32_t* pos_dev,
                        void* stream);
int eamd_decode_src_attn(const float* q, int64_t ldq, const float* kmem, const float* vmem, int64_t ldkv, const uint8_t* mask, int nutt,
                         int g, int T, int H, int D, float* ctx, void* stream);
int eamd_decode_src_attn_group(const float* q, int64_t ldq, const float* kmem, const float* vmem, int64_t ldkv, const uint8_t* mask, int nutt,
                         int g, int T, int H, int D, float* ctx, void* stream);
int64_t eamd_decode_src_attn_split_workspace(int nutt, int g, int H, int splits);
int eamd_decode_src_attn_split(const float* q, int64_t ldq, const float* kmem, const float* vmem, int64_t ldkv, const uint8_t* mask,
                               int nutt, int g, int T, int H, int D, int splits, float* ws, float* ctx, void* stream);
int eamd_weighted_sum(const float* const* logps, const float* weights, int nf, int64_t numel, float* out, void* stream);
int eamd_beam_select(const float* pre, const int64_t* ids, const float* psi, const float* c_s, const float* hyp, float w_ctc,
                     int nutt, int beam, int P, int V, float* c_local, float* top_s, int64_t* top_i, void* stream);
int eamd_topk_rows_i32(const float* x, int64_t ld, int rows, int n, int k, float* vals, int64_t* idx, int32_t* idx32, void* stream);
int eamd_copy_jobs(const void* const* src, void* const* dst, const int64_t* nbytes, int njobs, void* stream);
int eamd_weighted_topk_rows(const float* const* logps, const float* weights, int nf, int rows, int n, int k, int extra, float* pre,
                            float* vals, int64_t* idx, int32_t* idx32, void* stream);
int eamd_beam_step_dyn(const float* pre, const int64_t* ids, const float* psi, const float* c_s, const float* hyp, float w_ctc, int nutt,
                       int beam, int P, int V, int W, int L, int step, int eos, const int64_t* maxlen, int ns, int nf, const float* sc_in,
                       const float* const* logps, const int64_t* yseq_in, float* c_local, float* sc_out, int64_t* yseq_out, float* hyp_out,
                       int64_t* hyp_i, int64_t* tok_i, int32_t* tok32, float* cs_out, float* rec, const int32_t* step_dev, int32_t* step_out,
                       int ring, const int32_t* slot_in, int32_t* slot_out, int Lcap, void* stream);

int eamd_axpby(const float* x, const float* y, float* out, int64_t n, float a, float b, void* stream);
int eamd_cast_bf16(const float* x, void* y_bf16, int64_t n, void* stream);
int eamd_scale_dev(const float* x, const float* scale_dev, float* out, int64_t n, float extra, void* stream);
int eamd_act_fwd(const float* x, float* y, int64_t n, int act, void* stream);
int eamd_act_bwd(const float* dy, const float* x, float* dx, int64_t n, int act, void* stream);
int eamd_glu_fwd(const float* x, float* y, int64_t rows, int C, void* stream);
int eamd_glu_bwd(const float* dy, const float* x, float* dx, void* dx_bf16, int64_t rows, int C, void* stream);
int eamd_add_bias2(const void* q, int64_t ldq, const float* u, const float* v, void* qu, void* qv, int64_t rows, int D,
                   int bf16, void* stream);
int eamd_add_cast_bf16(const float* a, const float* b, void* out_bf16, int64_t rows, int cols, int64_t ld_out,
                       void* stream);
int eamd_add_block_f32(const float* a, const float* b, float* out, int64_t rows, int cols, int64_t ld_out, void* stream);
int eamd_add_cast_colsum2(const float* a, const float* b, void* out_bf16, int64_t ld_out, float* suma, float* sumb,
                          int64_t rows, int D, void* stream);
int eamd_add_colsum2_f32(const float* a, const float* b, float* out, int64_t ld_out, float* suma, float* sumb, int64_t rows,
                         int D, void* stream);
int eamd_colsum(const void* x, int64_t ld, float* out, int64_t rows, int D, float scale, int x_bf16, void* stream);
int eamd_embed_pe_dyn(const int64_t* tok, int64_t ldt, const float* table, const float* pe, float* out, int64_t rows, int U, int D,
                      float scale, int pos_offset, const int32_t* pos_dev, void* stream);
int eamd_embed_bwd(const int64_t* tok, const float* dout, float* dtable, int64_t rows, int D, float scale,
                   int64_t pad_idx, void* stream);
int eamd_posenc(const float* x, const float* pe, float* out, int64_t rows, int T, int D, float scale,
                void* stream);
int eamd_posenc_scaled(const float* x, const float* pe, const float* alpha, float* out, int64_t rows, int T, int D,
                       float scale, void* stream);
int eamd_posenc_scaled_bwd(const float* dout, const float* pe, float* dalpha, int64_t rows, int T, int D,
                           void* stream);
int eamd_permute4(const float* src, float* dst, int d0, int d1, int d2, int d3, int64_t s0, int64_t s1,
                  int64_t s2, int64_t s3, int accumulate, void* stream);
int eamd_dropout(const void* x, void* y, int64_t n, float p, const uint64_t* step_dev, uint64_t salt, int act,
                 int in_bf16, int out_bf16, void* stream);
int eamd_rng_advance(uint64_t* step_dev, void* stream);

int eamd_dwconv_fwd(const float* x, const float* w, const float* bias, float* y, int B, int T, int C, int K,
                    void* stream);
int eamd_dwconv_bwd_x(const float* dy, const float* w, float* dx, int B, int T, int C, int K, void* stream);
int eamd_dwconv_bwd_w(const float* dy, const float* x, float* dw, float* db, int B, int T, int C, int K,
                      void* stream);
int eamd_dwconv_glu_fwd(const float* a, const float* w, const float* bias, float* y, float* bn_part, int B, int T, int C, int K,
                        void* stream);
int eamd_dwconv_glu_bwd_x(const float* dy, const float* w, const float* a, void* da, int da_bf16, int B, int T, int C, int K,
                          void* stream);
int eamd_dwconv_glu_bwd_w(const float* dy, const float* a, float* dw, float* db, int B, int T, int C, int K, void* stream);
int eamd_bn_nslab(int64_t M, int C);
int eamd_bn_stats(const float* x, float* workspace, float* mean, float* rstd, float* running_mean,
                  float* running_var, int64_t* num_batches_tracked, int64_t M, int C, float eps, float momentum, void* stream);
int eamd_bn_finalize(const float* part, int nslab, float* mean, float* rstd, float* running_mean, float* running_var,
                     int64_t* num_batches_tracked, int C, float eps, float momentum, void* stream);
int eamd_bn_apply(const float* x, const float* mean, const float* rstd, const float* gamma, const float* beta,
                  void* y, int64_t M, int C, int act, int y_bf16, void* stream);
int eamd_bn_stats_bounded(const float* x, float* workspace, float* mean, float* rstd, float* running_mean,
                          float* running_var, int64_t* num_batches_tracked, int64_t M, int C, float eps, float momentum, int T,
                          const int32_t* bound, void* stream);
int eamd_bn_bwd_bounded(const float* dy, const float* x, const float* mean, const float* rstd, const float* gamma,
                        const float* beta, float* workspace, float* dx, float* dgamma, float* dbeta, int64_t M, int C,
                        int act, int training, int T, const int32_t* bound, void* stream);
int eamd_mask_time(void* x, int64_t rows, int C, int T, const int32_t* bound, int is_bf16, void* stream);
int eamd_bn_bwd(const float* dy, const float* x, const float* mean, const float* rstd, const float* gamma,
                const float* beta, float* workspace, float* dx, float* dgamma, float* dbeta, int64_t M, int C,
                int act, int training, void* stream);
int eamd_conv1_fwd(const float* x, const float* w, const float* bias, void* y, int B, int T, int F, int C,
                   int y_bf16, void* stream);
int64_t eamd_conv1_bwd_w_workspace(int B, int T, int C);
int eamd_conv1_bwd_w(const void* dy, const float* x, float* dw, float* db, float* workspace, int B, int T, int F,
                     int C, int dy_bf16, void* stream);

int64_t eamd_ctc_workspace_bytes(int B, int T, int Lmax);
int eamd_ctc_loss(const float* acts, int64_t stride_t, int64_t stride_b, const int64_t* ys_pad,
                  const int32_t* ilens, float* nll, float* grad, int64_t gstride_t, int64_t gstride_b,
                  void* workspace, int B, int T, int V, int Lmax, int blank, int ignore_id, float grad_scale,
                  void* stream);
int eamd_ctc_grad(const float* acts, int64_t stride_t, int64_t stride_b, const int32_t* ilens, const float* nll, float* grad,
                  int64_t gstride_t, int64_t gstride_b, const void* workspace, int B, int T, int V, int Lmax, int blank,
                  float grad_scale, const float* gscale_dev, void* stream);

int64_t eamd_ctc_pit_workspace_bytes(int S, int B, int T, int Lmax);
int eamd_ctc_pit_loss(const float* acts, const int64_t* ys_pad, const int32_t* ilens, float* nll_pair, int64_t* perm, float* pit,
                      float* grad, void* workspace, int S, int B, int T, int V, int Lmax, int blank, int ignore_id, float grad_scale,
                      void* stream);

int64_t eamd_ctc_align_workspace_bytes(int B, int T, int Lmax);
int eamd_ctc_forced_align(const float* acts, int64_t stride_t, int64_t stride_b, const int64_t* ys_pad, const int32_t* ilens,
                          float* score, int32_t* states, int64_t* tokens, int32_t* seg_start, int32_t* seg_end, void* workspace,
                          int B, int T, int V, int Lmax, int blank, int ignore_id, int normalized, void* stream);

int eamd_ctc_prefix_score(const float* logp, const float* r_prev, const int32_t* cand, const int32_t* last,
                          const int32_t* olen, float* psi, float* r_new, int nhyp, int ncand, int T, int V,
                          int blank, int eos, void* stream);

int eamd_ctc_prefix_score_batch(const float* logp, const int32_t* lens, int nutt, int per_utt, const float* r_prev,
                                const int32_t* cand, const int32_t* last, const int32_t* olen, float* psi, float* r_new,
                                int ncand, int Tmax, int V, int blank, int eos, void* stream);
int eamd_ctc_prefix_psi_dyn(const float* logp, const int32_t* lens, int nutt, int per_utt, const float* r_prev, const int32_t* cand,
                            const int32_t* last, int olen, const int32_t* olen_dev, float* psi, int ncand, int Tmax, int V, int blank,
                            int eos, void* stream);
int eamd_ctc_prefix_state_dyn(const float* logp, const int32_t* lens, int nutt, int per_utt, const float* r_prev, const int64_t* parent,
                              const int64_t* tok, const int32_t* last, int olen, const int32_t* olen_dev, const float* alive, float* r_out,
                              int Tmax, int V, int blank, void* stream);

int eamd_specaug(const float* x, float* y, const int32_t* lens, const int32_t* center, const int32_t* warped,
                 const int32_t* fpos, const int32_t* flen, int nf, const int32_t* tpos, const int32_t* tlen, int nt, int B,
                 int T, int F, void* stream);
int eamd_global_mvn(const float* x, float* y, const int32_t* lens, const float* mean, const float* stdv, int B, int T,
                    int F, void* stream);
int eamd_utterance_mvn(const float* x, float* y, const int32_t* lens, float* workspace, int norm_means, int norm_vars,
                       float eps, int B, int T, int F, void* stream);

int eamd_reflect_pad(const float* x, int64_t ldx, float* y, int64_t ldy, int B, int L, int pad, void* stream);
int eamd_logmel(const float* spec, int64_t ld, int64_t rows_per_utt, const float* melmat, const int32_t* lo,
                const int32_t* hi, const int32_t* flens, float* out, int B, int T, int F, int M, float log_scale,
                int power_input, void* stream);

int eamd_ft_logmel_fwd(const float* spec, const float* melmat, const int32_t* lo, const int32_t* hi, const int32_t* lens,
                       float* out, int B, int T, int F, int M, void* stream);
int eamd_ft_logmel_bwd(const float* spec, const float* g, const float* melmat, const int32_t* lo, const int32_t* hi,
                       const int32_t* mlo, const int32_t* mhi, const int32_t* lens, float* gspec, int B, int T, int F, int M,
                       void* stream);
int eamd_ft_mvn_fwd(const float* x, float* y, const int32_t* lens, const float* bias, const float* scale, float* workspace,
                    int apply_utt, int norm_means, int norm_vars, float eps, int B, int T, int M, void* stream);
int eamd_ft_mvn_bwd(const float* gy, float* gx, const int32_t* lens, const float* scale, float* workspace, int apply_utt,
                    int B, int T, int M, void* stream);

int eamd_lstm_cell_fwd(const float* gates, const float* c_prev, const float* h_prev, const uint8_t* live, float* h,
                       float* c, float* y, float* acts, int B, int H, void* stream);
int eamd_lstm_cell_bwd(const float* dy, const float* dh, const float* dc, const float* acts, const float* c_prev,
                       const float* c, const uint8_t* live, float* dgates, float* dc_prev, float* dh_pass, int B, int H,
                       void* stream);
int eamd_lstm_step_fwd(const float* gx, const float* w_hh, const float* b_hh, const float* h_prev, const float* c_prev,
                       const uint8_t* live, float* h, float* c, float* y, float* acts, int B, int H, void* stream);
int eamd_lstm_step_bwd(const float* dy, const float* dgates_next, const float* w_t, const float* dh_pass_in, const float* dc,
                       const float* acts, const float* c_prev, const float* c, const uint8_t* live, float* dgates,
                       float* dc_prev, float* dh_pass, int B, int H, void* stream);
typedef struct {
  const float* gx;
  const float* w_hh;
  const float* b_hh;
  const uint8_t* live;
  float* h_out;
  float* c_out;
  float* y;
  float* acts;
  int32_t reverse;
  int32_t reserved;
} eamd_lstm_seq_fwd_t;
typedef struct {
  const float* dy;
  const float* w_t;
  const float* acts;
  const float* c_out;
  const uint8_t* live;
  float* dgates;
  int32_t reverse;
  int32_t reserved;
} eamd_lstm_seq_bwd_t;
int64_t eamd_lstm_seq_sync_bytes(void);
int eamd_lstm_seq_fwd(const eamd_lstm_seq_fwd_t* jobs, int njobs, int T, int B, int H, void* sync_ws, void* stream);
int eamd_lstm_seq_bwd(const eamd_lstm_seq_bwd_t* jobs, int njobs, int T, int B, int H, void* sync_ws, void* stream);
int eamd_lstm_seq_status(const void* sync_ws, void* stream);
int eamd_lstm_seq_status_merge(const void* sync_ws, void* sticky, void* stream);
int eamd_gru_cell_fwd(const float* gx, const float* gh, const float* h_prev, const uint8_t* live, float* h, float* y,
                      float* acts, int B, int H, void* stream);
int eamd_gru_cell_bwd(const float* dy, const float* dh, const float* acts, const float* h_prev, const uint8_t* live,
                      float* dgx, float* dgh, float* dh_direct, int B, int H, void* stream);
int eamd_maxpool2x2_fwd(const float* x, float* y, uint8_t* idx, int B, int H, int W, int C, void* stream);
int eamd_maxpool2x2_bwd(const float* dy, const uint8_t* idx, float* dx, int B, int H, int W, int C, void* stream);
int eamd_mask_rows(const float* x, const uint8_t* keep, float* y, int64_t rows, int D, void* stream);
int eamd_unfold1d(const void* x, void* col, int B, int T, int C, int k, int bf16, void* stream);
int eamd_fold1d(const float* dcol, float* dx, int B, int T, int C, int k, void* stream);
int eamd_conv3x3_c1_fwd(const float* x, const float* w, const float* bias, void* y, int B, int T, int F, int C,
                        int y_bf16, void* stream);
int64_t eamd_conv3x3_c1_bwd_w_workspace(int B, int T, int C);
int eamd_conv3x3_c1_bwd_w(const void* dy, const float* x, float* dw, float* db, float* workspace, int B, int T, int F,
                          int C, int dy_bf16, void* stream);
int eamd_conv3x3_c1_bwd_x(const void* dy, const float* w, float* dx, int B, int T, int F, int C, int dy_bf16, void* stream);
int eamd_attloc_fwd(const float* att_prev, const float* conv_w, const float* w_att, const float* pre_enc,
                    const float* dec_proj, const float* gvec, const float* gb, const int32_t* lens, const float* enc_h,
                    float scaling, float* e, float* th, float* conv, float* w, float* ctx, int B, int T, int A, int C,
                    int K, int R, int E, void* stream);
int eamd_attloc_bwd_energy(const float* dctx, const float* dw_ext, const float* w, const float* enc_h, const float* th,
                           const float* gvec, float scaling, float* de, float* d_enc_h, float* df, float* dgvec,
                           float* dgb, float* d_dec_proj, int B, int T, int A, int E, void* stream);
int64_t eamd_attloc_bwd_workspace(int B, int T, int A, int C);
int eamd_attloc_bwd_energy_conv(const float* dctx, const float* dw_ext, const float* w, const float* enc_h, const float* th,
                                const float* gvec, float scaling, const float* conv, const float* w_att, float* de,
                                float* d_enc_h, float* df, float* dconv, float* dgvec, float* dgb, float* d_dec_proj,
                                float* dw_att, float* workspace, int accumulate, int B, int T, int A, int C, int E,
                                void* stream);
int eamd_att_dot_energy_fwd(const float* k, const float* q, const int32_t* lens, float* e, int B, int T, int A,
                            void* stream);
int eamd_att_dot_energy_bwd(const float* de, const float* k, const float* q, float* dk, float* dq, int B, int T, int A,
                            void* stream);
int eamd_att_ctx_fwd(const float* e, const float* v, float scaling, float* w, float* ctx, int B, int T, int E,
                     void* stream);
int eamd_att_ctx_bwd(const float* dctx, const float* dw_ext, const float* w, const float* v, float scaling, float* de,
                     float* d_v, float* dsum, int B, int T, int E, void* stream);
int eamd_attloc_bwd_conv(const float* dconv, const float* conv_w, const float* att_prev, float* d_prev, float* dconv_w,
                         int B, int T, int C, int K, int R, void* stream);
int eamd_attloc_convmax_fwd(const float* att_prev, const float* conv_w, float* pooled, int32_t* idx, int B, int T, int C,
                            int K, void* stream);
int eamd_attloc_convmax_bwd(const float* dpool, const float* pooled, const int32_t* idx, const float* att_prev,
                            const float* conv_w, float* d_prev, float* dconv_w, int B, int T, int C, int K, void* stream);

int eamd_joint_fwd(const float* enc, const float* dec, float* out, void* out_bf16, int B, int T, int U, int J, int act,
                   void* stream);
int eamd_joint_bwd(const float* dh, const float* enc, const float* dec, float* d_enc, float* d_dec, int B, int T, int U,
// ... 100 lines not shown
```

Measured before the change: 1.144 million frames/s.

## Fuse rel-pos bias add, dq colsum, and BN apply into rowproj kernels

Adds an extension struct to the row-projection kernel, enabling three fusions. The QKV projection writes q+pos_bias_u and q+pos_bias_v directly, replacing a separate add_bias2 kernel. In the backward LN path the kernel sums dqu+dqv while staging and emits per-block column partials, replacing add_cast_colsum2. The conv module's BatchNorm+activation is applied while staging the pointwise conv input instead of in a separate bn_apply kernel. Decoder FFN weights are also prepacked together with the encoder's in one batched pack launch. The cost is extra shared memory, more kernel specializations and more code complexity.

```diff
diff --git a/espnet_amd/_lib.py b/espnet_amd/_lib.py
--- a/espnet_amd/_lib.py
+++ b/espnet_amd/_lib.py
@@ -73,6 +73,14 @@
                 ("a_scale", C.c_void_p), ("a_shift", C.c_void_p), ("a_out", C.c_void_p),
                 ("lnb_x", C.c_void_p), ("lnb_gamma", C.c_void_p), ("lnb_mean", C.c_void_p), ("lnb_rstd", C.c_void_p),
                 ("lnb_dres", C.c_void_p), ("lnb_ws", C.c_void_p), ("lnb_drop_out", C.c_void_p), ("lnb_drop_salt", C.c_uint64)]
+
+
+class RowProjExtT(C.Structure):
+    _fields_ = [("bias_u", C.c_void_p), ("bias_v", C.c_void_p), ("out_u", C.c_void_p), ("out_v", C.c_void_p), ("ld_uv", C.c_int64),
+                ("a1", C.c_void_p), ("lda1", C.c_int64), ("a2", C.c_void_p), ("lda2", C.c_int64), ("a_sum_out", C.c_void_p),
+                ("ld_sum", C.c_int64), ("colsum_ws", C.c_void_p),
+                ("bn_mean", C.c_void_p), ("bn_rstd", C.c_void_p), ("bn_gamma", C.c_void_p), ("bn_beta", C.c_void_p),
+                ("a_out", C.c_void_p), ("bn_act", C.c_int32), ("reserved", C.c_int32)]
 
 
 class FfnPackT(C.Structure):
diff --git a/espnet_amd/csrc/rowproj_f32.hip b/espnet_amd/csrc/rowproj_f32.hip
--- a/espnet_amd/csrc/rowproj_f32.hip
+++ b/espnet_amd/csrc/rowproj_f32.hip
@@ -14,6 +14,8 @@
 constexpr int TL_LD = 264;
 
 __device__ __forceinline__ int xs_ld(int K) { return K + 8; }
+constexpr int SUM_RED = 8 * 2 * 256;
+__host__ __device__ __forceinline__ int sum_red_off(int K) { return RBM * (K + 8); }
 
 __device__ __forceinline__ void stage_ln(const eamd_rowproj_t& p, const int m0, const int t, float* xs, const int LD) {
   constexpr int D = 256;
@@ -70,9 +72,59 @@
   }
 }
 
-template <bool LNB>
-__global__ __launch_bounds__(RNT, 2) void rowproj_f32_kernel(const eamd_rowproj_t p) {
+__device__ __forceinline__ void stage_bn(const eamd_rowproj_t& p, const eamd_rowproj_ext_t& x, const int m0, const int t, float* xs,
+                                         const int LD) {
+  const int c4 = t & 63;
+  const float4 mu = *reinterpret_cast<const float4*>(x.bn_mean + c4 * 4), rs = *reinterpret_cast<const float4*>(x.bn_rstd + c4 * 4);
+  const float4 ga = *reinterpret_cast<const float4*>(x.bn_gamma + c4 * 4), be = *reinterpret_cast<const float4*>(x.bn_beta + c4 * 4);
+#pragma unroll
+  for (int i = 0; i < 4; ++i) {
+    const int row = (t >> 6) + 8 * i;
+    const long gr = (long)min(m0 + row, p.M - 1);
+    const float4 v = *reinterpret_cast<const float4*>(p.a + gr * p.lda + c4 * 4);
+    float4 o;
+    o.x = eamd_act((v.x - mu.x) * rs.x * ga.x + be.x, x.bn_act); o.y = eamd_act((v.y - mu.y) * rs.y * ga.y + be.y, x.bn_act);
+    o.z = eamd_act((v.z - mu.z) * rs.z * ga.z + be.z, x.bn_act); o.w = eamd_act((v.w - mu.w) * rs.w * ga.w + be.w, x.bn_act);
+    *reinterpret_cast<float4*>(&xs[row * LD + c4 * 4]) = o;
+    if (x.a_out && m0 + row < p.M) *reinterpret_cast<float4*>(x.a_out + gr * 256 + c4 * 4) = o;
+  }
+}
+
+__device__ __forceinline__ void stage_sum(const eamd_rowproj_t& p, const eamd_rowproj_ext_t& x, const int m0, const int t, float* xs,
+                                          const int LD, float* red) {
+  const int c4 = t & 63, rg = t >> 6;
+  float4 sa = make_float4(0.f, 0.f, 0.f, 0.f), sb = sa;
+#pragma unroll
+  for (int i = 0; i < 4; ++i) {
+    const int row = rg + 8 * i;
+    const long gr = (long)min(m0 + row, p.M - 1);
+    const float4 u = *reinterpret_cast<const float4*>(x.a1 + gr * x.lda1 + c4 * 4);
+    const float4 v = *reinterpret_cast<const float4*>(x.a2 + gr * x.lda2 + c4 * 4);
+    const float4 o = make_float4(u.x + v.x, u.y + v.y, u.z + v.z, u.w + v.w);
+    *reinterpret_cast<float4*>(&xs[row * LD + c4 * 4]) = o;
+    if (m0 + row < p.M) {
+      *reinterpret_cast<float4*>(x.a_sum_out + gr * x.ld_sum + c4 * 4) = o;
+      sa.x += u.x; sa.y += u.y; sa.z += u.z; sa.w += u.w;
+      sb.x += v.x; sb.y += v.y; sb.z += v.z; sb.w += v.w;
+    }
+  }
+  *reinterpret_cast<float4*>(&red[(rg * 2 + 0) * 256 + c4 * 4]) = sa;
+  *reinterpret_cast<float4*>(&red[(rg * 2 + 1) * 256 + c4 * 4]) = sb;
+  const int c4n = (p.K - 256) >> 2;
+  for (int idx = t; idx < RBM * c4n; idx += RNT) {
+    const int row = idx / c4n, c = idx - row * c4n;
+    *reinterpret_cast<f32x4*>(&xs[row * LD + 256 + c * 4]) =
+        *reinterpret_cast<const f32x4*>(p.a + (long)min(m0 + row, p.M - 1) * p.lda + 256 + c * 4);
+  }
+}
+
+template <bool EXT> struct RpArgs { eamd_rowproj_t p; };
+template <> struct RpArgs<true> { eamd_rowproj_t p; eamd_rowproj_ext_t x; };
+
+template <bool LNB, bool EXT>
+__global__ __launch_bounds__(RNT, 2) void rowproj_f32_kernel(const RpArgs<EXT> args) {
   extern __shared__ __attribute__((aligned(16))) float sm[];
+  const eamd_rowproj_t& p = args.p;
   const int K = p.K, N = p.N;
   const int LD = xs_ld(K);
   float* const xs = sm;
@@ -85,7 +137,15 @@
   const int nsteps = S * nchunk;
   float* const st = sm + RBM * LD + wave * ST_SZ;
 
-  if (p.ln_x) {
+  bool ext_staged = false;
+  if constexpr (EXT && !LNB) {
+    if (args.x.bn_mean) { stage_bn(p, args.x, m0, t, xs, LD); ext_staged = true; }
+  }
+  if constexpr (EXT && LNB) {
+    if (args.x.a2) { stage_sum(p, args.x, m0, t, xs, LD, sm + sum_red_off(K)); ext_staged = true; }
+  }
+  if (ext_staged) {
+  } else if (p.ln_x) {
     stage_ln(p, m0, t, xs, LD);
   } else if (p.a_scale) {
     stage_affine(p, m0, t, xs, LD);
@@ -143,6 +203,15 @@
   load_b(std::integral_constant<int, 1>{}, 1);
   load_b(std::integral_constant<int, 2>{}, 2);
   __syncthreads();
+  if constexpr (EXT && LNB) {
+    if (args.x.a2) {
+      const float* red = sm + sum_red_off(K) + t;
+      float s = 0.f;
+#pragma unroll
+      for (int w = 0; w < 8; ++w) s += red[w * 512];
+      args.x.colsum_ws[(long)blockIdx.x * 512 + t] = s;
+    }
+  }
   read_a(0, I0{});
 
   const unsigned thr_out = eamd_drop_thr16(p.p_out);
@@ -175,6 +244,28 @@
       const int col0 = c * RCH + wave * 32 + (lane & 7) * 4;
       float4 b4 = make_float4(0.f, 0.f, 0.f, 0.f);
       if (p.bias) b4 = *reinterpret_cast<const float4*>(p.bias + col0);
+      bool dual = false;
+      if constexpr (EXT) {
+        dual = args.x.out_u != nullptr && c == 0;
+        if (dual) {
+#pragma unroll 1
+          for (int o = 0; o < 2; ++o) {
+            const float4 e4 = *reinterpret_cast<const float4*>((o ? args.x.bias_v : args.x.bias_u) + col0);
+            float* const dst = o ? args.x.out_v : args.x.out_u;
+#pragma unroll 1
+            for (int it = 0; it < 4; ++it) {
+              const int lr = it * 8 + (lane >> 3);
+              const int row = m0 + lr;
+              const float4 a4 = *reinterpret_cast<const float4*>(&st[lr * ST_LD + (lane & 7) * 4]);
+              if (row < p.M)
+                *reinterpret_cast<float4*>(dst + (long)row * args.x.ld_uv + col0) =
+                    make_float4(((a4.x + b4.x) * p.alpha + 0.f) + e4.x, ((a4.y + b4.y) * p.alpha + 0.f) + e4.y,
+                                ((a4.z + b4.z) * p.alpha + 0.f) + e4.z, ((a4.w + b4.w) * p.alpha + 0.f) + e4.w);
+            }
+          }
+        }
+      }
+      if (!dual)
 #pragma unroll
       for (int it = 0; it < 4; ++it) {
         const int lr = it * 8 + (lane >> 3);
@@ -218,8 +309,9 @@
 }
 
 struct PackJob { const float* w; float* img; int K, N, ldw, trans; long npiece; };
-constexpr int PACK_JOBS = 48;
+constexpr int PACK_JOBS = 96;
 struct PackTable { PackJob j[PACK_JOBS]; };
+static_assert(sizeof(PackTable) <= 4096, "the job table travels in the kernel arguments");
 __global__ __launch_bounds__(256) void rowproj_pack_kernel(const PackTable tab) {
   const PackJob jb = tab.j[blockIdx.y];
   for (long piece = (long)blockIdx.x * 256 + threadIdx.x; piece < jb.npiece; piece += (long)gridDim.x * 256) {
@@ -242,8 +334,9 @@
 
 bool al16(const void* q) { return (reinterpret_cast<uintptr_t>(q) & 15) == 0; }
 
-size_t smem_bytes(int K, bool lnb) {
+size_t smem_bytes(int K, bool lnb, bool sum = false) {
   size_t rows = (size_t)RBM * (K + 8);
+  if (sum) rows += SUM_RED;
   if (lnb) {
     const size_t need = (size_t)RBM * TL_LD + 2 * (size_t)RBM * 256;
     return (rows > need ? rows : need) * sizeof(float);
@@ -277,18 +370,44 @@
   return EAMD_OK;
 }
 
-template <bool LNB>
-int launch_rowproj(const eamd_rowproj_t& p, hipStream_t stream) {
-  const size_t smem = smem_bytes(p.K, LNB);
+template <bool LNB, bool EXT>
+int launch_rowproj(const RpArgs<EXT>& args, hipStream_t stream) {
+  const eamd_rowproj_t& p = args.p;
+  const size_t smem = smem_bytes(p.K, LNB, LNB && EXT);
   static int attr_done = 0;
   if (!attr_done) {
-    const hipError_t e = hipFuncSetAttribute(reinterpret_cast<const void*>(&rowproj_f32_kernel<LNB>),
-                                             hipFuncAttributeMaxDynamicSharedMemorySize, (int)smem_bytes(768, LNB));
+    const hipError_t e = hipFuncSetAttribute(reinterpret_cast<const void*>(&rowproj_f32_kernel<LNB, EXT>),
+                                             hipFuncAttributeMaxDynamicSharedMemorySize, (int)smem_bytes(768, LNB, LNB && EXT));
     if (e != hipSuccess) return (int)e;
     attr_done = 1;
   }
-  hipLaunchKernelGGL((rowproj_f32_kernel<LNB>), dim3((p.M + RBM - 1) / RBM), dim3(RNT), smem, stream, p);
+  hipLaunchKernelGGL((rowproj_f32_kernel<LNB, EXT>), dim3((p.M + RBM - 1) / RBM), dim3(RNT), smem, stream, args);
   EAMD_LAUNCH_CHECK();
+  return EAMD_OK;
+}
+
+int check_rowproj_ext(const eamd_rowproj_t* p, const eamd_rowproj_ext_t* x) {
+  if (x->bias_u || x->bias_v || x->out_u || x->out_v) {
+    if (!x->bias_u || !x->bias_v || !x->out_u || !x->out_v || x->ld_uv < RCH) return EAMD_EINVAL;
+    if (p->p_out != 0.f || p->R || p->alpha != 1.f || p->lnb_x) return EAMD_EINVAL;
+    if (p->N < 2 * RCH) return EAMD_EUNSUPPORTED;
+    if (x->ld_uv % 4 != 0 || !al16(x->bias_u) || !al16(x->bias_v) || !al16(x->out_u) || !al16(x->out_v)) return EAMD_EUNSUPPORTED;
+  }
+  if (x->a1 || x->a2 || x->a_sum_out || x->colsum_ws) {
+    if (!x->a1 || !x->a2 || !x->a_sum_out || !x->colsum_ws) return EAMD_EINVAL;
+    if (x->lda1 < 256 || x->lda2 < 256 || x->ld_sum < 256 || p->ln_x || p->a_scale || x->bn_mean) return EAMD_EINVAL;
+    if (!p->lnb_x) return EAMD_EUNSUPPORTED;
+    if (x->lda1 % 4 != 0 || x->lda2 % 4 != 0 || x->ld_sum % 4 != 0 || !al16(x->a1) || !al16(x->a2) || !al16(x->a_sum_out))
+      return EAMD_EUNSUPPORTED;
+  }
+  if (x->bn_mean || x->bn_rstd || x->bn_gamma || x->bn_beta) {
+    if (!x->bn_mean || !x->bn_rstd || !x->bn_gamma || !x->bn_beta || p->ln_x || p->a_scale) return EAMD_EINVAL;
+    if (p->K != 256 || p->lnb_x) return EAMD_EUNSUPPORTED;
+    if (!al16(x->bn_mean) || !al16(x->bn_rstd) || !al16(x->bn_gamma) || !al16(x->bn_beta) || (x->a_out && !al16(x->a_out)))
+      return EAMD_EUNSUPPORTED;
+  } else if (x->a_out) {
+    return EAMD_EINVAL;
+  }
   return EAMD_OK;
 }
 
@@ -299,7 +418,19 @@
 extern "C" int eamd_rowproj(const eamd_rowproj_t* p, void* stream) {
   const int rc = check_rowproj(p);
   if (rc != EAMD_OK) return rc;
-  return p->lnb_x ? launch_rowproj<true>(*p, (hipStream_t)stream) : launch_rowproj<false>(*p, (hipStream_t)stream);
+  const RpArgs<false> args{*p};
+  return p->lnb_x ? launch_rowproj<true, false>(args, (hipStream_t)stream) : launch_rowproj<false, false>(args, (hipStream_t)stream);
+}
+
+extern "C" int eamd_rowproj_ext(const eamd_rowproj_t* p, const eamd_rowproj_ext_t* x, void* stream) {
+  int rc = check_rowproj(p);
+  if (rc != EAMD_OK) return rc;
+  if (!x) return EAMD_EINVAL;
+  rc = check_rowproj_ext(p, x);
+  if (rc != EAMD_OK) return rc;
+  if (!x->out_u && !x->a2 && !x->bn_mean) return eamd_rowproj(p, stream);
+  const RpArgs<true> args{*p, *x};
+  return p->lnb_x ? launch_rowproj<true, true>(args, (hipStream_t)stream) : launch_rowproj<false, true>(args, (hipStream_t)stream);
 }
 
 extern "C" int eamd_rowproj_pack_f32(const eamd_rowproj_pack_t* jobs, int njobs, void* stream) {
diff --git a/espnet_amd/functional.py b/espnet_amd/functional.py
--- a/espnet_amd/functional.py
+++ b/espnet_amd/functional.py
@@ -77,12 +77,18 @@
     return ops.layernorm_bwd(dxn, x2, ln_w, mean, rstd, do, gbuf, bbuf).view(shp)
 
 
-def _rp_ln_bwd(dy, img, x2, ln_w, mean, rstd, do, gbuf, bbuf, prev, shp):
+def _rp_ln_bwd(dy, img, x2, ln_w, mean, rstd, do, gbuf, bbuf, prev, shp, dq_sum=None):
     M, D = x2.shape
     ws = ops.rowproj_lnb_ws(M, x2.device)
     dcopy = torch.empty(M, D, device=x2.device, dtype=torch.float32) if prev is not None else None
-    dx = ops.rowproj(dy, img, D, lnb=(x2, ln_w, mean, rstd, do, ws, dcopy, prev))
+    ext = cws = None
+    if dq_sum is not None:
+        cws = torch.empty(((M + 31) // 32) * 512, device=x2.device, dtype=torch.float32)
+        ext = dict(asum=(dq_sum[0], dq_sum[1], (dy, 0, dy.stride(0)), cws))
+    dx = ops.rowproj(dy, img, D, lnb=(x2, ln_w, mean, rstd, do, ws, dcopy, prev), ext=ext)
     ops.ln_partials_reduce(ws, gbuf, bbuf, (M + 31) // 32, D)
+    if dq_sum is not None:
+        ops.ln_partials_reduce(cws, dq_sum[2], dq_sum[3], (M + 31) // 32, 256)
     out = dx.view(shp)
     if prev is not None:
         out._eamd_dropped = (dcopy, prev)
@@ -535,6 +541,9 @@
 
 
 FUSE_QKV = True
+FUSE_REL_BIAS = True
+FUSE_DQ_SUM = True
+FUSE_BN_STAGE = True
 
 
 def _adjacent3(a, b, c):
@@ -687,8 +696,14 @@
             T1 = 1
         else:
             xq, res, T1 = xn, (x2 if eps is not None else None), T1f
+        quv_rp = None
         if rp is not None:
-            qkv = ops.rowproj(xn, rp[0], 3 * D, bias=_span3(bq, (3 * D,)), ln=(x2, ln_w, ln_b, eps, mean, rstd))
+            if rel and FUSE_REL_BIAS:
+                quv_rp = (torch.empty_like(x2), torch.empty_like(x2))
+                qkv = ops.rowproj(xn, rp[0], 3 * D, bias=_span3(bq, (3 * D,)), ln=(x2, ln_w, ln_b, eps, mean, rstd),
+                                  ext=dict(dual=(params[11].reshape(-1), params[12].reshape(-1), quv_rp[0], quv_rp[1])))
+            else:
+                qkv = ops.rowproj(xn, rp[0], 3 * D, bias=_span3(bq, (3 * D,)), ln=(x2, ln_w, ln_b, eps, mean, rstd))
             q, k, v = _MV(qkv, 0, 3 * D), _MV(qkv, D, 3 * D), _MV(qkv, 2 * D, 3 * D)
         elif fused:
             w3, b3 = _span3(ops.wshadow(wq), (3 * D, D)), _span3(bq, (3 * D,))
@@ -711,7 +726,9 @@
             else:
                 pos2 = ops.to_act_shared(pos_emb).reshape(-1, D)
                 p = ops.linear_fwd(pos2, ops.wshadow(wpos), None, out_dtype=adt)
-            if fused:
+            if quv_rp is not None:
+                qu, qv = quv_rp
+            elif fused:
                 qu, qv = ops.add_bias2(qkv, pu.reshape(-1), pv.reshape(-1), rows=B * T1, D=D, ldq=3 * D, q_off=0)
             else:
                 qu, qv = ops.add_bias2(q, pu.reshape(-1), pv.reshape(-1))
@@ -808,12 +825,20 @@
             dqu, dqv, _, _, dp = attn_core_bwd(dctx, P, quv, qv, _MV(qkv, D, 3 * D), _MV(qkv, 2 * D, 3 * D), p, B, T1,
                                                T2, H, dk, Pd=Pd, attn_drop=(p_att, s_att), dqkv=dqkv, dp_out=dp_out,
                                                shift_len=ctx.shift_len)
+            dq_sum = None
             if rel:
                 wpos = params[10]
-                ops.add_cast_colsum2(dqu, dqv, sink.buf(11).view(-1), sink.buf(12).view(-1), out=dqkv, out_off=0,
-                                     ld_out=3 * D)
+                if rp is not None and FUSE_DQ_SUM and dqu is not None and dqkv.dtype == torch.float32:
+                    dq_sum = (dqu, dqv, sink.buf(11), sink.buf(12))
+                else:
+                    ops.add_cast_colsum2(dqu, dqv, sink.buf(11).view(-1), sink.buf(12).view(-1), out=dqkv, out_off=0,
+                                         ld_out=3 * D)
                 if dp_out is None:
                     ops.linear_bwd_w(ops.to_act(dp), pos2, sink.buf(10))
+            if dq_sum is not None:
+                dx = _rp_ln_bwd(dqkv, rp[1], x2, ln_w, mean, rstd, do, sink.buf(0), sink.buf(1), ctx.prev, (B, T1, D), dq_sum=dq_sum)
+                ops.linear_bwd_w(dqkv, xn, _span3(sink.buf(2), (3 * D, D)), db=_span3(sink.buf(3), (3 * D,)))
+                return (dx, None, None, None, None, None, None, None, None, None) + sink.results()
             ops.linear_bwd_w(dqkv, xn, _span3(sink.buf(2), (3 * D, D)), db=_span3(sink.buf(3), (3 * D,)))
             if rp is not None:
                 dx = _rp_ln_bwd(dqkv, rp[1], x2, ln_w, mean, rstd, do, sink.buf(0), sink.buf(1), ctx.prev, (B, T1, D))
@@ -906,9 +931,13 @@
             bmean = running_mean
             brstd = ops.axpby(running_var, None, 1.0, 0.0)
             brstd = torch.rsqrt_(brstd.add_(bn_eps))
-        e = ops.bn_apply(d, bmean, brstd, g, be, M, Cc, act, adt)
+        bn_stage = rp is not None and FUSE_BN_STAGE and training and bound is None and d.dtype == torch.float32
+        e = torch.empty(M, Cc, device=x2.device, dtype=torch.float32) if bn_stage else ops.bn_apply(d, bmean, brstd, g, be, M, Cc, act, adt)
         ctx.rp = rp
-        if rp is not None:
+        if bn_stage:
+            out = ops.rowproj(d.view(M, Cc), rp[2], Cc, bias=b2, R=x2, drop=(p_out, s_out) if p_out > 0.0 else None,
+                              ext=dict(bn=(bmean, brstd, g, be, act, e)))
+        elif rp is not None:
             out = ops.rowproj(e, rp[2], Cc, bias=b2, R=x2, drop=(p_out, s_out) if p_out > 0.0 else None)
         elif p_out > 0.0 and (ops.fast() or ops.f32_epilogue_drop()):
             out = ops.linear_fwd(e, ops.wshadow(w2).view(Cc, Cc), b2, R=x2, drop=(p_out, s_out))
diff --git a/espnet_amd/nets/e2e_asr_transformer.py b/espnet_amd/nets/e2e_asr_transformer.py
--- a/espnet_amd/nets/e2e_asr_transformer.py
+++ b/espnet_amd/nets/e2e_asr_transformer.py
@@ -197,6 +197,17 @@
     def forward_core(self, batch):
         xs_pad = batch["xs_pad"]
         ops.set_time_bound(batch.get("tbound"))
+        if self.decoder is not None:
+            Md = batch["ys_in_pad"].numel()
+            ops.ffn_prepack_also([(m.feed_forward.w_1.weight, m.feed_forward.w_2.weight) for m in self.decoder.decoders
+                                  if hasattr(getattr(m.feed_forward, "w_1", None), "weight") and ops.FUSED_FFN
+                                  and (Md >= ops.FUSED_FFN_MIN_ROWS or ops.ffn_hsplit(Md, m.feed_forward.w_1.weight.shape[0], False) > 1)])
+        try:
+            return self._forward_core(batch, xs_pad)
+        finally:
+            ops.ffn_prepack_release()
+
+    def _forward_core(self, batch, xs_pad):
         try:
             hs_pad, hs_mask = self.encoder(xs_pad, batch["src_mask"])
         finally:
diff --git a/espnet_amd/ops.py b/espnet_amd/ops.py
--- a/espnet_amd/ops.py
+++ b/espnet_amd/ops.py
@@ -614,7 +614,7 @@
     if buf is None or buf.numel() != 4 * F * D or buf.device != s1.device or buf.dtype != dt:
         buf = torch.empty(4, F * D, device=s1.device, dtype=dt)
         w1._eamd_ffn_pack = buf
-    elif _rp["active"] and getattr(w1, "_eamd_ffn_pack_epoch", -1) == _rp["epoch"]:
+    elif (_rp["active"] or _rp["ffn_hold"] == _rp["epoch"]) and getattr(w1, "_eamd_ffn_pack_epoch", -1) == _rp["epoch"]:
         return buf[0], buf[1], buf[2], buf[3]
     name = "eamd_ffn_pack_bf16" if bf else "eamd_ffn_pack_f32"
     check(getattr(_lib.lib(), name)(ptr(s1), ptr(s2), ptr(buf[0]), ptr(buf[1]), ptr(buf[2]), ptr(buf[3]), D, F, stream_ptr()), name)
@@ -622,8 +622,13 @@
 
 
 def ffn_prepack(pairs):
+    more = list(_ffn_more)
+    del _ffn_more[:]
+    pairs = list(pairs) + more
     if fast() or not pairs or not _rp["active"]:
         return
+    if more:
+        _rp["ffn_hold"] = _rp["epoch"]
     arr = (_lib.FfnPackT * len(pairs))()
     n = 0
     for w1, w2 in pairs:
@@ -641,6 +646,18 @@
         n += 1
     if n:
         check(_lib.lib().eamd_ffn_pack_f32_multi(arr, n, stream_ptr()), "eamd_ffn_pack_f32_multi")
+
+
+_ffn_more = []
+
+
+def ffn_prepack_also(pairs):
+    _ffn_more[:] = list(pairs)
+
+
+def ffn_prepack_release():
+    del _ffn_more[:]
+    _rp["ffn_hold"] = -1
 
 
 def ffn_bwd_lnb_ok(M, F, dt):
@@ -678,7 +695,7 @@
             and N <= 1024)
 
 
-_rp = {"epoch": 0, "active": False}
+_rp = {"epoch": 0, "active": False, "ffn_hold": -1}
 _rp_bufs = {}
 
 
@@ -725,7 +742,7 @@
     return imgs
 
 
-def rowproj(a, img, N, *, bias=None, R=None, alpha=1.0, drop=None, ln=None, affine=None, lnb=None, out=None):
+def rowproj(a, img, N, *, bias=None, R=None, alpha=1.0, drop=None, ln=None, affine=None, lnb=None, out=None, ext=None):
     M, K = a.shape
     dev = a.device
     if out is None:
@@ -748,11 +765,30 @@
         p.lnb_x, p.lnb_gamma, p.lnb_mean, p.lnb_rstd, p.lnb_dres, p.lnb_ws = ptr(xb), ptr(g), ptr(mean), ptr(rstd), ptr(dres), ptr(ws)
         if d_out is not None:
             p.lnb_drop_out, p.lnb_drop_p, p.lnb_drop_salt, p.drop_step = ptr(d_out), float(d_ps[0]), int(d_ps[1]), ptr(rng_state(dev))
-    fn = _lib.lib().eamd_rowproj
-    keep = (a, img, bias, R, out, ln, affine, lnb)
+    keep = (a, img, bias, R, out, ln, affine, lnb, ext)
+    if ext is not None:
+        x = _lib.RowProjExtT()
+        if ext.get("dual") is not None:
+            bu, bv, ou, ov = ext["dual"]
+            assert bu.numel() == 256 and bv.numel() == 256 and ou.shape == (M, 256) and ov.shape == (M, 256) and ou.stride(0) == ov.stride(0)
+            x.bias_u, x.bias_v, x.out_u, x.out_v, x.ld_uv = ptr(bu), ptr(bv), ptr(ou), ptr(ov), ou.stride(0)
+        if ext.get("asum") is not None:
+            a1, a2, (so, so_off, so_ld), cws = ext["asum"]
+            assert a1.shape == (M, 256) and a2.shape == (M, 256) and cws.numel() >= ((M + 31) // 32) * 512
+            assert so.numel() >= so_off + (M - 1) * so_ld + 256
+            x.a1, x.lda1, x.a2, x.lda2 = ptr(a1), a1.stride(0), ptr(a2), a2.stride(0)
+            x.a_sum_out, x.ld_sum, x.colsum_ws = ptr(so, so_off), so_ld, ptr(cws)
+        if ext.get("bn") is not None:
+            bm, br, bg, bb, act, e_out = ext["bn"]
+            assert min(bm.numel(), br.numel(), bg.numel(), bb.numel()) >= 256 and (e_out is None or e_out.numel() == M * 256)
+            x.bn_mean, x.bn_rstd, x.bn_gamma, x.bn_beta, x.bn_act, x.a_out = ptr(bm), ptr(br), ptr(bg), ptr(bb), int(act), ptr(e_out)
+        fx = _lib.lib().eamd_rowproj_ext
+        fn, name = (lambda pp, sp: fx(pp, C.byref(x), sp)), "eamd_rowproj_ext"
+    else:
+        fn, name = _lib.lib().eamd_rowproj, "eamd_rowproj"
     if _gemm_record is not None:
-        _gemm_record.append((dict(kind="rowproj", flop=2.0 * M * K * N), keep, lambda sp, p=p: check(fn(C.byref(p), sp), "eamd_rowproj")))
-    check(fn(C.byref(p), stream_ptr()), "eamd_rowproj")
+        _gemm_record.append((dict(kind="rowproj", flop=2.0 * M * K * N), keep, lambda sp, p=p: check(fn(C.byref(p), sp), name)))
+    check(fn(C.byref(p), stream_ptr()), name)
     return out
 
 
diff --git a/include/espnet_amd.h b/include/espnet_amd.h
--- a/include/espnet_amd.h
+++ b/include/espnet_amd.h
@@ -108,6 +108,13 @@
 int eamd_rowproj(const eamd_rowproj_t* p, void* stream);
 int eamd_rowproj_pack_f32(const eamd_rowproj_pack_t* jobs, int njobs, void* stream);
 int64_t eamd_rowproj_lnb_workspace(int M);
+typedef struct {
+  const float* bias_u; const float* bias_v; float* out_u; float* out_v; int64_t ld_uv;
+  const float* a1; int64_t lda1; const float* a2; int64_t lda2; float* a_sum_out; int64_t ld_sum; float* colsum_ws;
+  const float* bn_mean; const float* bn_rstd; const float* bn_gamma; const float* bn_beta; float* a_out;
+  int32_t bn_act; int32_t reserved;
+} eamd_rowproj_ext_t;
+int eamd_rowproj_ext(const eamd_rowproj_t* p, const eamd_rowproj_ext_t* x, void* stream);
 int eamd_ffn_pack_f32(const float* w1, const float* w2, float* fwd_first, float* fwd_second, float* bwd_first, float* bwd_second,
                       int D, int F, void* stream);
 int eamd_ffn_pack_bf16(const void* w1, const void* w2, void* fwd_first, void* fwd_second, void* bwd_first, void* bwd_second,
```

After: 1.152 million frames/s, median of 6. No clear change (+0.7%).
